# QizhiPei/FABind

Hardware: AMD Instinct MI355X
Metric: complexes/sec fwd+bwd (1500p/40l nodes), full IaBNet on the whole graph (pocket model + 4-layer complex model + distance-map head on all nodes / pairs) with the pocket-cls + pocket-centre + coord + distmap + distmap-by-coords + distill losses (BASELINE configs[2] read literally) (higher is better)
Workload: dtype bf16

## Files before the change

fabind_amd/_lib.py:

```python
import ctypes
import os

import torch

from . import config as _cfg

_HERE = os.path.dirname(os.path.abspath(__file__))
LIB_PATH = _cfg.knob("FABIND_LIB") or os.path.join(_HERE, "libfabind_hip.so")

ABI_VERSION = 19
DT_F32, DT_BF16 = 0, 1
ACT_NONE, ACT_SILU, ACT_RELU, ACT_SIGMOID, ACT_STORED_DERIV = 0, 1, 2, 3, 4
GEMM_FAM_NT_F32, GEMM_FAM_NT_F32_BF16, GEMM_FAM_NT_BF16, GEMM_FAM_GLDS, GEMM_FAM_PIPE, GEMM_FAM_X3, GEMM_FAM_X3_PRO, GEMM_FAM_PERSIST = range(8)

LNR_8S16, LNR_8S32, LNR_V8_1, LNR_V8_2, LNR_V8_3, LNR_V8_4, LNR_S2, LNR_S8, LNR_S16, LNR_S32, LNR_COUNT = range(11)
LNB_8S16, LNB_8S32, LNB_V8_1, LNB_V8_2, LNB_V8_3, LNB_S2, LNB_S8, LNB_S16, LNB_S20, LNB_S32, LNB_COUNT = range(11)
RST_BF16_1, RST_BF16_2, RST_BF16_4, RST_GENERIC, RST_COUNT = range(5)
ELF_WAVE1, ELF_WAVE1_TAIL, ELF_WAVE2_TAIL, ELF_CHUNK, ELF_COUNT = range(5)
ELB_NPL1, ELB_NPL2, ELB_NPL3, ELB_COUNT = range(4)

_vp, _i, _f, _l = ctypes.c_void_p, ctypes.c_int, ctypes.c_float, ctypes.c_long


class GemmArgs(ctypes.Structure):
    _fields_ = [(n, _vp) for n in ("A", "A2", "W", "C", "bias", "R", "r_index", "dotvec", "dot_out", "aux", "groups", "C2")] + \
               [(n, _i) for n in ("M", "N", "K", "K1", "lda", "lda2", "ldw", "ldc", "ldr", "ldaux", "dot_ld",
                                  "a_dtype", "w_dtype", "c_dtype", "aux_dtype", "act_pro", "act_epi", "dact_epi",
                                  "accumulate", "store_preact", "n_groups", "max_m", "max_n", "groups_ext", "epi_fast", "k_splits")] + \
               [("alpha", _f), ("p_drop", _f), ("drop_seed", ctypes.c_uint)] + \
               [(n, _vp) for n in ("row_mu", "row_rs", "col_c", "C16")] + [("ldc16", _i), ("split3", _i), ("r_dtype", _i), ("c2_bf16", _i)]


class EdgeBwdArgs(ctypes.Structure):
    _fields_ = [(n, _vp) for n in ("AB", "row", "col", "rhohat", "w_r", "W2p", "Wcp", "W2Tp", "WcTp", "b2", "bc", "w3", "ds",
                                  "dagg", "S1", "Mm", "dT", "dP2", "dP1", "drh", "dABrow", "part", "dbg", "bnd", "d2scratch")] + \
               [(n, _i) for n in ("ldab", "lddagg", "lddab", "E")] + [("p_drop", _f), ("seed", ctypes.c_uint), ("xcd_aware", _i), ("lddab16", _i), ("dAB16", _vp),
                                                                  ("d2f", _vp), ("z3f", _vp)]


class PairUpdateArgs(ctypes.Structure):
    _fields_ = [(n, _vp) for n in ("T", "p_node", "c_node", "z_in", "z_out", "Wop", "bo", "ln_w", "ln_b", "W1p", "b1", "W2p", "b2",
                                  "Wbp", "bb", "bias_out")] + \
               [(n, _i) for n in ("ldt", "b_off", "n_pairs")] + [("eps", _f), ("p_drop", _f), ("seed", ctypes.c_uint)]


class TnJob(ctypes.Structure):
    _fields_ = [(n, _vp) for n in ("Y", "X", "C_part", "out", "out_tail")] + \
               [(n, _i) for n in ("ldy", "ldx", "M", "N", "E", "splits", "e_per", "n_tiles", "with_colsum", "out_dt", "ldo",
                                  "wg0", "n_wg", "blk0", "n_blk", "pad_")]


class AttnFusedBwdArgs(ctypes.Structure):
    _fields_ = [(n, _vp) for n in ("qg", "kv", "a0", "bo", "boT", "toff", "koff", "bconst", "desc", "desc_p", "out", "lse", "dout",
                                  "dqg", "dkv", "dO", "Dv", "da0", "acat", "colpart", "part")] + \
               [(n, _i) for n in ("ldq", "ldkv", "lda0", "ldda0", "ldacat", "kcol0", "ldcolpart", "kp")] + [("scale", _f)] + \
               [(n, _i) for n in ("nsplit", "B", "part_rows")]


class AdamRow(ctypes.Structure):
    _fields_ = [(n, _vp) for n in ("p", "g", "m", "v")] + [("numel", ctypes.c_longlong), ("chunk0", _i), ("step_idx", _i)] + \
               [(n, ctypes.c_double) for n in ("lr", "beta1", "beta2", "eps", "weight_decay")] + [("decoupled", _i), ("pad_", _i)]


SIGNATURES = {
    "fabind_gemm": [ctypes.POINTER(GemmArgs), _vp],
    "fabind_gemm_plan": [ctypes.POINTER(GemmArgs), ctypes.POINTER(_i), ctypes.POINTER(_i), ctypes.POINTER(_i)],
    "fabind_gemm_tn_multi": [_vp, _vp, _i, _vp, _i, _vp, _i, _vp, _vp],
    "fabind_gemm_tn": [_vp, _i, _vp, _i, _vp, _i, _i, _i, _i, _vp, _vp, _i, _i, _vp],
    "fabind_transpose_act": [_vp, _i, _i, _vp, _i, _i, _i, _i, _i, _vp],
    "fabind_colsum": [_vp, _i, _i, _vp, _i, _i, _i, _vp, _i, _vp],
    "fabind_edges_count": [_vp, _vp, _vp, _i, _i, _vp, _vp, _f, _f, _vp, _vp, _vp],
    "fabind_edges_fill": [_vp, _vp, _vp, _i, _i, _vp, _vp, _vp, _f, _f, _vp, _vp, _vp, _vp, _vp, _vp, _vp],
    "fabind_exclusive_scan": [_vp, _vp, _i, _vp],
    "fabind_inter_meta": [_vp, _vp, _i, _vp, _vp, _vp, _i, _vp, _vp, _vp, _vp, _vp, _vp],
    "fabind_edge_geom": [_vp, _vp, _vp, _vp, _vp, _i, _vp, _vp, _vp, _vp, _vp],
    "fabind_gcl_pre": [_vp, _i, _i, _i, _vp, _vp, _vp, _vp, _vp, _i, _i, _i, _vp, _vp],
    "fabind_gcl_edge_fused": [_vp, _i, _i, _vp, _vp, _vp, _vp, _vp, _vp, _vp, _vp, _vp, _i, _vp, _vp, _f, ctypes.c_uint, _vp, _vp, _vp],
    "fabind_gcl_edge_fused_train": [_vp, _i, _i, _vp, _vp, _vp, _vp, _vp, _vp, _vp, _vp, _vp, _i, _vp, _vp, _f, ctypes.c_uint, _vp, _vp, _vp, _vp, _vp, _vp],
    "fabind_gcl_edge_fused_x3": [_vp, _i, _i, _i, _vp, _vp, _vp, _vp, _vp, _vp, _vp, _vp, _vp, _vp, _vp, _i, _vp, _vp, _f, ctypes.c_uint, _vp, _vp],
    "fabind_gcl_edge_fused_x3_train": [_vp, _i, _i, _i, _vp, _vp, _vp, _vp, _vp, _vp, _vp, _vp, _vp, _vp, _vp, _i, _vp, _vp, _f, ctypes.c_uint, _vp, _vp, _vp, _vp, _vp],
    "fabind_gcl_edge_fused_bwd": [ctypes.POINTER(EdgeBwdArgs), _i, _i, _vp],
    "fabind_pair_update_fused": [ctypes.POINTER(PairUpdateArgs), _i, _vp],
    "fabind_gcl_edge_fused_bwd_set_tile": [_i],
    "fabind_gcl_edge_fused_bwd_tile": [],
    "fabind_gcl_edge_fused_bwd_set_variant": [_i],
    "fabind_gcl_edge_fused_set_variant": [_i],
    "fabind_gcl_edge_fused_variant": [],
    "fabind_gcl_edge_fused_bwd_variant": [],
    "fabind_gcl_edge_fused_bwd_variant_for": [_i],
    "fabind_row_stats": [_vp, _i, _i, _f, _i, _i, _vp, _vp, _vp],
    "fabind_layernorm_rows": [_vp, _i, _i, _vp, _vp, _f, _i, _i, _vp, _i, _i, _i, _vp],
    "fabind_edge_ln_concat": [_vp, _i, _i, _vp, _vp, _vp, _vp, _vp, _f, _i, _vp, _i, _i, _i, _vp],
    "fabind_edge_lnfold": [_vp, _i, _i, _i, _vp, _vp, _vp, _vp, _f, _vp, _vp, _vp, _vp, _i, _vp, _f, ctypes.c_uint, _vp],
    "fabind_edge_lnfold_bwd_blocks": [_i],
    "fabind_edge_lnfold_bwd": [_vp, _i, _i, _i, _vp, _vp, _vp, _vp, _f, _vp, _vp, _vp, _vp, _vp, _i, _f, _vp, _vp, _vp, _vp, _i, _vp],
    "fabind_layernorm_rows_form": [_vp, _i, _i, _vp, _i, _i],
    "fabind_layernorm_rows_bwd_form": [_vp, _i, _vp, _i, _vp, _i, _i],
    "fabind_row_stats_form": [_vp, _i, _i, _i],
    "fabind_edge_lnfold_form": [_i, _i, ctypes.POINTER(_i)],
    "fabind_edge_lnfold_blocks": [_i],
    "fabind_edge_lnfold_bwd_form": [_i, ctypes.POINTER(_i)],
    "fabind_inter_coord_fold_blocks": [_i],
    "fabind_inter_coord_fold": [_vp, _i, _i, _vp, _vp, _vp, _f, _f, _vp, _vp, _vp, _i, _vp, _f, ctypes.c_uint, _vp],
    "fabind_post_optimize": [_vp, _vp, _vp, _vp, _vp, _i, _i, _i, _i, _f, _vp, _vp, _vp, _vp],
    "fabind_sym_automorphisms": [_vp, _vp, _vp, _vp, _i, _i, _i, _vp, _vp, _vp, _vp, _vp, _vp],
    "fabind_sym_score": [_vp, _i, _i, _vp, _vp, _vp, _vp, _vp, _i, _i, _vp, _vp, _vp, _vp, _vp, _vp],
    "fabind_pose_stats": [_vp, _vp, _vp, _i, _vp, _vp, _vp],
    "fabind_rank_loss_fwd": [_vp, _vp, _vp, _i, _i, _i, _vp, _vp, _vp, _vp],
    "fabind_multi_copy": [_vp, _i, _i, _vp],
    "fabind_adam_chunk": [],
    "fabind_multi_sqnorm": [_vp, _i, _i, _vp, _vp, _vp, _vp],
    "fabind_multi_adam": [_vp, _i, _i, _vp, _vp, _vp, _f, _i, _vp, _vp, _vp],
    "fabind_zero_empty_rows": [_vp, _i, _vp, _i, _i, _i, _vp, _i, _i, _vp],
    "fabind_split_sum": [_vp, _i, ctypes.c_long, _vp, _i, ctypes.c_long, _vp, _vp],
    "fabind_segment_sum": [_vp, _i, _i, _i, _vp, _vp, _i, _i, _i, _vp, _i, _vp, _i, _vp],
    "fabind_coord_update": [_vp, _vp, _vp, _i, _vp, _vp, _i, _i, _f, _vp, _vp, _vp],
    "fabind_cross_attn_fwd": [_vp, _i, _vp, _vp, _i, _vp, _i, _vp, _i, _i, _i, _vp, _i, _i, _f, _vp, _i, _vp, _i, _vp, _i,
                              _vp],
    "fabind_cross_attn_mfma_fwd": [_vp, _i, _vp, _vp, _i, _vp, _i, _vp, _i, _i, _i, _vp, _i, _i, _f, _vp, _i, _vp, _i, _vp, _i,
                                   _vp],
    "fabind_cross_attn_fused_fwd": [_vp, _i, _vp, _vp, _i, _vp, _i, _vp, _i, _vp, _vp, _vp, _vp, _i, _i, _i, _i, _i, _f, _vp, _i, _vp, _i, _vp, _vp],
    "fabind_cross_attn_fused_bwd": [ctypes.POINTER(AttnFusedBwdArgs), _i, _i, _i, _i, _i, _i, _vp],
    "fabind_pair_bot_pack": [_vp, _i, _vp, _i, _vp, _vp, _vp, _vp, _i, _vp, _i, _l, _vp],
    "fabind_pair_bo_pack": [_vp, _i, _vp, _i, _vp, _vp, _vp, _vp, _i, _vp, _i, _l, _vp],
    "fabind_cross_attn_mfma_bwd": [_vp, _i, _vp, _i, _vp, _i, _i, _i, _vp, _i, _i, _i, _f, _vp, _vp, _vp, _vp, _vp, _vp, _vp,
                                   _vp, _vp, _vp],
    "fabind_pair_bmat": [_vp, _i, _vp, _i, _i, _vp, _i, _vp, _i, _vp],
    "fabind_pair_hadamard": [_vp, _vp, _i, _i, _vp, _vp, _i, _i, _vp, _vp, _i, _vp, _i, _i, _vp],
    "fabind_inter_attn_fwd": [_vp, _i, _vp, _i, _i, _vp, _i, _vp, _vp, _vp, _vp, _vp, _vp, _vp, _i, _vp, _vp, _vp,
                              _vp, _f, _i, _vp, _vp, _vp, _vp, _vp, _vp, _vp],
    "fabind_inter_attn_fwd_rows": [_vp, _i, _vp, _i, _i, _vp, _i, _vp, _vp, _vp, _vp, _vp, _vp, _vp, _i, _vp, _vp, _vp,
                                   _vp, _f, _i, _vp, _vp, _vp, _vp, _vp, _vp, _vp, _i, _i, _vp],
    "fabind_layernorm_rows_bwd": [_vp, _i, _i, _vp, _vp, _i, _i, _f, _i, _i, _vp, _i, _i, _vp, _vp, _i, _vp],
    "fabind_edge_concat": [_vp, _i, _i, _vp, _vp, _vp, _i, _vp, _i, _i, _i, _vp],
    "fabind_las_step": [_vp, _vp, _vp, _vp, _vp, _vp, _vp, _i, _i, _f, _f, _vp, _vp, _vp],
    "fabind_select_rows": [_vp, _vp, _vp, _i, _i, _vp, _vp],
    "fabind_add": [_vp, _vp, _vp, _l, _vp],
    "fabind_mul_dact": [_vp, _i, _vp, _i, _i, _vp, _i, _l, _f, _vp],
    "fabind_mul_dact_colsum": [_vp, _i, _vp, _i, _i, _vp, _i, _i, _i, _vp, _vp, _i, _f, _vp],
    "fabind_drop_mix": [_vp, _vp, _vp, _l, _f, ctypes.c_uint, _vp],
    "fabind_drop_mix_bwd": [_vp, _vp, _vp, _l, _f, ctypes.c_uint, _vp],
    "fabind_mul_dropmask_colsum": [_vp, _i, _vp, _i, _i, _i, _f, ctypes.c_uint, _vp, _vp, _i, _vp],
    "fabind_rowdot_bwd": [_vp, _i, _vp, _i, _vp, _i, _i, _i, _vp, _vp, _vp, _i, _vp],
    "fabind_edge_geom_bwd": [_vp, _vp, _vp, _vp, _vp, _vp, _vp, _vp, _vp, _vp, _i, _i, _i, _vp, _vp, _vp, _vp],
    "fabind_gcl_pre_bwd": [_vp, _i, _i, _vp, _vp, _i, _vp, _vp, _vp, _i, _vp],
    "fabind_gather_dact": [_vp, _i, _vp, _vp, _i, _i, _vp, _i, _i, _i, _vp],
    "fabind_coord_update_bwd": [_vp, _vp, _vp, _i, _i, _f, _vp, _vp, _vp, _vp],
    "fabind_cross_attn_bwd": [_vp, _i, _vp, _i, _vp, _i, _i, _i, _vp, _i, _i, _i, _f, _vp, _vp, _vp, _vp, _vp, _vp, _vp,
                              _vp, _vp, _vp],
    "fabind_pair_bias_cat": [_vp, _i, _vp, _i, _i, _i, _vp, _i, _vp, _i, _vp, _vp, _i, _vp, _i, _vp, _vp],
    "fabind_batched_transpose_pad": [_vp, _i, _vp, _i, _i, _i, _i, _vp, _vp],
    "fabind_node_chain_fwd": [_vp, _i, _vp, _i, _vp, _vp, _vp, _vp, _vp, _vp, _i, _i, _vp, _i, _vp, _i, _vp, _i, _i, _i, _vp],
    "fabind_node_chain_x3_fwd": [_vp, _i, _vp, _i, _vp, _vp, _vp, _vp, _vp, _vp, _vp, _vp, _vp, _vp, _i, _i, _vp, _i, _vp, _i, _vp, _i, _vp, _i, _vp, _i,
                                 _i, _i, _vp],
    "fabind_rows_hadamard_bwd": [_vp, _i, _i, _vp, _i, _i, _vp, _vp, _vp, _i, _vp, _i, _vp],
    "fabind_pair_hadamard_bwd_grid": [_vp, _i, _i, _vp, _i, _i, _vp, _vp, _vp, _vp, _i, _vp, _i, _vp],
    "fabind_pair_hadamard_bwd_rows": [_vp, _i, _i, _vp, _i, _i, _vp, _i, _i, _vp, _vp, _vp, _vp, _i, _vp, _i, _vp, _i, _vp],
    "fabind_pair_hadamard_bwd": [_vp, _i, _i, _vp, _vp, _i, _i, _vp, _vp, _i, _i, _vp, _vp, _i, _vp, _vp, _i, _vp, _vp, _i,
                                 _vp],
    "fabind_inter_attn_bwd": [_vp, _i, _vp, _i, _i, _vp, _vp, _vp, _vp, _vp, _vp, _vp, _vp, _vp, _vp, _vp, _vp, _f, _i,
                              _vp, _vp, _vp, _vp, _vp, _vp, _vp, _vp, _vp, _vp, _i, _vp],
    "fabind_inter_attn_bwd_rows": [_vp, _i, _vp, _i, _i, _vp, _vp, _vp, _vp, _vp, _vp, _vp, _vp, _vp, _vp, _vp, _vp, _f, _i,
                                   _vp, _vp, _vp, _vp, _vp, _vp, _vp, _vp, _vp, _vp, _i, _vp, _i, _i, _vp],
    "fabind_las_step_bwd": [_vp, _vp, _vp, _vp, _vp, _vp, _vp, _vp, _i, _i, _f, _f, _vp, _vp, _vp],
    "fabind_pair_bias_bwd": [_vp, _i, _vp, _i, _i, _vp, _vp, _i, _i, _i, _vp, _vp, _vp, _vp, _vp],
    "fabind_pair_bias_btcat": [_vp, _i, _vp, _vp, _vp, _i, _i, _i, _vp, _i, _i, _vp],
    "fabind_pair_bias_finish": [_vp, _vp, _i, _i, _vp, _vp, _i, _vp, _vp, _l, _vp],
    "fabind_pack_frag_multi": [_vp, _vp, _i, _vp],
    "fabind_lower_bound": [_vp, _i, _vp, _i, _vp, _vp],
    "fabind_pocket_center_fwd": [_vp, _vp, _vp, _vp, _i, _i, _f, _i, _vp, _vp, _vp],
    "fabind_pocket_center_bwd": [_vp, _vp, _vp, _vp, _i, _i, _f, _vp, _vp, _vp, _vp, _vp],
    "fabind_pair_dist_fwd": [_vp, _i, _i, _vp, _vp, _f, _f, _f, _vp, _vp],
    "fabind_pair_dist_bwd": [_vp, _i, _i, _vp, _vp, _vp, _f, _f, _f, _vp, _vp, _vp],
    "fabind_block_hadamard_fwd": [_vp, _i, _i, _vp, _i, _vp, _i, _i, _vp, _i, _vp],
    "fabind_block_hadamard_bwd": [_vp, _i, _i, _vp, _i, _vp, _i, _vp, _i, _i, _vp, _i, _i, _vp, _vp, _i, _vp, _i, _vp],
    "fabind_loss_fwd": [_vp, _vp, _l, _vp, _vp, _vp, _l, _vp, _vp, _i, _vp, _l, _vp, _vp, _l, _f, _f, _f, _f, _f, _f, _vp, _vp, _vp, _vp, _vp, _vp],
    "fabind_loss_bwd": [_vp, _vp, _l, _vp, _vp, _vp, _l, _vp, _vp, _i, _l, _vp, _vp, _l, _f, _f, _f, _f, _f, _f, _vp, _vp, _vp,
                        _vp, _vp, _vp, _vp, _vp, _vp],
    "fabind_layernorm_fwd": [_vp, _vp, _vp, _f, _i, _i, _vp, _vp, _vp, _vp],
    "fabind_layernorm_bwd": [_vp, _vp, _vp, _vp, _vp, _i, _i, _vp, _vp, _vp, _vp],
}

_lib = None


def load():
    global _lib
    if _lib is not None:
        return _lib
    if not os.path.exists(LIB_PATH):
        raise RuntimeError(
            "fabind_amd: %s is missing -- build it with `python -m fabind_amd.build` (hipcc, gfx950). "
            "There is no CPU/eager fallback for the hot path." % LIB_PATH)
    lib = ctypes.CDLL(LIB_PATH)
    lib.fabind_last_error.restype = ctypes.c_char_p
    lib.fabind_abi_version.restype = ctypes.c_int
    got = lib.fabind_abi_version()
    if got != ABI_VERSION:
# ... 68 lines not shown
```

fabind_amd/csrc/fused_common.h:

```cpp
#pragma once
#include "common.h"

#define FE_BM 64
#define FE_PRIO(x) __builtin_amdgcn_s_setprio(x)

__device__ __forceinline__ float fe_sigmoid(float x) { return __builtin_amdgcn_rcpf(1.0f + __builtin_amdgcn_exp2f(-1.44269504f * x)); }
__device__ __forceinline__ float fe_silu(float x) { return x * fe_sigmoid(x); }

__device__ __forceinline__ uint32_t fe_hash(uint32_t x) {
    x ^= x >> 16; x *= 0x7feb352dU; x ^= x >> 15; x *= 0x846ca68bU; x ^= x >> 16;
    return x;
}
__device__ __forceinline__ float fe_keep(uint32_t seed, uint32_t e, uint32_t c, uint32_t H, uint32_t thr16, float scale) {
    const uint32_t h = fe_hash(seed + (e >> 1) * H + c);
    return (((e & 1u) ? (h >> 16) : (h & 0xffffu)) >= thr16) ? scale : 0.f;
}

__device__ __forceinline__ void unpack8(const uint4 u, float* f) {
    f[0] = __uint_as_float(u.x << 16); f[1] = __uint_as_float(u.x & 0xffff0000u);
    f[2] = __uint_as_float(u.y << 16); f[3] = __uint_as_float(u.y & 0xffff0000u);
    f[4] = __uint_as_float(u.z << 16); f[5] = __uint_as_float(u.z & 0xffff0000u);
    f[6] = __uint_as_float(u.w << 16); f[7] = __uint_as_float(u.w & 0xffff0000u);
}
__device__ __forceinline__ uint4 pack8(const float* f) {
// ... 125 lines not shown
    bf16x8_t b0[4];
    fe_gemm_prefetch(Wp, wave, lane, b0);
    fe_gemm_rolled_pf<H, MI, SWAP, SWZ>(sX, Wp, wave, lane, acc, b0, wmode);
}
template <int H, int MI, bool SWAP = false, int SWZ = 7>
__device__ __forceinline__ void fe_gemm_rot(const bf16_t* sX, const bf16_t* __restrict__ Wp, int wave, int lane, f32x4_t (&acc)[MI][4]) {
    bf16x8_t b0[4];
    fe_gemm_prefetch(Wp, wave, lane, b0);
    fe_gemm_rot_pf<H, MI, SWAP, SWZ>(sX, Wp, wave, lane, acc, b0);
}

template <int H, int MI, int SWZ>
__device__ __forceinline__ void fe_gemm_x3(const bf16_t* sXh, const bf16_t* sXl, const bf16_t* __restrict__ Wph,
                                           const bf16_t* __restrict__ Wpl, int wave, int lane, f32x4_t (&acc)[MI][4]) {
    constexpr int NKS = H / 32;
    constexpr int NG = H / 16;
    const int fr = lane & 15, fq = lane >> 4;
    const bf16x8_t* wh = (const bf16x8_t*)Wph + ((size_t)wave * 4) * 64 + lane;
    const bf16x8_t* wl = (const bf16x8_t*)Wpl + ((size_t)wave * 4) * 64 + lane;
    bf16x8_t h0[4], l0[4], h1[4], l1[4];
#pragma unroll
    for (int j = 0; j < 4; ++j) { h0[j] = wh[(size_t)j * 64]; l0[j] = wl[(size_t)j * 64]; }
#pragma unroll 1
    for (int ks = 0; ks < NKS; ks += 2) {
#pragma unroll
        for (int j = 0; j < 4; ++j) { h1[j] = wh[((size_t)(ks + 1) * NG + j) * 64]; l1[j] = wl[((size_t)(ks + 1) * NG + j) * 64]; }
        bf16x8_t ah[MI], al[MI];
#pragma unroll
        for (int i = 0; i < MI; ++i) {
            const int r = i * 16 + fr;
            const int o = r * H + (((ks * 4 + fq) ^ (r & SWZ)) * 8);
            ah[i] = *(const bf16x8_t*)&sXh[o];
            al[i] = *(const bf16x8_t*)&sXl[o];
        }
        FE_PRIO(1);
#pragma unroll
        for (int i = 0; i < MI; ++i) {
#pragma unroll
            for (int j = 0; j < 4; ++j) acc[i][j] = __builtin_amdgcn_mfma_f32_16x16x32_bf16(h0[j], al[i], acc[i][j], 0, 0, 0);
#pragma unroll
            for (int j = 0; j < 4; ++j) acc[i][j] = __builtin_amdgcn_mfma_f32_16x16x32_bf16(l0[j], ah[i], acc[i][j], 0, 0, 0);
#pragma unroll
            for (int j = 0; j < 4; ++j) acc[i][j] = __builtin_amdgcn_mfma_f32_16x16x32_bf16(h0[j], ah[i], acc[i][j], 0, 0, 0);
        }
        FE_PRIO(0);
        {
            const int kn = min(ks + 2, NKS - 2);
#pragma unroll
            for (int j = 0; j < 4; ++j) { h0[j] = wh[((size_t)kn * NG + j) * 64]; l0[j] = wl[((size_t)kn * NG + j) * 64]; }
        }
#pragma unroll
        for (int i = 0; i < MI; ++i) {
            const int r = i * 16 + fr;
            const int o = r * H + ((((ks + 1) * 4 + fq) ^ (r & SWZ)) * 8);
            ah[i] = *(const bf16x8_t*)&sXh[o];
            al[i] = *(const bf16x8_t*)&sXl[o];
        }
        FE_PRIO(1);
#pragma unroll
        for (int i = 0; i < MI; ++i) {
#pragma unroll
            for (int j = 0; j < 4; ++j) acc[i][j] = __builtin_amdgcn_mfma_f32_16x16x32_bf16(h1[j], al[i], acc[i][j], 0, 0, 0);
#pragma unroll
            for (int j = 0; j < 4; ++j) acc[i][j] = __builtin_amdgcn_mfma_f32_16x16x32_bf16(l1[j], ah[i], acc[i][j], 0, 0, 0);
#pragma unroll
            for (int j = 0; j < 4; ++j) acc[i][j] = __builtin_amdgcn_mfma_f32_16x16x32_bf16(h1[j], ah[i], acc[i][j], 0, 0, 0);
        }
        FE_PRIO(0);
    }
}

__device__ __forceinline__ void fe_split2(float x0, float x1, uint32_t& hi, uint32_t& lo) {
    hi = pack2_bf16(x0, x1);
    lo = pack2_bf16(x0 - __uint_as_float(hi << 16), x1 - __uint_as_float(hi & 0xffff0000u));
}

template <int H>
__device__ __forceinline__ void fe_tile_store(const bf16_t* sB, bf16_t* __restrict__ g, int e0, int ne, int tid) {
    constexpr int CH = H / 8;
    bf16_t* gt = g + (size_t)e0 * H;
    for (unsigned q = tid; q < (unsigned)ne * CH; q += H) {
        const unsigned rw = q / CH, ch = q % CH;
        *(uint4*)&gt[rw * H + ch * 8] = *(const uint4*)&sB[rw * H + ((ch ^ (rw & 7)) * 8)];
    }
}

typedef unsigned int fe_u32x4_t __attribute__((ext_vector_type(4)));
__device__ __forceinline__ void fe_store16_stream(__amdgpu_buffer_rsrc_t rsrc, unsigned byte_off, const uint4 v) {
    __builtin_amdgcn_raw_buffer_store_b128(fe_u32x4_t{v.x, v.y, v.z, v.w}, rsrc, (int)byte_off, 0,  16);
}
__device__ __forceinline__ __amdgpu_buffer_rsrc_t fe_rsrc(void* base, unsigned bytes) {
    return __builtin_amdgcn_make_buffer_rsrc(base, 0, (int)bytes, 0x00020000);
}
template <int H>
__device__ __forceinline__ void fe_tile_store_stream(const bf16_t* sB, bf16_t* __restrict__ g, int e0, int ne, int tid) {
    constexpr int CH = H / 8;
    const __amdgpu_buffer_rsrc_t rs = fe_rsrc(g + (size_t)e0 * H, (unsigned)ne * H * 2);
    for (unsigned q = tid; q < (unsigned)ne * CH; q += H) {
        const unsigned rw = q / CH, ch = q % CH;
        fe_store16_stream(rs, (rw * H + ch * 8) * 2, *(const uint4*)&sB[rw * H + ((ch ^ (rw & 7)) * 8)]);
    }
}

template <int MI>
__device__ __forceinline__ void fe_zero(f32x4_t (&acc)[MI][4]) {
#pragma unroll
    for (int i = 0; i < MI; ++i)
#pragma unroll
        for (int j = 0; j < 4; ++j) acc[i][j] = f32x4_t{0.f, 0.f, 0.f, 0.f};
}


template <int H, bool WITH_RH, int BM_, int SWZ = 7>
__device__ __forceinline__ float fe_scan_rows(const bf16_t* sX, const int* sRow, const float* sRh, int ne, bool head_cont,
                                              bool tail_cont, float* out, unsigned ld, float* bnd_tile, int c,
                                              bf16_t* out16 = nullptr, unsigned ld16 = 0) {
    auto put = [&](int node, float v) {
        if (out) out[(unsigned)node * ld + c] = v;
        if (out16) out16[(unsigned)node * ld16 + c] = f32_to_bf16(v);
    };
    float run = 0.f, pwr = 0.f;
    int cur = sRow[0];
    bool first = true;
    for (int rw0 = 0; rw0 < ne; rw0 += 8) {
        int rr[8];
        float v[8], rhv[8];
#pragma unroll
        for (int u = 0; u < 8; ++u) {
            const int rw = min(rw0 + u, BM_ - 1);
            rr[u] = sRow[rw];
            rhv[u] = WITH_RH ? sRh[rw] : 0.f;
            v[u] = bf16_to_f32(sX[rw * H + (((c >> 3) ^ (rw & SWZ)) * 8) + (c & 7)]);
        }
#pragma unroll
        for (int u = 0; u < 8; ++u) {
            if (rw0 + u < ne) {
                if (rr[u] != cur) {
                    if (first && head_cont) bnd_tile[c] = run; else put(cur, run);
                    run = 0.f; cur = rr[u]; first = false;
                }
                run += v[u];
                if (WITH_RH) pwr += rhv[u] * v[u];
            }
        }
    }
    if (ne > 0) {
        if (first && head_cont) bnd_tile[c] = run;
        else if (tail_cont) bnd_tile[H + c] = run;
        else put(cur, run);
    }
    return pwr;
}

template <int H, bool WITH_RH, int SWZ>
__device__ __forceinline__ float fe_scan_runs64(const bf16_t* sX, const int* sRow, const float* sRh, int ne, bool head_cont,
                                                bool tail_cont, float* out, unsigned ld, float* bnd_tile, int c,
                                                bf16_t* out16 = nullptr, unsigned ld16 = 0, const bf16_t* sXlo = nullptr) {
    const int lane = threadIdx.x & 63;
    const int mine = sRow[lane], prev = sRow[max(lane - 1, 0)];
    const float rhl = WITH_RH ? sRh[lane] : 0.f;
    const unsigned long long m = __ballot(lane < ne && lane > 0 && mine != prev);
    const int c8 = c >> 3, c7 = c & 7;
    float v[64];
#pragma unroll
    for (int rw = 0; rw < 64; ++rw) v[rw] = bf16_to_f32(sX[rw * H + ((c8 ^ (rw & SWZ)) * 8) + c7]);
    if (sXlo) {
#pragma unroll
        for (int rw = 0; rw < 64; ++rw) v[rw] += bf16_to_f32(sXlo[rw * H + ((c8 ^ (rw & SWZ)) * 8) + c7]);
    }
    float run = 0.f, pwr = 0.f;
    int rs = 0;
    auto flush = [&](bool last) {
        if (rs == 0 && head_cont) bnd_tile[c] = run;
        else if (last && tail_cont) bnd_tile[H + c] = run;
        else {
            const unsigned node = (unsigned)__builtin_amdgcn_readlane(mine, rs);
            if (out) out[node * ld + c] = run;
            if (out16) out16[node * ld16 + c] = f32_to_bf16(run);
        }
    };
#pragma unroll
    for (int rw = 0; rw < 64; ++rw) {
        if (rw < ne) {
            if ((m >> rw) & 1ull) {
                flush(false);
                run = 0.f;
                rs = rw;
            }
            run += v[rw];
            if (WITH_RH) pwr += __builtin_bit_cast(float, __builtin_amdgcn_readlane(__builtin_bit_cast(int, rhl), rw)) * v[rw];
        }
    }
    if (ne > 0) flush(true);
    return pwr;
}

template <int BM>
__global__ void fe_boundary_fix_kernel(const int* __restrict__ row, int E, int H, const float* __restrict__ bnd, float* out,
                                       unsigned ld, bf16_t* out16 = nullptr, unsigned ld16 = 0) {
    const int t = blockIdx.x, e0 = t * BM, ne = min(BM, E - e0);
    if (ne <= 0 || e0 + ne >= E) return;
    const int r = row[e0 + ne - 1];
    if (row[e0 + ne] != r) return;
    if (row[e0] == r && e0 > 0 && row[e0 - 1] == r) return;
    for (int c = threadIdx.x; c < H; c += blockDim.x) {
        float sum = bnd[((size_t)t * 2 + 1) * H + c];
        for (int u = t + 1;; ++u) {
            const int f0 = u * BM, fn = min(BM, E - f0);
            sum += bnd[((size_t)u * 2) * H + c];
            const bool through = row[f0 + fn - 1] == r && f0 + fn < E && row[f0 + fn] == r;
            if (!through) break;
        }
        if (out) out[(unsigned)r * ld + c] = sum;
        if (out16) out16[(unsigned)r * ld16 + c] = f32_to_bf16(sum);
    }
}

__device__ __forceinline__ float fe3_row16_sum(float v) {
#define FE_DPP_ADD(ctrl_) v += __builtin_bit_cast(float, __builtin_amdgcn_update_dpp(0, __builtin_bit_cast(int, v), (ctrl_), 0xF, 0xF, true))
    FE_DPP_ADD(0xB1);
    FE_DPP_ADD(0x4E);
    FE_DPP_ADD(0x141);
    FE_DPP_ADD(0x140);
#undef FE_DPP_ADD
    return v;
}

typedef float fe_f2 __attribute__((ext_vector_type(2)));
__device__ __forceinline__ void fe3_silu_pair(const fe_f2 z, fe_f2& m, fe_f2& d) {
    const fe_f2 t = z * -1.44269504f;
    const fe_f2 o = fe_f2{__builtin_amdgcn_exp2f(t.x), __builtin_amdgcn_exp2f(t.y)} + 1.0f;
    const fe_f2 s = fe_f2{__builtin_amdgcn_rcpf(o.x), __builtin_amdgcn_rcpf(o.y)};
    m = z * s;
    d = s + (m - m * s);
}
__device__ __forceinline__ uint32_t fe3_pack(const fe_f2 v) { return pack2_bf16(v.x, v.y); }
__device__ __forceinline__ fe_f2 fe3_unpack(const uint32_t u) { return fe_f2{__uint_as_float(u << 16), __uint_as_float(u & 0xffff0000u)}; }

__device__ __forceinline__ uint4 fe3_bload16(const __amdgpu_buffer_rsrc_t rs, const unsigned voff, const unsigned soff) {
    const fe_u32x4_t v = __builtin_amdgcn_raw_buffer_load_b128(rs, (int)voff, (int)soff, 0);
    return make_uint4(v.x, v.y, v.z, v.w);
}
__device__ __forceinline__ void fe3_bstore16(const __amdgpu_buffer_rsrc_t rs, const unsigned voff, const unsigned soff, const uint4 v) {
    __builtin_amdgcn_raw_buffer_store_b128(fe_u32x4_t{v.x, v.y, v.z, v.w}, rs, (int)voff, (int)soff, 0);
}

struct FabindEdgeBwdArgs;
int fe_bwd3_launch(const FabindEdgeBwdArgs* a, int H, int bm, int n_groups, hipStream_t stream);
int fe_fwd3_launch(const float* AB, int ldab, int H, const int* row, const int* col, const float* rhohat, const float* w_r,
                   const void* W2ph, const void* W2pl, const float* b2, const void* Wcph, const void* Wcpl, const float* bc,
                   const float* w3, int E, float* agg, float* s_out, uint32_t thr16, float dscale, unsigned seed, float* bnd,
                   int xcd_aware, hipStream_t stream, void* Msave = nullptr, void* d2f = nullptr, void* z3f = nullptr);
int fe_fwd2_launch(const void* AB, int ldab, int H, const int* row, const int* col, const float* rhohat, const float* w_r,
                   const void* W2p, const float* b2, const void* Wcp, const float* bc, const float* w3, int E, float* agg,
                   float* s_out, uint32_t thr16, float dscale, unsigned seed, float* bnd, void* agg16, int xcd_aware, hipStream_t stream,
                   void* Msave = nullptr, void* d2f = nullptr, void* z3f = nullptr);
int fe_bwd4_launch(const FabindEdgeBwdArgs* a, int H, int n_groups, hipStream_t stream);
```

fabind_amd/csrc/fused_edge.hip:

```cpp
#include "common.h"
#include "fabind_hip.h"
#include "fused_common.h"

static int g_fe_xcd_aware = 1;
extern "C" void fabind_gcl_edge_fused_set_xcd_aware(int on) { g_fe_xcd_aware = on ? 1 : 0; }
static int g_fe_fwd_variant = 1;
extern "C" int fabind_gcl_edge_fused_set_variant(int v) {
    FB_REQUIRE(v == 1, "fabind_gcl_edge_fused_set_variant: 1 (row-wise / operand-swapped) is the only forward form built (variant 0 was retired in round 5)");
    g_fe_fwd_variant = v;
    return 0;
}
extern "C" int fabind_gcl_edge_fused_variant(void) { return g_fe_fwd_variant; }

static int fe_fwd_entry(const void* AB, int ldab, int H, const int* row, const int* col, const float* rhohat,
                        const float* w_r, const void* W2p, const float* b2, const void* Wcp, const float* bc,
                        const float* w3, int E, float* agg, float* s_out, float p_drop, unsigned seed,
                        float* bnd, void* agg16, void* Msave, void* d2f, void* z3f, hipStream_t stream) {
    if (E <= 0) return 0;
    FB_REQUIRE((Msave != nullptr) == (d2f != nullptr) && (Msave != nullptr) == (z3f != nullptr),
               "fabind_gcl_edge_fused_train: M, d2f and z3f come together");
    FB_REQUIRE(Msave == nullptr || g_fe_fwd_variant == 1, "fabind_gcl_edge_fused_train: the saving forward is the row-wise / operand-swapped kernel (variant 1)");
    FB_REQUIRE(bnd != nullptr, "fabind_gcl_edge_fused: bnd (ceil(E/64) x 2 x H floats of scratch) is required");
    FB_REQUIRE(p_drop >= 0.f && p_drop < 1.f, "fabind_gcl_edge_fused: p_drop in [0, 1)");
    const uint32_t thr16 = (uint32_t)(p_drop * 65536.0f + 0.5f);
    const float dscale = 1.0f / (1.0f - (float)thr16 / 65536.0f);
    FB_REQUIRE(H == 512 || H == 256 || H == 128 || H == 64, "fabind_gcl_edge_fused: H must be 64, 128, 256 or 512");
    FB_REQUIRE(ldab % 8 == 0, "fabind_gcl_edge_fused: ldab % 8");
    {
        const int rc = fe_fwd2_launch(AB, ldab, H, row, col, rhohat, w_r, W2p, b2, Wcp, bc, w3, E, agg, s_out, thr16, dscale, seed, bnd,
                                      agg16, g_fe_xcd_aware, stream, Msave, d2f, z3f);
        if (rc) return rc;
    }
    hipLaunchKernelGGL((fe_boundary_fix_kernel<FE_BM>), dim3((E + FE_BM - 1) / FE_BM), dim3(H < 256 ? H : 256), 0, stream, row, E, H,
                       bnd, agg, (unsigned)H, (bf16_t*)agg16, (unsigned)H);
    FB_CHECK_LAUNCH();
    return 0;
}

extern "C" int fabind_gcl_edge_fused(const void* AB, int ldab, int H, const int* row, const int* col, const float* rhohat,
                                     const float* w_r, const void* W2p, const float* b2, const void* Wcp, const float* bc,
                                     const float* w3, int E, float* agg, float* s_out, float p_drop, unsigned seed,
                                     float* bnd, void* agg16, hipStream_t stream) {
    return fe_fwd_entry(AB, ldab, H, row, col, rhohat, w_r, W2p, b2, Wcp, bc, w3, E, agg, s_out, p_drop, seed, bnd, agg16, nullptr, nullptr,
                        nullptr, stream);
}
extern "C" int fabind_gcl_edge_fused_train(const void* AB, int ldab, int H, const int* row, const int* col, const float* rhohat,
                                           const float* w_r, const void* W2p, const float* b2, const void* Wcp, const float* bc,
                                           const float* w3, int E, float* agg, float* s_out, float p_drop, unsigned seed,
                                           float* bnd, void* agg16, void* M, void* d2f, void* z3f, hipStream_t stream) {
    FB_REQUIRE(M != nullptr && d2f != nullptr && z3f != nullptr, "fabind_gcl_edge_fused_train: M, d2f, z3f are required");
    return fe_fwd_entry(AB, ldab, H, row, col, rhohat, w_r, W2p, b2, Wcp, bc, w3, E, agg, s_out, p_drop, seed, bnd, agg16, M, d2f, z3f, stream);
}

static int fe_x3_entry(const float* AB, int ldab, int n_rows, int H, const int* row, const int* col, const float* rhohat,
                       const float* w_r, const void* W2ph, const void* W2pl, const float* b2, const void* Wcph,
                       const void* Wcpl, const float* bc, const float* w3, int E, float* agg, float* s_out,
                       float p_drop, unsigned seed, float* bnd, void* Msave, void* d2f, void* z3f, hipStream_t stream) {
    if (E <= 0) return 0;
    FB_REQUIRE(bnd != nullptr, "fabind_gcl_edge_fused_x3: bnd (ceil(E/64) x 2 x H floats of scratch) is required");
    FB_REQUIRE(p_drop >= 0.f && p_drop < 1.f, "fabind_gcl_edge_fused_x3: p_drop in [0, 1)");
    FB_REQUIRE(H == 512 || H == 256 || H == 128 || H == 64, "fabind_gcl_edge_fused_x3: H must be 64, 128, 256 or 512");
    FB_REQUIRE(ldab % 4 == 0 && ((uintptr_t)AB & 15) == 0, "fabind_gcl_edge_fused_x3: AB must be 16-byte aligned with ldab % 4 == 0");
    FB_REQUIRE(n_rows >= 0 && (size_t)n_rows * (size_t)ldab * 4 < ((size_t)1 << 32), "fabind_gcl_edge_fused_x3: AB larger than 4 GiB (n_rows * ldab * 4 bytes): split the batch");
    const uint32_t thr16 = (uint32_t)(p_drop * 65536.0f + 0.5f);
    const float dscale = 1.0f / (1.0f - (float)thr16 / 65536.0f);
    const int rc = fe_fwd3_launch(AB, ldab, H, row, col, rhohat, w_r, W2ph, W2pl, b2, Wcph, Wcpl, bc, w3, E, agg, s_out, thr16, dscale,
                                  seed, bnd, g_fe_xcd_aware, stream, Msave, d2f, z3f);
    if (rc) return rc;
    hipLaunchKernelGGL((fe_boundary_fix_kernel<FE_BM>), dim3((E + FE_BM - 1) / FE_BM), dim3(H < 256 ? H : 256), 0, stream, row, E, H,
                       bnd, agg, (unsigned)H, (bf16_t*)nullptr, 0u);
    FB_CHECK_LAUNCH();
    return 0;
}
extern "C" int fabind_gcl_edge_fused_x3(const float* AB, int ldab, int n_rows, int H, const int* row, const int* col, const float* rhohat,
                                        const float* w_r, const void* W2ph, const void* W2pl, const float* b2, const void* Wcph,
                                        const void* Wcpl, const float* bc, const float* w3, int E, float* agg, float* s_out,
                                        float p_drop, unsigned seed, float* bnd, hipStream_t stream) {
    return fe_x3_entry(AB, ldab, n_rows, H, row, col, rhohat, w_r, W2ph, W2pl, b2, Wcph, Wcpl, bc, w3, E, agg, s_out, p_drop, seed, bnd,
                       nullptr, nullptr, nullptr, stream);
}
extern "C" int fabind_gcl_edge_fused_x3_train(const float* AB, int ldab, int n_rows, int H, const int* row, const int* col, const float* rhohat,
                                              const float* w_r, const void* W2ph, const void* W2pl, const float* b2, const void* Wcph,
                                              const void* Wcpl, const float* bc, const float* w3, int E, float* agg, float* s_out,
                                              float p_drop, unsigned seed, float* bnd, void* M, void* d2f, void* z3f, hipStream_t stream) {
    FB_REQUIRE(M != nullptr && d2f != nullptr && z3f != nullptr, "fabind_gcl_edge_fused_x3_train: M, d2f, z3f are required");
    return fe_x3_entry(AB, ldab, n_rows, H, row, col, rhohat, w_r, W2ph, W2pl, b2, Wcph, Wcpl, bc, w3, E, agg, s_out, p_drop, seed, bnd,
                       M, d2f, z3f, stream);
}

template <int H, int BM, bool DBG>
__global__ __launch_bounds__(H, (BM == 32 ? 4 : 2)) void gcl_edge_fused_bwd_kernel(const FabindEdgeBwdArgs p) {
    constexpr int TPE = H / BM;
    constexpr int CPT = BM / 8;
    constexpr int MI = BM / 16;
    extern __shared__ __attribute__((aligned(16))) unsigned char smem[];
    bf16_t* sX = (bf16_t*)smem;
    bf16_t* sY = sX + BM * H;
    int* sRow = (int*)(sY + BM * H);
    float* sDs = (float*)(sRow + BM);
    float* sRh = sDs + BM;
    const bf16_t* __restrict__ AB = (const bf16_t*)p.AB;
    const int tid = threadIdx.x, lane = tid & 63, wave = tid >> 6;
    const int fr = lane & 15, cq = lane >> 4;
    const int el = tid / TPE, cth = tid % TPE;
    const int n_tiles = (p.E + BM - 1) / BM;
    const uint32_t thr16 = (uint32_t)(p.p_drop * 65536.0f + 0.5f);
    const float dscale = 1.0f / (1.0f - (float)thr16 / 65536.0f);
    int cbase[2][2];
#pragma unroll
    for (int f0 = 0; f0 < 2; ++f0)
#pragma unroll
        for (int f2 = 0; f2 < 2; ++f2)
            cbase[f0][f2] = cq * 4 * H + (wave * 8 + (((cq & 1) ^ f2) << 2) + ((fr >> 3) ^ f0)) * 8 + (fr & 7);
#define FE_COFF(i, j, r) (cbase[(r) & 1][(j) >> 1] + ((i) * 16 + (r)) * H + ((((j) & 1) ^ ((r) >> 1)) * 16))
    long long tph[12] = {0, 0, 0, 0, 0, 0, 0, 0, 0, 0, 0, 0};
    long long tlast = 0;
#define FE_TICK(k_)                                                   \
    if constexpr (DBG) {                                              \
        const long long now_ = __builtin_readcyclecounter();         \
        tph[k_] += now_ - tlast;                                      \
        tlast = now_;                                                 \
    }
    float pb2[4] = {0.f, 0.f, 0.f, 0.f}, pbc[4] = {0.f, 0.f, 0.f, 0.f}, pw3[4] = {0.f, 0.f, 0.f, 0.f}, pwr = 0.f;

    uint4 pfa[CPT], pfb[CPT];
    const unsigned uld = (unsigned)p.ldab;
    auto fe_prefetch = [&](unsigned r, unsigned c) {
        const unsigned aoff = r * uld + cth * (CPT * 8), boff = c * uld + H + cth * (CPT * 8);
#pragma unroll
        for (int q = 0; q < CPT; ++q) {
            pfa[q] = *(const uint4*)(AB + (aoff + q * 8));
            pfb[q] = *(const uint4*)(AB + (boff + q * 8));
        }
    };
    int t_first, t_end, t_step;
    if (p.xcd_aware && (gridDim.x & 7) == 0) {
        const int tpx = (n_tiles + 7) / 8, xcd = blockIdx.x & 7;
        t_first = xcd * tpx + (int)(blockIdx.x >> 3);
        t_end = min(n_tiles, (xcd + 1) * tpx);
        t_step = (int)(gridDim.x >> 3);
    } else {
        t_first = blockIdx.x; t_end = n_tiles; t_step = gridDim.x;
    }
    unsigned ur = 0, uc = 0;
    if (t_first < t_end) {
        const int e0 = t_first * BM;
        if (el < min(BM, p.E - e0)) {
            ur = (unsigned)(p.row + e0)[(unsigned)el];
            uc = (unsigned)(p.col + e0)[(unsigned)el];
        }
    }
    fe_prefetch(ur, uc);

    for (int tile = t_first; tile < t_end; tile += t_step) {
        const int e0 = tile * BM;
        const int ne = min(BM, p.E - e0);
        int lz = 0;
        asm volatile("" : "+s"(lz));
        const float* w_r = p.w_r + lz;
        const float* b2 = p.b2 + lz;
        const float* bc = p.bc + lz;
        const float* w3 = p.w3 + lz;
        const bf16_t* W2p = (const bf16_t*)p.W2p + lz;
        const bf16_t* Wcp = (const bf16_t*)p.Wcp + lz;
        const bf16_t* W2Tp = (const bf16_t*)p.W2Tp + lz;
        const bf16_t* WcTp = (const bf16_t*)p.WcTp + lz;
        if constexpr (DBG) tlast = __builtin_readcyclecounter();
        const int* grow = p.row + e0;
        const int* gcol = p.col + e0;
        const float* grh = p.rhohat + e0;
        const float* gds = p.ds + e0;
        if (tid < BM) {
            const bool ok = tid < ne;
            sRow[tid] = ok ? grow[(unsigned)tid] : -1;
// ... 106 lines not shown
        fe_tile_store<H>(sX, (bf16_t*)p.dT, e0, ne, tid);
        FE_TICK(1)

#pragma unroll
        for (int i = 0; i < MI; ++i)
#pragma unroll
            for (int r = 0; r < 4; ++r) {
                const int rr = sRow[i * 16 + cq * 4 + r];
                const unsigned doff = (unsigned)max(rr, 0) * (unsigned)p.lddagg + wave * 64 + fr;
                const float keep = rr >= 0 ? 1.f : 0.f;
#pragma unroll
                for (int j = 0; j < 4; ++j) acc[i][j][r] = p.dagg[doff + j * 16] * keep;
            }
        FE_TICK(5)
        fe_gemm_rolled<H, MI>(sX, WcTp, wave, lane, acc);
        FE_TICK(2)
#pragma unroll 1
        for (int j = 0; j < 4; ++j) {
            FE_JADDR(j)
            float a2 = 0.f;
#pragma unroll
            for (int i = 0; i < MI; ++i)
#pragma unroll
                for (int r = 0; r < 4; ++r) {
                    const uint32_t pk = (r >> 1) ? d2b[i][0] : d2a[i][0];
                    const float dd = __uint_as_float((r & 1) ? (pk & 0xffff0000u) : (pk << 16));
                    const float dp = acc[i][0][r] * dd;
                    a2 += dp;
                    sY[FE_LOFF(i, r)] = f32_to_bf16(dp);
                }
            pb2[0] += a2;
            FE_ROT_ACC() FE_ROT_D2() FE_ROT4(pb2)
        }
        __syncthreads();
        FE_TICK(6)
        fe_tile_store<H>(sY, (bf16_t*)p.dP2, e0, ne, tid);
        FE_TICK(1)

        fe_prefetch(ur, uc);
        fe_zero(acc);
        fe_gemm_rolled<H, MI>(sY, W2Tp, wave, lane, acc);
        FE_TICK(2)
#pragma unroll 1
        for (int j = 0; j < 4; ++j) {
            FE_JADDR(j)
#pragma unroll
            for (int i = 0; i < MI; ++i)
#pragma unroll
                for (int r = 0; r < 4; ++r) sX[FE_LOFF(i, r)] = f32_to_bf16(acc[i][0][r]);
            FE_ROT_ACC()
        }
        __syncthreads();
        FE_TICK(7)

        if (el < ne) {
            const float rh = sRh[el];
            const float* wp = w_r + (unsigned)(cth * (CPT * 8));
            float dot = 0.f;
#pragma unroll
            for (int q = 0; q < CPT; ++q) {
                float fa[8], fb[8], g[8];
                unpack8(pfa[q], fa);
                unpack8(pfb[q], fb);
                uint4* sp = (uint4*)&sX[el * H + (((cth * CPT + q) ^ (el & 7)) * 8)];
                unpack8(*sp, g);
                const float4 w0 = *(const float4*)(wp + q * 8), w1 = *(const float4*)(wp + q * 8 + 4);
                const float wv[8] = {w0.x, w0.y, w0.z, w0.w, w1.x, w1.y, w1.z, w1.w};
#pragma unroll
                for (int k = 0; k < 8; ++k) {
                    const float z = fa[k] + fb[k] + rh * wv[k], sg = fe_sigmoid(z);
                    g[k] *= sg * (1.0f + z * (1.0f - sg));
                    dot += g[k] * wv[k];
                }
                *sp = pack8(g);
            }
#pragma unroll
            for (int o = 1; o < TPE; o <<= 1) dot += __shfl_xor(dot, o, 64);
            if (cth == 0) (p.drh + e0)[(unsigned)el] = dot;
        }
        ur = nr; uc = nc;
        fe_prefetch(ur, uc);
        __syncthreads();
        FE_TICK(8)
        fe_tile_store<H>(sX, (bf16_t*)p.dP1, e0, ne, tid);
        FE_TICK(1)

        {
            const bool head_cont = e0 > 0 && p.row[e0 - 1] == sRow[0];
            const bool tail_cont = e0 + ne < p.E && p.row[e0 + ne] == sRow[ne - 1];
            pwr += fe_scan_rows<H, true, BM>(sX, sRow, sRh, ne, head_cont, tail_cont, p.dABrow, (unsigned)p.lddab,
                                             p.bnd + (size_t)tile * 2 * H, tid);
        }
        __syncthreads();
        FE_TICK(9)
    }
    if constexpr (DBG) {
        if (p.dbg && blockIdx.x == 0 && tid == 0)
            for (int k = 0; k < 12; ++k) ((long long*)p.dbg)[k] = tph[k];
    }

    float* part = p.part + (size_t)blockIdx.x * 4 * H;
#pragma unroll
    for (int j = 0; j < 4; ++j) {
        float a = pb2[j], b = pbc[j], c = pw3[j];
        a += __shfl_xor(a, 16, 64); a += __shfl_xor(a, 32, 64);
        b += __shfl_xor(b, 16, 64); b += __shfl_xor(b, 32, 64);
        c += __shfl_xor(c, 16, 64); c += __shfl_xor(c, 32, 64);
        if (cq == 0) {
            const int colj = wave * 64 + j * 16 + fr;
            part[colj] = a; part[H + colj] = b; part[2 * H + colj] = c;
        }
    }
    part[3 * H + tid] = pwr;
}

#undef FE_COFF
#undef FE_ROT4
#undef FE_ROT_ACC
#undef FE_ROT_D2
#undef FE_JADDR
#undef FE_LOFF
#undef FE_TICK

static int g_fe_bwd_bm = 64;
extern "C" int fabind_gcl_edge_fused_bwd_set_tile(int bm) {
    FB_REQUIRE(bm == 64, "fabind_gcl_edge_fused_bwd_set_tile: 64 edges per tile (the 32-edge build of the two-tile kernel was retired in round 5)");
    g_fe_bwd_bm = bm;
    return 0;
}
extern "C" int fabind_gcl_edge_fused_bwd_tile(void) { return g_fe_bwd_bm; }
static bool g_fe_bwd_variant_set = false;
static int g_fe_bwd_variant = 5;
extern "C" int fabind_gcl_edge_fused_bwd_set_variant(int v) {
    FB_REQUIRE(v == 0 || v == 5,
               "fabind_gcl_edge_fused_bwd_set_variant: 0 (two LDS tiles of 64 edges: the default for H <= 128) or 5 (row-wise, operand-swapped in-place tile + store wave: the recompute default above); variants 1-4 were knobs nobody reached and were retired in round 5");
    g_fe_bwd_variant = v;
    g_fe_bwd_variant_set = true;
    return 0;
}
extern "C" int fabind_gcl_edge_fused_bwd_variant(void) { return g_fe_bwd_variant; }
extern "C" int fabind_gcl_edge_fused_bwd_variant_for(int H) {
    return (!g_fe_bwd_variant_set && g_fe_bwd_variant == 5 && H <= 128) ? 0 : g_fe_bwd_variant;
}

extern "C" int fabind_gcl_edge_fused_bwd(const FabindEdgeBwdArgs* a_in, int H, int n_groups, hipStream_t stream) {
    FabindEdgeBwdArgs a_copy = *a_in;
    a_copy.xcd_aware = g_fe_xcd_aware;
    const FabindEdgeBwdArgs* a = &a_copy;
    if (a->E <= 0 || n_groups <= 0) return 0;
    FB_REQUIRE(H == 512 || H == 256 || H == 128 || H == 64, "fabind_gcl_edge_fused_bwd: H must be 64, 128, 256 or 512");
    FB_REQUIRE(a->ldab % 8 == 0, "fabind_gcl_edge_fused_bwd: ldab % 8");
    FB_REQUIRE(a->p_drop >= 0.f && a->p_drop < 1.f, "fabind_gcl_edge_fused_bwd: p_drop in [0, 1)");
    const int g_fe_bwd_variant = fabind_gcl_edge_fused_bwd_variant_for(H);
    if (a->d2f != nullptr || a->z3f != nullptr) {
        FB_REQUIRE(a->d2f != nullptr && a->z3f != nullptr, "fabind_gcl_edge_fused_bwd: d2f and z3f (saved by fabind_gcl_edge_fused_train) come together");
        return fe_bwd4_launch(a, H, n_groups, stream);
    }
    if (g_fe_bwd_variant == 5) return fe_bwd3_launch(a, H, 64, n_groups, stream);
    FB_REQUIRE(a->dAB16 == nullptr, "fabind_gcl_edge_fused_bwd: dAB16 (bf16 receiving-side sums) exists in variant 5 only");
    FB_REQUIRE(a->bnd != nullptr, "fabind_gcl_edge_fused_bwd: bnd (ceil(E / tile) x 2 x H floats of scratch) is required");
    const int BMr = g_fe_bwd_bm;
    const size_t lds = (size_t)2 * BMr * H * 2 + BMr * (sizeof(int) + 2 * sizeof(float));
#define FE_LAUNCH2(HH, BB)                                                                                         \
    do {                                                                                                           \
        static bool set_ = false;                                                                                  \
        if (!set_) { (void)hipFuncSetAttribute((const void*)gcl_edge_fused_bwd_kernel<HH, BB, false>, hipFuncAttributeMaxDynamicSharedMemorySize, (int)lds); set_ = true; } \
        hipLaunchKernelGGL((gcl_edge_fused_bwd_kernel<HH, BB, false>), dim3(n_groups), dim3(HH), lds, stream, *a);  \
    } while (0)
#define FE_LAUNCH(HH) FE_LAUNCH2(HH, 64)
    if (a->dbg != nullptr && H == 512) {
        static bool setd_ = false;
        if (!setd_) { (void)hipFuncSetAttribute((const void*)gcl_edge_fused_bwd_kernel<512, 64, true>, hipFuncAttributeMaxDynamicSharedMemorySize, (int)lds); }
        hipLaunchKernelGGL((gcl_edge_fused_bwd_kernel<512, 64, true>), dim3(n_groups), dim3(512), lds, stream, *a);
    } else
    if (H == 512) FE_LAUNCH(512); else if (H == 256) FE_LAUNCH(256); else if (H == 128) FE_LAUNCH(128); else FE_LAUNCH(64);
    hipLaunchKernelGGL((fe_boundary_fix_kernel<64>), dim3((a->E + 63) / 64), dim3(H < 256 ? H : 256), 0, stream, a->row, a->E, H,
                           a->bnd, a->dABrow, (unsigned)a->lddab);
#undef FE_LAUNCH
#undef FE_LAUNCH2
#undef FE_COFF
#undef FE_ROT4
#undef FE_ROT_ACC
#undef FE_ROT_D2
#undef FE_JADDR
#undef FE_LOFF
#undef FE_TICK
    FB_CHECK_LAUNCH();
    return 0;
}
```

fabind_amd/csrc/fused_edge_bwd3.hip:

```cpp
#include "common.h"
#include "fabind_hip.h"
#include "fused_common.h"
#ifndef FE3_ROT
#define FE3_ROT 0
#endif

template <int H, int SWZ>
__device__ __forceinline__ void fe3_wave_store(const bf16_t* sB, bf16_t* __restrict__ g, int e0, int ne, int lane) {
    constexpr int CH = H / 8;
    bf16_t* gt = g + (size_t)e0 * H;
    const unsigned total = (unsigned)ne * CH;
#pragma unroll 8
    for (unsigned q = lane; q < total; q += 64) {
        const unsigned rw = q / CH, ch = q % CH;
        *(uint4*)&gt[rw * H + ch * 8] = *(const uint4*)&sB[rw * H + ((ch ^ (rw & SWZ)) * 8)];
    }
}

template <int H, int SWZ>
__device__ __forceinline__ void fe3_wave_store_nt(const bf16_t* sB, bf16_t* __restrict__ g, int e0, int ne, int lane) {
    constexpr int CH = H / 8;
    const __amdgpu_buffer_rsrc_t rs = fe_rsrc(g + (size_t)e0 * H, (unsigned)ne * H * 2);
    const unsigned total = (unsigned)ne * CH;
#pragma unroll 8
    for (unsigned q = lane; q < total; q += 64) {
        const unsigned rw = q / CH, ch = q % CH;
        const uint4 v = *(const uint4*)&sB[rw * H + ((ch ^ (rw & SWZ)) * 8)];
        __builtin_amdgcn_raw_buffer_store_b128(fe_u32x4_t{v.x, v.y, v.z, v.w}, rs, (int)((rw * H + ch * 8) * 2), 0,  2);
    }
}

template <int H, int BM, bool DROP, bool DBG>
__global__ __launch_bounds__(H + 64) void gcl_edge_fused_bwd3_kernel(const FabindEdgeBwdArgs p, const int xf) {
    constexpr int MI = BM / 16;
    constexpr int NW = H / 64;
    constexpr int CH = H / 8;
    constexpr int EPW = 64 / CH;
    constexpr int EPI = NW * EPW;
    constexpr int NIT = BM / EPI;
    constexpr int PB = (NIT % 8 == 0) ? 8 : (NIT % 6 == 0) ? 6 : 4;
    static_assert(NIT % PB == 0 && BM % 16 == 0, "tile height");
    constexpr int SWZ = (H >= 128) ? 15 : 7;
    extern __shared__ __attribute__((aligned(16))) unsigned char smem[];
    bf16_t* sX = (bf16_t*)smem;
    bf16_t* sD = sX + BM * H;
    int* sTab = (int*)(sD + BM * H);
    float* sPart = (float*)(sTab + 8 * BM);
    const bf16_t* __restrict__ AB = (const bf16_t*)p.AB;
    const int tid = threadIdx.x, lane = tid & 63, wave = tid >> 6;
    const int n_tiles = (p.E + BM - 1) / BM;
    int t_first, t_end, t_step;
    if (p.xcd_aware && (gridDim.x & 7) == 0) {
        const int tpx = (n_tiles + 7) / 8, xcd = blockIdx.x & 7;
        t_first = xcd * tpx + (int)(blockIdx.x >> 3);
        t_end = min(n_tiles, (xcd + 1) * tpx);
        t_step = (int)(gridDim.x >> 3);
    } else {
        t_first = blockIdx.x; t_end = n_tiles; t_step = gridDim.x;
    }

    if (wave == NW) {
        __syncthreads();
        for (int tile = t_first; tile < t_end; tile += t_step) {
            const int e0 = tile * BM;
            const int ne = min(BM, p.E - e0);
            const bool st = !(xf & 1), nt = (xf & 32) == 0;
            auto put = [&](bf16_t* dst) {
                if (nt) fe3_wave_store_nt<H, SWZ>(sX, dst, e0, ne, lane); else fe3_wave_store<H, SWZ>(sX, dst, e0, ne, lane);
            };
            __syncthreads();
            if (st) put((bf16_t*)p.S1);
            fe3_wave_store<H, SWZ>(sD, (bf16_t*)p.d2scratch + (size_t)blockIdx.x * (BM * H), 0, BM, lane);
            __syncthreads();
            __syncthreads();
            if (st) put((bf16_t*)p.Mm);
            __syncthreads();
            __syncthreads();
            if (st) put((bf16_t*)p.dT);
            __syncthreads();
            __syncthreads();
            if (st) put((bf16_t*)p.dP2);
            __syncthreads();
            __syncthreads();
            __syncthreads();
            if (st) put((bf16_t*)p.dP1);
            __syncthreads();
        }
        __syncthreads();
        return;
    }

    const int fr = lane & 15, cq = lane >> 4;
    const int sub = lane / CH, ch = lane % CH;
    const uint32_t thr16 = (uint32_t)(p.p_drop * 65536.0f + 0.5f);
    const float dscale = 1.0f / (1.0f - (float)thr16 / 65536.0f);
    for (int k = 0; k < 4; ++k) sPart[k * H + tid] = 0.f;
    const unsigned uld = (unsigned)p.ldab;
    const __amdgpu_buffer_rsrc_t rs_d1 = fe_rsrc((bf16_t*)p.d2scratch + (size_t)blockIdx.x * (BM * H), BM * H * 2);
    const unsigned rw_off = (unsigned)((wave * EPW + sub) * CH + ch) * 16;
    const __amdgpu_buffer_rsrc_t rs_ab = fe_rsrc(const_cast<void*>(p.AB), 0xffffffffu);
    const __amdgpu_buffer_rsrc_t rs_dagg = fe_rsrc(const_cast<float*>(p.dagg), 0xffffffffu);
    const int cx = (wave * 8 + (cq >> 1)) ^ (fr & SWZ);
    const int lbase = fr * H + (cq & 1) * 4;
    const int wmode = DBG ? ((xf >> 2) & 3) : 0;
#define FE_QOFF(i, j) (lbase + (i) * 16 * H + ((cx ^ ((j) * 2)) * 8))
    const int fcol = wave * 64 + cq * 4;
    long long tph[12] = {0, 0, 0, 0, 0, 0, 0, 0, 0, 0, 0, 0};
    long long tlast = 0;
#define FE_TICK(k_)                                                   \
    if constexpr (DBG) {                                              \
        const long long now_ = __builtin_readcyclecounter();         \
        tph[k_] += now_ - tlast;                                      \
        tlast = now_;                                                 \
    }
    int tb_r = -1, tb_c = 0;
    float tb_d = 0.f, tb_h = 0.f;
    auto fetch_tables = [&](int tile) {
        const int e0 = tile * BM;
        const int ne = min(BM, p.E - e0);
        if (tid < BM) {
            const bool ok = tid < ne;
            const unsigned ge = (unsigned)(e0 + (ok ? tid : 0));
            const int r = p.row[ge], c = p.col[ge];
            const float d = p.ds[ge], h = p.rhohat[ge];
            tb_r = ok ? r : -1; tb_c = ok ? c : 0; tb_d = ok ? d : 0.f; tb_h = ok ? h : 0.f;
        }
    };
    auto commit_tables = [&](int hb) {
        int* tb = sTab + hb * 4 * BM;
        if (tid < BM) {
            tb[tid] = tb_r;
            tb[BM + tid] = tb_c;
            ((float*)tb)[2 * BM + tid] = tb_d;
            ((float*)tb)[3 * BM + tid] = tb_h;
        }
    };
    constexpr int NB = NIT / PB;
    uint4 ga[NB][PB], gb[NB][PB];
    auto gather_batch = [&](const int* tab, int b) {
#pragma unroll
        for (int u = 0; u < PB; ++u) {
            const int e = (b * PB + u) * EPI + wave * EPW + sub;
            const unsigned r = (unsigned)max(tab[e], 0), c = (unsigned)tab[BM + e];
            ga[b][u] = fe3_bload16(rs_ab, (r * uld + ch * 8) * 2, 0);
            gb[b][u] = fe3_bload16(rs_ab, (c * uld + H + ch * 8) * 2, 0);
        }
    };
    static_assert(BM <= H, "one thread per table row");
    if (t_first < t_end) { fetch_tables(t_first); commit_tables(0); }
    __syncthreads();
    int hb = 0;

    for (int tile = t_first; tile < t_end; tile += t_step, hb ^= 1) {
        const int e0 = tile * BM;
        const int ne = min(BM, p.E - e0);
        const int* sRow = sTab + hb * 4 * BM;
        const int* sCol = sRow + BM;
        const float* sDs = (const float*)(sRow + 2 * BM);
        const float* sRh = (const float*)(sRow + 3 * BM);
        int lz = 0;
        asm volatile("" : "+s"(lz));
        const float* w_r = p.w_r + lz;
        const float* b2 = p.b2 + lz;
        const float* bc = p.bc + lz;
        const float* w3 = p.w3 + lz;
        const bf16_t* W2p = (const bf16_t*)p.W2p + lz;
        const bf16_t* Wcp = (const bf16_t*)p.Wcp + lz;
        const bf16_t* W2Tp = (const bf16_t*)p.W2Tp + lz;
// ... 157 lines not shown

        fe_zero(acc);
        if (DBG || FE3_ROT == 0) fe_gemm_rolled<H, MI, true, SWZ>(sX, W2Tp, wave, lane, acc, wmode);
        else fe_gemm_rot<H, MI, true, SWZ>(sX, W2Tp, wave, lane, acc);
        __syncthreads();
        FE_TICK(2)
        uint4 gd[NIT];
#pragma unroll
        for (int it = 0; it < NIT; ++it) gd[it] = fe3_bload16(rs_d1, rw_off, (unsigned)(it * EPI * CH * 16));
#pragma unroll
        for (int j = 0; j < 4; ++j)
#pragma unroll
            for (int i = 0; i < MI; ++i)
                *(uint2*)&sX[FE_QOFF(i, j)] = make_uint2(pack2_bf16(acc[i][j][0], acc[i][j][1]), pack2_bf16(acc[i][j][2], acc[i][j][3]));
        __syncthreads();
        FE_TICK(7)

        const bool has_next = tile + t_step < t_end;
        {
            fe_f2 wv2[4];
            {
                const float4 w0 = *(const float4*)(w_r + ch * 8), w1 = *(const float4*)(w_r + ch * 8 + 4);
                wv2[0] = fe_f2{w0.x, w0.y}; wv2[1] = fe_f2{w0.z, w0.w}; wv2[2] = fe_f2{w1.x, w1.y}; wv2[3] = fe_f2{w1.z, w1.w};
            }
#pragma unroll
            for (int it0 = 0; it0 < NIT; it0 += PB) {
#pragma unroll
                for (int u = 0; u < PB; ++u) {
                    const int e = (it0 + u) * EPI + wave * EPW + sub;
                    uint4* sp = (uint4*)&sX[e * H + ((ch ^ (e & SWZ)) * 8)];
                    const uint4 gs = *sp;
                    const uint4 gq = gd[it0 + u];
                    const uint32_t ug[4] = {gs.x, gs.y, gs.z, gs.w}, ud[4] = {gq.x, gq.y, gq.z, gq.w};
                    uint32_t pg[4];
                    fe_f2 dot2 = fe_f2{0.f, 0.f};
#pragma unroll
                    for (int k = 0; k < 4; ++k) {
                        const fe_f2 g = fe3_unpack(ug[k]) * fe3_unpack(ud[k]);
                        dot2 += g * wv2[k];
                        pg[k] = fe3_pack(g);
                    }
                    float dot = dot2.x + dot2.y;
                    *sp = make_uint4(pg[0], pg[1], pg[2], pg[3]);
                    if constexpr (CH >= 16) {
                        dot = fe3_row16_sum(dot);
#pragma unroll
                        for (int o = 16; o < CH; o <<= 1) dot += __shfl_xor(dot, o, 64);
                    } else {
#pragma unroll
                        for (int o = 1; o < CH; o <<= 1) dot += __shfl_xor(dot, o, 64);
                    }
                    if (ch == 0 && e < ne) (p.drh + e0)[(unsigned)e] = dot;
                }
            }
        }
        __syncthreads();
        FE_TICK(8)

        if (has_next) fetch_tables(tile + t_step);
        if (!(xf & 16)) {
            const bool head_cont = e0 > 0 && p.row[e0 - 1] == sRow[0];
            const bool tail_cont = e0 + ne < p.E && p.row[e0 + ne] == sRow[ne - 1];
            sPart[3 * H + tid] += fe_scan_rows<H, true, BM, SWZ>(sX, sRow, sRh, ne, head_cont, tail_cont, p.dAB16 ? nullptr : p.dABrow, (unsigned)p.lddab,
                                                         p.bnd + (size_t)tile * 2 * H, tid, (bf16_t*)p.dAB16, (unsigned)p.lddab16);
        }
        if (has_next) commit_tables(hb ^ 1);
        __syncthreads();
        FE_TICK(9)
    }
    if constexpr (DBG) {
        if (p.dbg && blockIdx.x == 0 && tid == 0)
            for (int k = 0; k < 12; ++k) ((long long*)p.dbg)[k] = tph[k];
    }
    __syncthreads();
    float* part = p.part + (size_t)blockIdx.x * 4 * H;
    for (int k = 0; k < 4; ++k) part[k * H + tid] = sPart[k * H + tid];
#undef FE_QOFF
#undef FE_TICK
}

static int g_fe_bwd3_exp = 0;
extern "C" void fabind_gcl_edge_fused_bwd3_set_exp(int m) { g_fe_bwd3_exp = m; }

int fe_bwd3_launch(const FabindEdgeBwdArgs* a, int H, int bm, int n_groups, hipStream_t stream) {
    FB_REQUIRE(a->d2scratch != nullptr, "fabind_gcl_edge_fused_bwd: the store-wave form needs d2scratch (n_groups x 64 x H x 2 bytes)");
    FB_REQUIRE(a->bnd != nullptr, "fabind_gcl_edge_fused_bwd: bnd (ceil(E / tile) x 2 x H floats of scratch) is required");
    FB_REQUIRE(a->lddagg % 4 == 0 && ((uintptr_t)a->dagg & 15) == 0, "fabind_gcl_edge_fused_bwd: dagg must be 16-byte aligned with lddagg % 4 == 0");
    const size_t lds = (size_t)2 * bm * H * 2 + (size_t)8 * bm * sizeof(int) + (size_t)4 * H * sizeof(float);
#define FE_LAUNCH3_(HH, BB, KK, DD)                                                                                   \
    do {                                                                                                           \
        static bool set_ = false;                                                                                  \
        if (!set_) {                                                                                               \
            const hipError_t e_ = hipFuncSetAttribute((const void*)gcl_edge_fused_bwd3_kernel<HH, BB, KK, DD>,         \
                                                      hipFuncAttributeMaxDynamicSharedMemorySize, (int)lds);       \
            if (e_ != hipSuccess) { fabind_set_error(hipGetErrorString(e_)); return (int)e_; }                     \
            set_ = true;                                                                                           \
        }                                                                                                          \
        hipLaunchKernelGGL((gcl_edge_fused_bwd3_kernel<HH, BB, KK, DD>), dim3(n_groups), dim3(HH + 64), lds, stream, *a, g_fe_bwd3_exp); \
    } while (0)
#define FE_LAUNCH3(HH, BB, DD) do { if (a->p_drop > 0.f) FE_LAUNCH3_(HH, BB, true, DD); else FE_LAUNCH3_(HH, BB, false, DD); } while (0)
    FB_REQUIRE(bm == 64, "fabind_gcl_edge_fused_bwd: the store-wave form has 64-edge tiles");
    if (a->dbg != nullptr && H == 512) FE_LAUNCH3(512, 64, true);
    else if (H == 512) FE_LAUNCH3(512, 64, false); else if (H == 256) FE_LAUNCH3(256, 64, false);
    else if (H == 128) FE_LAUNCH3(128, 64, false); else FE_LAUNCH3(64, 64, false);
    hipLaunchKernelGGL((fe_boundary_fix_kernel<64>), dim3((a->E + 63) / 64), dim3(H < 256 ? H : 256), 0, stream, a->row, a->E, H,
                       a->bnd, a->dAB16 ? nullptr : a->dABrow, (unsigned)a->lddab, (bf16_t*)a->dAB16, (unsigned)a->lddab16);
#undef FE_LAUNCH3
#undef FE_LAUNCH3_
    FB_CHECK_LAUNCH();
    return 0;
}
```

fabind_amd/csrc/fused_edge_bwd4.hip:

```cpp
#include "common.h"
#include "fabind_hip.h"
#include "fused_common.h"

#ifndef FE4_E3_DB
#define FE4_E3_DB 0
#endif
#ifndef FE4_SCAN64
#define FE4_SCAN64 0
#endif
#ifndef FE4_P5_BATCH
#define FE4_P5_BATCH 4
#endif

#ifndef FE4_NT_LOADS
#define FE4_NT_LOADS 1
#endif
#if FE4_NT_LOADS
typedef unsigned fe_u32x2_nt_t __attribute__((ext_vector_type(2)));
__device__ __forceinline__ uint2 fe4_ldq(const bf16_t* p_) { const fe_u32x2_nt_t v = __builtin_nontemporal_load((const fe_u32x2_nt_t*)p_); return make_uint2(v.x, v.y); }
#else
__device__ __forceinline__ uint2 fe4_ldq(const bf16_t* p_) { return *(const uint2*)p_; }
#endif

template <int H>
__global__ __launch_bounds__(H, 4) void gcl_edge_fused_bwd4_kernel(const FabindEdgeBwdArgs p, const int xf) {
    constexpr int BM = FE_BM, MI = BM / 16;
    constexpr int NW = H / 64;
    constexpr int CH = H / 8;
    constexpr int EPW = 64 / CH;
    constexpr int EPI = NW * EPW;
    constexpr int NIT = BM / EPI;
    constexpr int SWZ = (H >= 128) ? 15 : 7;
    static_assert(BM <= H, "one thread per table row");
    extern __shared__ __attribute__((aligned(16))) unsigned char smem[];
    bf16_t* sX = (bf16_t*)smem;
    int* sTab = (int*)(sX + BM * H);
    float* sPart = (float*)(sTab + 8 * BM);
    const int tid = threadIdx.x, lane = tid & 63, wave = tid >> 6;
    const int fr = lane & 15, cq = lane >> 4;
    const int sub = lane / CH, ch = lane % CH;
    const int n_tiles = (p.E + BM - 1) / BM;
    int t_first, t_end, t_step;
    if (p.xcd_aware && (gridDim.x & 7) == 0) {
        const int tpx = (n_tiles + 7) / 8, xcd = blockIdx.x & 7;
        t_first = xcd * tpx + (int)(blockIdx.x >> 3);
        t_end = min(n_tiles, (xcd + 1) * tpx);
        t_step = (int)(gridDim.x >> 3);
    } else {
        t_first = blockIdx.x; t_end = n_tiles; t_step = gridDim.x;
    }
    for (int k = 0; k < 4; ++k) sPart[k * H + tid] = 0.f;
    const unsigned uld = (unsigned)p.ldab;
    const __amdgpu_buffer_rsrc_t rs_ab = fe_rsrc(const_cast<void*>(p.AB), 0xffffffffu);
    const __amdgpu_buffer_rsrc_t rs_dagg = fe_rsrc(const_cast<float*>(p.dagg), 0xffffffffu);
    const bf16_t* __restrict__ d2f = (const bf16_t*)p.d2f;
    const bf16_t* __restrict__ z3f = (const bf16_t*)p.z3f;
    const int cx = (wave * 8 + (cq >> 1)) ^ (fr & SWZ);
    const int lbase = fr * H + (cq & 1) * 4;
#define FE_OPAQUE(v_) asm volatile("" : "+v"(v_))
#define FE_QOFF(i, j) (lb_ + (i) * 16 * H + ((cx_ ^ ((j) * 2)) * 8))
#define FE_FOFF(i, j) (fbase + (size_t)((i) * 4 + (j)) * 256)
    const int fcol = wave * 64 + cq * 4;

    int tb_r = -1, tb_c = 0;
    float tb_d = 0.f, tb_h = 0.f;
    auto fetch_tables = [&](int tile) {
        const int e0 = tile * BM;
        const int ne = min(BM, p.E - e0);
        if (tid < BM) {
            const bool ok = tid < ne;
            const unsigned ge = (unsigned)(e0 + (ok ? tid : 0));
            const int r = p.row[ge], c = p.col[ge];
            const float d = p.ds[ge], h = p.rhohat[ge];
            tb_r = ok ? r : -1; tb_c = ok ? c : 0; tb_d = ok ? d : 0.f; tb_h = ok ? h : 0.f;
        }
    };
    auto commit_tables = [&](int hb) {
        int* tb = sTab + hb * 4 * BM;
        if (tid < BM) {
            tb[tid] = tb_r;
            tb[BM + tid] = tb_c;
            ((float*)tb)[2 * BM + tid] = tb_d;
            ((float*)tb)[3 * BM + tid] = tb_h;
        }
    };
    if (t_first < t_end) { fetch_tables(t_first); commit_tables(0); }
    __syncthreads();
    int hb = 0;

    for (int tile = t_first; tile < t_end; tile += t_step, hb ^= 1) {
        const int e0 = tile * BM;
        const int ne = min(BM, p.E - e0);
        const int* sRow = sTab + hb * 4 * BM;
        const int* sCol = sRow + BM;
        const float* sDs = (const float*)(sRow + 2 * BM);
        const float* sRh = (const float*)(sRow + 3 * BM);
        int lz = 0;
        asm volatile("" : "+s"(lz));
        const float* w_r = p.w_r + lz;
        const float* w3 = p.w3 + lz;
        const bf16_t* W2Tp = (const bf16_t*)p.W2Tp + lz;
        const bf16_t* WcTp = (const bf16_t*)p.WcTp + lz;
        int ln_ = lane;
        FE_OPAQUE(ln_);
        const size_t fbase = (((size_t)tile * NW + wave) * (MI * 4) * 64 + ln_) * 4;
        auto copy_out = [&](void* dst) {
            const __amdgpu_buffer_rsrc_t rs = fe_rsrc((bf16_t*)dst + (size_t)e0 * H, (unsigned)ne * H * 2);
            int t_ = tid;
            FE_OPAQUE(t_);
#pragma unroll
            for (int it = 0; it < BM * CH / H; ++it) {
                const int q = t_ + it * H;
                const int rw = q / CH, c8 = q % CH;
                const uint4 v = *(const uint4*)&sX[rw * H + ((c8 ^ (rw & SWZ)) * 8)];
                __builtin_amdgcn_raw_buffer_store_b128(fe_u32x4_t{v.x, v.y, v.z, v.w}, rs, (int)((rw * H + c8 * 8) * 2), 0,  2);
            }
        };

        {
            int cx_ = cx, lb_ = lbase;
            FE_OPAQUE(cx_); FE_OPAQUE(lb_);
            uint2 zq[4][MI];
#pragma unroll
            for (int j = 0; j < 4; ++j)
#pragma unroll
                for (int i = 0; i < MI; ++i) zq[j][i] = fe4_ldq(&z3f[FE_FOFF(i, j)]);
            float dsr[MI];
#pragma unroll
            for (int i = 0; i < MI; ++i) dsr[i] = sDs[i * 16 + fr];
            float4 wq4[4];
#pragma unroll
            for (int j = 0; j < 4; ++j) wq4[j] = *(const float4*)(w3 + fcol + j * 16);
#pragma unroll
            for (int j = 0; j < 4; ++j) {
                const fe_f2 w01 = fe_f2{wq4[j].x, wq4[j].y}, w23 = fe_f2{wq4[j].z, wq4[j].w};
                fe_f2 a3a = fe_f2{0.f, 0.f}, a3b = a3a, aca = a3a, acb = a3a;
#pragma unroll
                for (int i = 0; i < MI; ++i) {
                    fe_f2 m01, d01, m23, d23;
                    fe3_silu_pair(fe3_unpack(zq[j][i].x), m01, d01);
                    fe3_silu_pair(fe3_unpack(zq[j][i].y), m23, d23);
                    const fe_f2 t01 = (w01 * dsr[i]) * d01, t23 = (w23 * dsr[i]) * d23;
                    a3a += m01 * dsr[i]; a3b += m23 * dsr[i];
                    aca += t01; acb += t23;
                    *(uint2*)&sX[FE_QOFF(i, j)] = make_uint2(fe3_pack(t01), fe3_pack(t23));
                }
                float a3[4] = {a3a.x, a3a.y, a3b.x, a3b.y}, ac[4] = {aca.x, aca.y, acb.x, acb.y};
#pragma unroll
                for (int r = 0; r < 4; ++r) { a3[r] = fe3_row16_sum(a3[r]); ac[r] = fe3_row16_sum(ac[r]); }
                if (fr < 4) {
                    const float va = fr == 0 ? a3[0] : fr == 1 ? a3[1] : fr == 2 ? a3[2] : a3[3];
                    const float vc = fr == 0 ? ac[0] : fr == 1 ? ac[1] : fr == 2 ? ac[2] : ac[3];
                    sPart[2 * H + fcol + j * 16 + fr] += va;
                    sPart[1 * H + fcol + j * 16 + fr] += vc;
                }
                __builtin_amdgcn_sched_barrier(0);
            }
        }
        __syncthreads();

        if (!(xf & 1)) copy_out(p.dT);
        f32x4_t acc[MI][4];
        fe_zero(acc);
        if (!(xf & 8)) fe_gemm_rolled<H, MI, true, SWZ>(sX, WcTp, wave, lane, acc);
        __syncthreads();

        {
            int cx_ = cx, lb_ = lbase;
            FE_OPAQUE(cx_); FE_OPAQUE(lb_);
            float4 dg[FE4_E3_DB ? 2 : 1][MI];
            uint2 dq[FE4_E3_DB ? 2 : 1][MI];
            unsigned dgo[MI];
            float dgk[MI];
#pragma unroll
            for (int i = 0; i < MI; ++i) {
                const int rr = sRow[i * 16 + fr];
                dgk[i] = rr >= 0 ? 1.f : 0.f;
                dgo[i] = ((unsigned)max(rr, 0) * (unsigned)p.lddagg + fcol) * 4;
            }
            auto fetch_block = [&](int j, int slot) {
#pragma unroll
                for (int i = 0; i < MI; ++i) {
                    const uint4 v = fe3_bload16(rs_dagg, dgo[i], (unsigned)(j * 64));
                    dg[slot][i] = make_float4(__uint_as_float(v.x), __uint_as_float(v.y), __uint_as_float(v.z), __uint_as_float(v.w));
                    dq[slot][i] = fe4_ldq(&d2f[FE_FOFF(i, j)]);
                }
            };
            if (FE4_E3_DB) fetch_block(0, 0);
#pragma unroll
            for (int j = 0; j < 4; ++j) {
                if (FE4_E3_DB) { if (j < 3) fetch_block(j + 1, (j + 1) & 1); } else fetch_block(j, 0);
                fe_f2 a2a = fe_f2{0.f, 0.f}, a2b = a2a;
#pragma unroll
                for (int i = 0; i < MI; ++i) {
                    const float4 g4 = dg[FE4_E3_DB ? (j & 1) : 0][i];
                    const uint2 dd = dq[FE4_E3_DB ? (j & 1) : 0][i];
                    const fe_f2 p01 = (fe_f2{acc[i][j][0], acc[i][j][1]} + fe_f2{g4.x, g4.y} * dgk[i]) * fe3_unpack(dd.x);
                    const fe_f2 p23 = (fe_f2{acc[i][j][2], acc[i][j][3]} + fe_f2{g4.z, g4.w} * dgk[i]) * fe3_unpack(dd.y);
                    a2a += p01; a2b += p23;
                    *(uint2*)&sX[FE_QOFF(i, j)] = make_uint2(fe3_pack(p01), fe3_pack(p23));
                }
                float a2[4] = {a2a.x, a2a.y, a2b.x, a2b.y};
#pragma unroll
                for (int r = 0; r < 4; ++r) a2[r] = fe3_row16_sum(a2[r]);
                if (fr < 4) sPart[fcol + j * 16 + fr] += fr == 0 ? a2[0] : fr == 1 ? a2[1] : fr == 2 ? a2[2] : a2[3];
                __builtin_amdgcn_sched_barrier(0);
            }
        }
        __syncthreads();

        if (!(xf & 1)) copy_out(p.dP2);
        fe_zero(acc);
        if (!(xf & 8)) fe_gemm_rolled<H, MI, true, SWZ>(sX, W2Tp, wave, lane, acc);
        __syncthreads();
        {
            int cx_ = cx, lb_ = lbase;
            FE_OPAQUE(cx_); FE_OPAQUE(lb_);
#pragma unroll
            for (int j = 0; j < 4; ++j)
#pragma unroll
                for (int i = 0; i < MI; ++i)
                    *(uint2*)&sX[FE_QOFF(i, j)] = make_uint2(pack2_bf16(acc[i][j][0], acc[i][j][1]), pack2_bf16(acc[i][j][2], acc[i][j][3]));
        }
        __syncthreads();

        const bool has_next = tile + t_step < t_end;
        {
            int ch_ = ch, es_ = wave * EPW + sub;
            FE_OPAQUE(ch_); FE_OPAQUE(es_);
#define ch ch_
            fe_f2 wv2[4];
            {
                const float4 w0 = *(const float4*)(w_r + ch * 8), w1 = *(const float4*)(w_r + ch * 8 + 4);
                wv2[0] = fe_f2{w0.x, w0.y}; wv2[1] = fe_f2{w0.z, w0.w}; wv2[2] = fe_f2{w1.x, w1.y}; wv2[3] = fe_f2{w1.z, w1.w};
            }
            const __amdgpu_buffer_rsrc_t rs_s1 = fe_rsrc((bf16_t*)p.S1 + (size_t)e0 * H, (unsigned)ne * H * 2);
            const __amdgpu_buffer_rsrc_t rs_p1 = fe_rsrc((bf16_t*)p.dP1 + (size_t)e0 * H, (unsigned)ne * H * 2);
            constexpr int PB = (NIT % FE4_P5_BATCH == 0) ? FE4_P5_BATCH : NIT;
#pragma unroll
            for (int u0 = 0; u0 < NIT; u0 += PB) {
            uint4 ga[PB], gb[PB];
#pragma unroll
            for (int v = 0; v < PB; ++v) {
                const int e = (u0 + v) * EPI + es_;
                const unsigned r = (unsigned)max(sRow[e], 0), c = (unsigned)sCol[e];
                ga[v] = fe3_bload16(rs_ab, (r * uld + ch * 8) * 2, 0);
                gb[v] = fe3_bload16(rs_ab, (c * uld + H + ch * 8) * 2, 0);
            }
#pragma unroll
            for (int v = 0; v < PB; ++v) {
                const int u = v;
                const int e = (u0 + v) * EPI + es_;
                const float rh = sRh[e];
                uint4* sp = (uint4*)&sX[e * H + ((ch ^ (e & SWZ)) * 8)];
                const uint4 gs = *sp;
                const uint32_t ua[4] = {ga[u].x, ga[u].y, ga[u].z, ga[u].w}, ub[4] = {gb[u].x, gb[u].y, gb[u].z, gb[u].w};
                const uint32_t ug[4] = {gs.x, gs.y, gs.z, gs.w};
                uint32_t po[4], pg[4];
                fe_f2 dot2 = fe_f2{0.f, 0.f};
#pragma unroll
                for (int k = 0; k < 4; ++k) {
                    const fe_f2 z = fe3_unpack(ua[k]) + fe3_unpack(ub[k]) + wv2[k] * rh;
                    fe_f2 m, d;
                    fe3_silu_pair(z, m, d);
                    const fe_f2 g = fe3_unpack(ug[k]) * d;
                    dot2 += g * wv2[k];
                    po[k] = fe3_pack(m);
                    pg[k] = fe3_pack(g);
                }
                *sp = make_uint4(pg[0], pg[1], pg[2], pg[3]);
                const unsigned goff = (unsigned)(e * H + ch * 8) * 2;
                if (!(xf & 2)) {
                    __builtin_amdgcn_raw_buffer_store_b128(fe_u32x4_t{po[0], po[1], po[2], po[3]}, rs_s1, (int)goff, 0,  2);
                    __builtin_amdgcn_raw_buffer_store_b128(fe_u32x4_t{pg[0], pg[1], pg[2], pg[3]}, rs_p1, (int)goff, 0,  2);
                }
                float dot = dot2.x + dot2.y;
                if constexpr (CH >= 16) {
                    dot = fe3_row16_sum(dot);
#pragma unroll
                    for (int o = 16; o < CH; o <<= 1) dot += __shfl_xor(dot, o, 64);
                } else {
#pragma unroll
                    for (int o = 1; o < CH; o <<= 1) dot += __shfl_xor(dot, o, 64);
                }
                if (ch == 0 && e < ne) (p.drh + e0)[(unsigned)e] = dot;
            }
            }
#undef ch
        }
        __syncthreads();

        if (has_next) fetch_tables(tile + t_step);
        if (!(xf & 4)) {
            const bool head_cont = e0 > 0 && p.row[e0 - 1] == sRow[0];
            const bool tail_cont = e0 + ne < p.E && p.row[e0 + ne] == sRow[ne - 1];
#if FE4_SCAN64
            sPart[3 * H + tid] += fe_scan_runs64<H, true, SWZ>(sX, sRow, sRh, ne, head_cont, tail_cont, p.dAB16 ? nullptr : p.dABrow, (unsigned)p.lddab,
                                                              p.bnd + (size_t)tile * 2 * H, tid, (bf16_t*)p.dAB16, (unsigned)p.lddab16);
#else
            sPart[3 * H + tid] += fe_scan_rows<H, true, BM, SWZ>(sX, sRow, sRh, ne, head_cont, tail_cont, p.dAB16 ? nullptr : p.dABrow, (unsigned)p.lddab,
                                                                p.bnd + (size_t)tile * 2 * H, tid, (bf16_t*)p.dAB16, (unsigned)p.lddab16);
#endif
        }
        if (has_next) commit_tables(hb ^ 1);
        __syncthreads();
    }
    __syncthreads();
    float* part = p.part + (size_t)blockIdx.x * 4 * H;
    for (int k = 0; k < 4; ++k) part[k * H + tid] = sPart[k * H + tid];
#undef FE_QOFF
#undef FE_FOFF
#undef FE_OPAQUE
}

static int g_fe_bwd4_exp = 0;
extern "C" void fabind_gcl_edge_fused_bwd4_set_exp(int m) { g_fe_bwd4_exp = m; }

int fe_bwd4_launch(const FabindEdgeBwdArgs* a, int H, int n_groups, hipStream_t stream) {
    FB_REQUIRE(a->bnd != nullptr, "fabind_gcl_edge_fused_bwd: bnd (ceil(E / 64) x 2 x H floats of scratch) is required");
    FB_REQUIRE(a->lddagg % 4 == 0 && ((uintptr_t)a->dagg & 15) == 0, "fabind_gcl_edge_fused_bwd: dagg must be 16-byte aligned with lddagg % 4 == 0");
    const size_t lds = (size_t)FE_BM * H * 2 + (size_t)8 * FE_BM * sizeof(int) + (size_t)4 * H * sizeof(float);
#define FE_LAUNCH4(HH)                                                                                                \
    do {                                                                                                           \
        static bool set_ = false;                                                                                  \
        if (!set_) {                                                                                               \
            const hipError_t e_ = hipFuncSetAttribute((const void*)gcl_edge_fused_bwd4_kernel<HH>,                    \
                                                      hipFuncAttributeMaxDynamicSharedMemorySize, (int)lds);       \
            if (e_ != hipSuccess) { fabind_set_error(hipGetErrorString(e_)); return (int)e_; }                     \
            set_ = true;                                                                                           \
        }                                                                                                          \
        hipLaunchKernelGGL((gcl_edge_fused_bwd4_kernel<HH>), dim3(n_groups), dim3(HH), lds, stream, *a, g_fe_bwd4_exp); \
    } while (0)
    if (H == 512) FE_LAUNCH4(512); else if (H == 256) FE_LAUNCH4(256); else if (H == 128) FE_LAUNCH4(128); else FE_LAUNCH4(64);
#undef FE_LAUNCH4
    hipLaunchKernelGGL((fe_boundary_fix_kernel<64>), dim3((a->E + 63) / 64), dim3(H < 256 ? H : 256), 0, stream, a->row, a->E, H,
                       a->bnd, a->dAB16 ? nullptr : a->dABrow, (unsigned)a->lddab, (bf16_t*)a->dAB16, (unsigned)a->lddab16);
    FB_CHECK_LAUNCH();
    return 0;
}
```

fabind_amd/csrc/gcl.hip:

```cpp
#include "common.h"
#include "fabind_hip.h"

__global__ __launch_bounds__(256) void gcl_pre_kernel(const void* __restrict__ AB, int ab_dt, int ldab, int H,
                                                      const int* row, const int* col, const float* rhohat,
                                                      const float* __restrict__ w_r, void* pre, int pre_dt, int E, int act,
                                                      void* dact_out) {
    const int lane = threadIdx.x & 63;
    int e = blockIdx.x * 4 + (threadIdx.x >> 6);
    if (e >= E) return;
    const size_t a = (size_t)row[e] * ldab, b = (size_t)col[e] * ldab + H;
    const float rh = rhohat[e];
    for (int c = lane * 4; c < H; c += 256) {
        float4 va = ld4_any(AB, ab_dt, a + c), vb = ld4_any(AB, ab_dt, b + c), w = *(const float4*)(w_r + c);
        const float4 z = make_float4(va.x + vb.x + rh * w.x, va.y + vb.y + rh * w.y, va.z + vb.z + rh * w.z,
                                     va.w + vb.w + rh * w.w);
        st4_any(pre, pre_dt, (size_t)e * H + c,
                make_float4(apply_act(z.x, act), apply_act(z.y, act), apply_act(z.z, act), apply_act(z.w, act)));
        if (dact_out)
            st4_any(dact_out, pre_dt, (size_t)e * H + c,
                    make_float4(apply_dact(z.x, act), apply_dact(z.y, act), apply_dact(z.z, act), apply_dact(z.w, act)));
    }
}

#define GP_PASSES 4
// ... 183 lines not shown
                *(float4*)(o + 4) = make_float4(acc[s].v[4], acc[s].v[5], acc[s].v[6], acc[s].v[7]);
            }
            if (out16) st8_any(out16, FB_DT_BF16, (size_t)r * ldo16 + c, acc[s]);
        }
    }
}

template <int NSLAB>
__global__ __launch_bounds__(1024) void segment_sum_heavy_kernel(const void* __restrict__ Z, int z_dt, int ldz, int H,
                                                                 const int* rowptr, const int* eidx, int act, float* out,
                                                                 int ldo, int n_rows, bf16_t* out16, int ldo16, int rpw, int heavy_min) {
    __shared__ F8 part[15][NSLAB * 64];
    __shared__ int heavy[1024];
    __shared__ int n_heavy;
    const int lane = threadIdx.x & 63, w = threadIdx.x >> 6;
    if (threadIdx.x == 0) n_heavy = 0;
    __syncthreads();
    const int rr = blockIdx.x * rpw + threadIdx.x;
    if ((int)threadIdx.x < rpw && rr < n_rows && rowptr[rr + 1] - rowptr[rr] > heavy_min) heavy[atomicAdd(&n_heavy, 1)] = rr;
    __syncthreads();
    const int nh = n_heavy;
    for (int q = 0; q < nh; ++q) {
        const int r = heavy[q];
        F8 acc[NSLAB];
#pragma unroll
        for (int s = 0; s < NSLAB; ++s)
#pragma unroll
            for (int k = 0; k < 8; ++k) acc[s].v[k] = 0.f;
        ss_accum<NSLAB, 8 / NSLAB>(Z, z_dt, ldz, H, eidx, act, lane, rowptr[r] + w, rowptr[r + 1], 16, acc);
        if (w > 0) {
#pragma unroll
            for (int s = 0; s < NSLAB; ++s) part[w - 1][s * 64 + lane] = acc[s];
        }
        __syncthreads();
        if (w == 0) {
#pragma unroll
            for (int s = 0; s < NSLAB; ++s) {
                for (int k = 0; k < 15; ++k) {
                    const F8 p = part[k][s * 64 + lane];
#pragma unroll
                    for (int t = 0; t < 8; ++t) acc[s].v[t] += p.v[t];
                }
                const int c = s * 512 + lane * 8;
                if (c < H) {
                    if (out) {
                        float* o = out + (size_t)r * ldo + c;
                        *(float4*)o = make_float4(acc[s].v[0], acc[s].v[1], acc[s].v[2], acc[s].v[3]);
                        *(float4*)(o + 4) = make_float4(acc[s].v[4], acc[s].v[5], acc[s].v[6], acc[s].v[7]);
                    }
                    if (out16) st8_any(out16, FB_DT_BF16, (size_t)r * ldo16 + c, acc[s]);
                }
            }
        }
        __syncthreads();
    }
}

extern "C" int fabind_segment_sum(const void* Z, int z_dt, int ldz, int H, const int* rowptr, const int* eidx,
                                  int n_rows, int n_edges, int act, float* out, int ldo, void* out16v, int ldo16,
                                  hipStream_t stream) {
    bf16_t* out16 = (bf16_t*)out16v;
    FB_REQUIRE(H % 8 == 0 && ldz % 8 == 0 && ldo % 4 == 0, "fabind_segment_sum: H/ldz must be multiples of 8, ldo of 4");
    FB_REQUIRE(H <= 1024, "fabind_segment_sum: H <= 1024");
    FB_REQUIRE(out != nullptr || out16 != nullptr, "fabind_segment_sum: no output");
    FB_REQUIRE(((uintptr_t)Z % 16 == 0) && ((uintptr_t)out % 16 == 0), "fabind_segment_sum: 16-byte alignment");
    FB_REQUIRE(out16 == nullptr || (ldo16 % 8 == 0 && (uintptr_t)out16 % 16 == 0), "fabind_segment_sum: out16 needs 16-byte alignment and ldo16 % 8 == 0");
    if (n_rows <= 0) return 0;
    (void)n_edges;
    int rpw = 1024;
    while (rpw > 64 && (n_rows + rpw - 1) / rpw < 256) rpw >>= 1;
    const int heavy_min = n_rows < 16384 ? 32 : 128;
    const dim3 g((n_rows + 3) / 4), gh((n_rows + rpw - 1) / rpw);
    if (H <= 512) {
        hipLaunchKernelGGL((segment_sum_kernel<1>), g, dim3(256), 0, stream, Z, z_dt, ldz, H, rowptr, eidx, act, out, ldo, n_rows, out16, ldo16, heavy_min);
        hipLaunchKernelGGL((segment_sum_heavy_kernel<1>), gh, dim3(1024), 0, stream, Z, z_dt, ldz, H, rowptr, eidx, act, out, ldo, n_rows, out16, ldo16, rpw, heavy_min);
    } else {
        hipLaunchKernelGGL((segment_sum_kernel<2>), g, dim3(256), 0, stream, Z, z_dt, ldz, H, rowptr, eidx, act, out, ldo, n_rows, out16, ldo16, heavy_min);
        hipLaunchKernelGGL((segment_sum_heavy_kernel<2>), gh, dim3(1024), 0, stream, Z, z_dt, ldz, H, rowptr, eidx, act, out, ldo, n_rows, out16, ldo16, rpw, heavy_min);
    }
    FB_CHECK_LAUNCH();
    return 0;
}

__global__ __launch_bounds__(256) void coord_update_kernel(const float* __restrict__ x, const float* __restrict__ d,
                                                           const float* __restrict__ s_part, int n_part,
                                                           const float* weight, const int* rowptr, int n_rows, int mean,
                                                           float clampv, float* x_out, float* s_out) {
    const int lane = threadIdx.x & 63;
    int r = blockIdx.x * 4 + (threadIdx.x >> 6);
    if (r >= n_rows) return;
    const int e0 = rowptr[r], e1 = rowptr[r + 1];
    float ax = 0.f, ay = 0.f, az = 0.f;
    for (int e = e0 + lane; e < e1; e += 64) {
        float s = 0.f;
        for (int k = 0; k < n_part; ++k) s += s_part[(size_t)e * n_part + k];
        if (weight) s *= weight[e];
        if (s_out) s_out[e] = s;
        ax += d[(size_t)e * 3] * s; ay += d[(size_t)e * 3 + 1] * s; az += d[(size_t)e * 3 + 2] * s;
    }
    ax = wave_sum(ax); ay = wave_sum(ay); az = wave_sum(az);
    if (lane == 0) {
        const int deg = e1 - e0;
        const float den = mean ? (float)(deg < 1 ? 1 : deg) : 1.f;
        float tx = ax / den, ty = ay / den, tz = az / den;
        tx = fminf(fmaxf(tx, -clampv), clampv); ty = fminf(fmaxf(ty, -clampv), clampv); tz = fminf(fmaxf(tz, -clampv), clampv);
        x_out[(size_t)r * 3] = x[(size_t)r * 3] + tx;
        x_out[(size_t)r * 3 + 1] = x[(size_t)r * 3 + 1] + ty;
        x_out[(size_t)r * 3 + 2] = x[(size_t)r * 3 + 2] + tz;
    }
}

extern "C" int fabind_coord_update(const float* x, const float* d, const float* s_part, int n_part,
                                   const float* weight, const int* rowptr, int n_rows, int mean, float clampv,
                                   float* x_out, float* s_out, hipStream_t stream) {
    if (n_rows <= 0) return 0;
    hipLaunchKernelGGL(coord_update_kernel, dim3((n_rows + 3) / 4), dim3(256), 0, stream, x, d, s_part, n_part, weight,
                       rowptr, n_rows, mean, clampv, x_out, s_out);
    FB_CHECK_LAUNCH();
    return 0;
}

__global__ __launch_bounds__(256) void zero_empty_rows_kernel(const int* __restrict__ rowptr, int n_rows, void* out, int out_dt, int ld,
                                                              int C, void* out2, int out2_dt, int ld2) {
    const int lane = threadIdx.x & 63;
    const int r = blockIdx.x * 4 + (threadIdx.x >> 6);
    if (r >= n_rows || rowptr[r] != rowptr[r + 1]) return;
    for (int c = lane; c < C; c += 64) {
        st_any(out, out_dt, (size_t)r * ld + c, 0.f);
        if (out2) st_any(out2, out2_dt, (size_t)r * ld2 + c, 0.f);
    }
}

extern "C" int fabind_zero_empty_rows(const int* rowptr, int n_rows, void* out, int out_dt, int ld, int C, void* out2, int out2_dt,
                                      int ld2, hipStream_t stream) {
    if (n_rows <= 0 || C <= 0) return 0;
    FB_REQUIRE(rowptr != nullptr && out != nullptr, "fabind_zero_empty_rows: rowptr / out");
    hipLaunchKernelGGL(zero_empty_rows_kernel, dim3((n_rows + 3) / 4), dim3(256), 0, stream, rowptr, n_rows, out, out_dt, ld, C, out2,
                       out2_dt, ld2);
    FB_CHECK_LAUNCH();
    return 0;
}


__global__ __launch_bounds__(256) void pack_frag_multi_kernel(const FabindPackSeg* __restrict__ segs) {
    const FabindPackSeg sg = segs[blockIdx.y];
    const int N = sg.N, Kd = sg.K;
    const long n_vec = (long)N * Kd / 8;
    bf16_t* dst = (bf16_t*)sg.dst;
    for (long t = (long)blockIdx.x * 256 + threadIdx.x; t < n_vec; t += (long)gridDim.x * 256) {
        const int r = (int)(t & 15), q = (int)((t >> 4) & 3);
        const long tb = t >> 6;
        const int nb = (int)(tb % (N / 16)), kb = (int)(tb / (N / 16));
        const long n = (long)nb * 16 + r, k0 = (long)kb * 32 + q * 8;
        uint32_t w[4];
#pragma unroll
        for (int j = 0; j < 4; ++j) {
            float a, b;
            const long i0 = n * sg.src_sr + (k0 + 2 * j) * sg.src_sc, i1 = i0 + sg.src_sc;
            if (sg.src_dt == FB_DT_BF16) {
                a = bf16_to_f32(((const bf16_t*)sg.src)[i0]);
                b = bf16_to_f32(((const bf16_t*)sg.src)[i1]);
            } else {
                a = ((const float*)sg.src)[i0];
                b = ((const float*)sg.src)[i1];
                if (sg.src_dt == 2) {
                    const uint32_t h = pack2_bf16(a, b);
// ... 26 lines not shown
```

fabind_amd/engine.py:

```python
import math

import numpy as np
import torch

from . import config as _cfg
from . import kernels as K
from . import ops

from .config import fp32_storage, get_precision, set_precision, split_sites
from .config import x3_backward_bf16 as config_x3_backward_bf16
from .param_pack import EagerPack, ParamPack


FUSED_EDGE = True
LAYOUT_CACHE = _cfg.knob("FABIND_LAYOUT_CACHE")
DEBUG_GRAPH = _cfg.knob("FABIND_DEBUG_GRAPH")
DEBUG_CAPTURE = None


def _wd():
    return torch.float32 if fp32_storage() else torch.bfloat16


def _count(idx, n):
# ... 8 lines not shown
        import weakref
        if not LAYOUT_CACHE:
            return cls(batch_id, segment_id, n_pair_out)
        for ent in cls._cache:
            if ent[0]() is batch_id and ent[2]() is segment_id and ent[1] == batch_id._version and ent[3] == segment_id._version \
                    and ent[4] == n_pair_out:
                return ent[5]
        lay = cls(batch_id, segment_id, n_pair_out)
        cls._cache.insert(0, (weakref.ref(batch_id), batch_id._version, weakref.ref(segment_id), segment_id._version, n_pair_out, lay))
        del cls._cache[4:]
        return lay

    def __init__(self, batch_id, segment_id, n_pair_out=8):
        dev = batch_id.device
        B = int(batch_id[-1].item()) + 1
        seg = (segment_id > 0.5) if segment_id.is_floating_point() else segment_id.bool()
        bid = batch_id.long()
        bound = torch.searchsorted(bid, torch.arange(B + 1, dtype=torch.int64, device=dev))
        cs = torch.cat([torch.zeros(1, dtype=torch.int64, device=dev), torch.cumsum(seg.to(torch.int64), 0)])
        ok = (bid[1:] >= bid[:-1]).all().to(torch.int64).reshape(1) if bid.numel() > 1 else torch.ones(1, dtype=torch.int64, device=dev)
        cnt = torch.cat([bound[1:] - bound[:-1], cs[bound[1:]] - cs[bound[:-1]], ok]).cpu().numpy()
        if cnt[-1] != 1:
            raise ValueError("fabind_amd: batch_id must be sorted (the nodes of a complex contiguous), as the reference's to_dense_batch requires")
        n, P = cnt[:B].astype(np.int64), cnt[B:2 * B].astype(np.int64)
        C = n - P
        off = np.concatenate([[0], np.cumsum(n)])
        self.B, self.N = B, int(off[-1])
        self.n, self.P, self.C, self.off = n, P, C, off
        self.max_n, self.max_P, self.max_C = int(n.max()), int(P.max()), int(C.max())
        coff = np.concatenate([[0], np.cumsum(C)])
        poff = np.concatenate([[0], np.cumsum(P)])
        pair_off = np.concatenate([[0], np.cumsum(P * C)])
        self.n_pairs = int(pair_off[-1])
        self.sumC, self.sumP = int(coff[-1]), int(poff[-1])
        bidx = np.repeat(np.arange(B), n)
        loc = np.arange(self.N) - off[:-1][bidx]
        is_c = loc < C[bidx]
        c_index, p_index = np.nonzero(is_c)[0], np.nonzero(~is_c)[0]
        inv = np.empty(self.N, dtype=np.int64)
        inv[c_index] = np.arange(self.sumC)
        inv[p_index] = self.sumC + np.arange(self.sumP)
        lo = lambda v: (v & 0xFFFFFFFF).astype(np.uint32).astype(np.int64)
        hi = lambda v: v >> 32
        one, zero = np.ones(B, dtype=np.int64), np.zeros(B, dtype=np.int64)
        o, cf, pf, po = off[:-1], coff[:-1], poff[:-1], pair_off[:-1]
        NO = n_pair_out
        self.NO = NO
        desc = lambda cols: np.stack(cols, 1).reshape(-1)
        parts = dict(
            node_off=off, c_cnt=C, c_index=c_index, p_index=p_index, inv_perm=inv,
            desc_p=desc([pf, P, cf, C, lo(po), hi(po), C, one]),
            desc_c=desc([cf, C, pf, P, lo(po), hi(po), one, C]),
            desc_pf=desc([o + C, P, cf, C, lo(po), hi(po), C, one]),
            desc_cf=desc([cf, C, o + C, P, lo(po), hi(po), one, C]),
            pb_groups=desc([o + C, P, cf * NO, C * NO, lo(po * NO), hi(po * NO), C * NO, zero]),
            pb_tn_groups=desc([lo(po * NO), hi(po * NO), C * NO, C * NO, o + C, P, zero, zero]))
        flat = np.concatenate([np.asarray(v, dtype=np.int64) for v in parts.values()])
        flat = torch.from_numpy((flat & 0xFFFFFFFF).astype(np.uint32).view(np.int32)).to(dev)
        pos = 0
        for name, v in parts.items():
            t = flat[pos:pos + len(v)]
            pos += len(v)
            setattr(self, name, t.view(-1, 8) if name.startswith(("desc", "pb_")) else t)
        for name in ("desc_p", "desc_c", "desc_pf", "desc_cf"):
            getattr(self, name)._fab_covers_all = True
        self.c_index64, self.p_index64 = self.c_index.long(), self.p_index.long()
        self.inv_perm = self.inv_perm.long()
        self.pb_max_n = int((C * NO).max())
        self.coff, self.pair_off_np = coff, pair_off

    def ranges(self, idx_first):
        if idx_first.is_cuda and idx_first.dtype == torch.int32 and idx_first.is_contiguous():
            out = torch.empty(self.B + 1, dtype=torch.int32, device=idx_first.device)
            K.check(K._lib.load().fabind_lower_bound(K.ptr(idx_first), idx_first.shape[0], K.ptr(self.node_off), self.B + 1, K.ptr(out),
                                                     K.stream()), "fabind_lower_bound")
            return out
        which = torch.bucketize(idx_first, self.node_off[1:].to(idx_first.dtype), right=True)
        cnt = _count(which, self.B)
        out = torch.zeros(self.B + 1, dtype=torch.int32, device=idx_first.device)
        out[1:] = torch.cumsum(cnt, 0).to(torch.int32)
        return out


class Graph:
    _warned_fallback = False

    @torch.no_grad()
    def __init__(self, lay, x, bond_row, bond_col, bond_off, cut_intra, cut_inter):
        deg_ctx, deg_int = K.edges_count(x, lay.node_off, lay.c_cnt, lay.B, lay.max_n, bond_row, bond_off, cut_intra,
                                         cut_inter)
        rp_ctx, rp_int = K.exclusive_scan(deg_ctx), K.exclusive_scan(deg_int)
        lo = lay.node_off[:-1].long()
        n_lig_rows = (rp_int[lo + lay.c_cnt.long()] - rp_int[lo]).sum()
        E_ctx, E_int, n_half, n_act, n_heavy = torch.stack([rp_ctx[-1], rp_int[-1], n_lig_rows.to(rp_int.dtype), (deg_int > 0).sum().to(rp_int.dtype),
                                                            (deg_int > K.INTER_ATTN_HEAVY).sum().to(rp_int.dtype)]).tolist()
        if 2 * n_half != E_int:
            raise RuntimeError("fabind_amd: inter-graph is not symmetric (%d ligand-row edges of %d): finite coordinates: %s"
                               % (n_half, E_int, bool(torch.isfinite(x).all())))
        if E_int == 0:
            if get_precision() == "bf16" and not Graph._warned_fallback:
                Graph._warned_fallback = True
                import warnings
                warnings.warn("fabind_amd: no ligand-protein pair within the inter cut-off in this batch -- the reference's one "
                              "fake pair is used (att_model.py:85-86).  In bf16 mode ligand coordinates are accurate to only "
                              "~0.1-0.3 A on such inputs (long edges amplify bf16 operand rounding; DESIGN.md); use "
                              "engine.set_precision('fp32') if that matters.")
            u, v = 1, int(lay.C[0]) + 1
            deg_int[u] = 1
            deg_int[v] = 1
            rp_int = K.exclusive_scan(deg_int)
            E_int, n_act, n_heavy = 2, 2, 0
            self.col_ctx, self.row_ctx, _, _ = K.edges_fill(x, lay.node_off, lay.c_cnt, lay.B, lay.max_n, bond_row,
                                                            bond_col, bond_off, cut_intra, -1.0, rp_ctx, rp_ctx * 0,
                                                            E_ctx, 0)
            self.col_int = torch.tensor([v, u], dtype=torch.int32, device=x.device)
            self.row_int = torch.tensor([u, v], dtype=torch.int32, device=x.device)
        else:
            self.col_ctx, self.row_ctx, self.col_int, self.row_int = K.edges_fill(
                x, lay.node_off, lay.c_cnt, lay.B, lay.max_n, bond_row, bond_col, bond_off, cut_intra, cut_inter, rp_ctx,
                rp_int, E_ctx, E_int)
        self.rp_ctx, self.rp_int, self.E_ctx, self.E_int = rp_ctx, rp_int, E_ctx, E_int
        if DEBUG_GRAPH:
            r, c, Nn = self.row_int.long(), self.col_int.long(), lay.N
            k1, k2 = torch.sort(r * Nn + c)[0], torch.sort(c * Nn + r)[0]
            nbad = int((k1 != k2).sum())
            rr = torch.repeat_interleave(torch.arange(Nn, device=r.device), (rp_int[1:] - rp_int[:-1]).long())
            print("[fabind] graph check: E_int %d, col range [%d, %d] of %d, row mismatch %d, mirror mismatches %d, finite %s"
                  % (E_int, int(c.min()), int(c.max()), Nn, int((rr != r).sum()), nbad, bool(torch.isfinite(x).all())), flush=True)
        self.red_off, self.red_idx, self.red_c, self.red_p, self.mirror = K.inter_meta(
            lay.node_off, lay.c_cnt, lay.B, rp_int, self.col_int, self.row_int)
        self.int_deal = (torch.argsort(deg_int, descending=True, stable=True).to(torch.int32), int(n_heavy), int(n_act))
        self._ctx_bycol = None
        self.N = lay.N

    def int_by_col(self):
        return self.rp_int, self.mirror

    def ctx_by_col(self):
        if self._ctx_bycol is None:
            colsorted, perm = torch.sort(self.col_ctx.long(), stable=True)
            cnt = _count(colsorted, self.N)
            colptr = torch.zeros(self.N + 1, dtype=torch.int32, device=perm.device)
            colptr[1:] = torch.cumsum(cnt, 0).to(torch.int32)
            self._ctx_bycol = (colptr, perm.to(torch.int32).contiguous())
        return self._ctx_bycol


def _cat(ts, d=0):
    return torch.cat(list(ts), d)


def gcl_params(m, pk=None):
    wd = _wd()
    own = pk is None
    pk = pk or EagerPack(m.edge_mlp[0].weight.device)
    W1 = m.edge_mlp[0].weight
    Hin = (W1.shape[1] - 1) // 2
    H = W1.shape[0]
    d = dict(
        W_ab=pk.cat([W1[:, :Hin], W1[:, Hin:2 * Hin]], 0, wd, with_T=True),
        b_ab=pk.cat([m.edge_mlp[0].bias, pk.zeros(H)]),
        w_r=pk.copy(W1[:, 2 * Hin]), W2=pk.copy(m.edge_mlp[2].weight, wd), b2=pk.copy(m.edge_mlp[2].bias),
        Wc=pk.copy(m.coord_mlp[0].weight, wd), bc=pk.copy(m.coord_mlp[0].bias), w3=pk.copy(m.coord_mlp[2].weight[0]),
        Wn1=pk.copy(m.node_mlp[0].weight, wd, with_T=True), bn1=pk.copy(m.node_mlp[0].bias),
        Wn2=pk.copy(m.node_mlp[2].weight, wd, with_T=True), bn2=pk.copy(m.node_mlp[2].bias))
    return pk.resolve(d) if own else d


_PACK_CACHE = {}
_LAST_PARAMS = [None, None]


def last_params_of(model):
    ref = _LAST_PARAMS[0]
    return _LAST_PARAMS[1] if (ref is not None and ref() is model) else list(model.parameters())


def cached_pack(model, builder):
    params = list(model.parameters())
    import weakref
    _LAST_PARAMS[:] = [weakref.ref(model), params]
    if torch.is_grad_enabled() and any(p.requires_grad for p in params):
        return builder(model)
    key = (get_precision(), split_sites(), tuple((p.data_ptr(), p._version) for p in params))
    ent = _PACK_CACHE.get(id(model))
    if ent is not None and ent[0] == key and ent[2]() is model:
        return ent[1]
    import weakref
    with torch.no_grad():
        P = builder(model)
    _PACK_CACHE[id(model)] = (key, P, weakref.ref(model, lambda _r, k=id(model): _PACK_CACHE.pop(k, None)))
    return P


def prepare_stack_params(model):
    return cached_pack(model, _build_stack_params)


def cam_node_params(cam, pk=None):
    wd = _wd()
    own = pk is None
    pk = pk or EagerPack(cam.inter_layer.linear_p.weight.device)
    d = {}
    for tag, blk in (("p", cam.p_attention_block), ("c", cam.c_attention_block)):
        a = blk.mha
        d["Wqg_" + tag] = pk.cat([a.linear_q.weight, a.linear_g.weight], 0, wd, with_T=True)
        d["bqg_" + tag] = pk.cat([pk.zeros(a.linear_g.bias.shape[0]), a.linear_g.bias])
        d["Wkv_" + tag] = pk.cat([a.linear_k.weight, a.linear_v.weight], 0, wd, with_T=True)
        d["Wo_" + tag], d["bo_" + tag] = pk.copy(a.linear_o.weight, wd, with_T=True), pk.copy(a.linear_o.bias)
    for tag, tr in (("p", cam.p_transition), ("c", cam.c_transition)):
        d["Wt1_" + tag], d["bt1_" + tag] = pk.copy(tr.linear_1.weight, wd, with_T=True), pk.copy(tr.linear_1.bias)
        d["Wt2_" + tag], d["bt2_" + tag] = pk.copy(tr.linear_2.weight, wd, with_T=True), pk.copy(tr.linear_2.bias)
    i32 = cam.inter_layer
    zw, zb = pk.zeros(*i32.linear_p.weight.shape), pk.zeros(i32.linear_p.bias.shape[0])
    d["W_ab32"] = pk.cat([i32.linear_p.weight, zw, i32.linear_c.weight, zw], 0, wd, with_T=True)
    d["b_ab32"] = pk.cat([i32.linear_p.bias, zb, i32.linear_c.bias, zb])
    return pk.resolve(d) if own else d


def att_edge_params(m, pk=None):
    wd = _wd()
    own = pk is None
    pk = pk or EagerPack(m.linear_q.weight.device)
    d = {}
    Wkv, bkv = m.linear_kv.weight, m.linear_kv.bias
    d["Wqkv"] = pk.cat([m.linear_q.weight, Wkv[0::2, 1:], Wkv[1::2, 1:]], 0, wd, with_T=True)
    d["bqkv"] = pk.cat([m.linear_q.bias, bkv[0::2], bkv[1::2]])
    d["w_rk"], d["w_rv"] = pk.copy(Wkv[0::2, 0]), pk.copy(Wkv[1::2, 0])
# ... 409 lines not shown
        self.step = float(args.geometry_reg_step_size)
        self.clampv = 10.0 / self.scale
        self.P = prepare_stack_params(model)
        pre = _take_prefetched(X, batch_id) if _PREFETCHED else None
        self.prefetched_graph = pre[1] if pre is not None else None
        self.lay = lay = pre[0] if pre is not None else Layout.of(batch_id, segment_id)
        self.bond_row = compound_edge_index[0].to(torch.int32).contiguous()
        self.bond_col = compound_edge_index[1].to(torch.int32).contiguous()
        self.bond_off = lay.ranges(self.bond_row)
        las = (LAS_edge_index[0].to(torch.int32).contiguous(), LAS_edge_index[1].to(torch.int32).contiguous())
        self.las = las + (lay.ranges(las[0]),)
        self.x_las = coord_LAS.reshape(-1, 3).float().contiguous()
        self.mask_u8 = mask.to(torch.uint8).contiguous()
        self.Hin = Hin.float().contiguous()
        self.a0b0 = ops.shared_grad(ops.linear(self.Hin, self.P["W_ab0"], self.P["b_ab0"]))
        self.pairbias = pair_bias_all(self.P, self.a0b0, lay)
        self.cut_intra = float(model.extract_edges.intra_cutoff)
        self.cut_inter = float(model.extract_edges.inter_cutoff)
        self.drop = None
        if model.training:
            gnn = model.gnn
            drop = dict(gnn=gnn.dropout.p, gcl=gnn.gcl_0.dropout.p, att=gnn.att_0.dropout.p, out=gnn.out_layer.dropout.p,
                        row=gnn.att_0.cross_attn_module.p_attention_block.dropout.p)
            self.drop = drop if any(v > 0 for v in drop.values()) else None
        self.g = None

    def rebuild_graph(self, x, input_coords=False):
        pre, self.prefetched_graph = self.prefetched_graph, None
        if input_coords and pre is not None:
            self.g = pre
            return self.g
        self.g = Graph(self.lay, x.detach().reshape(-1, 3).float().contiguous(), self.bond_row, self.bond_col, self.bond_off,
                       self.cut_intra, self.cut_inter)
        return self.g

    def layer(self, i, h, x):
        dp = self.drop or {}
        h, x = gcl_layer(self.P["gcl"][i], h, x, self.lay, self.g, self.clampv, dp.get("gcl", 0.0))
        h, x, alpha = att_layer(self.P["att"][i], h, x, self.lay, self.g, self.a0b0, self.pairbias, i, self.clampv,
                                dp.get("att", 0.0), dp.get("row", 0.0))
        x = ops.las_step(x, self.x_las, self.las, self.lay, self.step, 15.0 / self.scale)
        return h, x, alpha

    def gnn(self, h, x):
        return egnn_forward(self.P, h, x, self.lay, self.g, self.las, self.x_las, self.a0b0, self.pairbias, self.scale,
                            self.step, self.drop)


def stack_forward(model, X, Hin, batch_id, segment_id, mask, is_global, compound_edge_index, LAS_edge_index,
                  coord_LAS, n_iter):
    ctx = StackContext(model, X, Hin, batch_id, segment_id, mask, is_global, compound_edge_index, LAS_edge_index, coord_LAS)
    x = X.reshape(-1, 3).float().contiguous()
    Hout = None
    for r in range(n_iter):
        last = r == n_iter - 1
        g = ctx.rebuild_graph(x, input_coords=(r == 0))
        with torch.set_grad_enabled(last and torch.is_grad_enabled()):
            Hout, z = ctx.gnn(ctx.Hin, x)
            x = ops.select_rows(x, z, ctx.mask_u8)
    model.last_graph = g
    with torch.no_grad():
        X.copy_(x.reshape(X.shape).to(X.dtype))
    Xout = x.reshape(X.shape)
    return (Xout if Xout.requires_grad else X), Hout


class EdgeListGraph:

    def __init__(self, edge_index, n_nodes):
        row, col = edge_index[0].long(), edge_index[1].long()
        srow, order = torch.sort(row, stable=True)
        self.row_ctx = srow.to(torch.int32).contiguous()
        self.col_ctx = col[order].to(torch.int32).contiguous()
        rp = torch.zeros(n_nodes + 1, dtype=torch.int32, device=row.device)
        rp[1:] = torch.cumsum(torch.bincount(srow, minlength=n_nodes), 0).to(torch.int32)
        self.rp_ctx, self.N, self.E_ctx, self._bycol = rp, n_nodes, int(row.shape[0]), None

    def ctx_by_col(self):
        if self._bycol is None:
            cs, perm = torch.sort(self.col_ctx.long(), stable=True)
            cp = torch.zeros(self.N + 1, dtype=torch.int32, device=perm.device)
            cp[1:] = torch.cumsum(torch.bincount(cs, minlength=self.N), 0).to(torch.int32)
            self._bycol = (cp, perm.to(torch.int32).contiguous())
        return self._bycol


class BatchOnlyLayout:

    def __init__(self, batch_id):
        B = int(batch_id[-1].item()) + 1
        off = torch.zeros(B + 1, dtype=torch.int32, device=batch_id.device)
        off[1:] = torch.cumsum(torch.bincount(batch_id, minlength=B), 0).to(torch.int32)
        self.node_off, self.B, self.N = off, B, int(batch_id.shape[0])
```

fabind_amd/kernels.py:

```python
import ctypes

import numpy as np
import torch

from . import _lib
from . import config as _cfg
from ._lib import ACT_NONE, ACT_RELU, ACT_SIGMOID, ACT_SILU, ACT_STORED_DERIV, GemmArgs, check, dt_code, ptr, stream

__all__ = ["gemm", "colsum", "edges_count", "edges_fill", "exclusive_scan", "inter_meta",
           "edge_geom", "gcl_pre", "segment_sum", "coord_update", "cross_attn_fwd", "pair_bmat", "pair_hadamard",
           "inter_attn_fwd", "las_step", "select_rows", "ACT_NONE", "ACT_SILU", "ACT_RELU", "ACT_SIGMOID", "ACT_STORED_DERIV"]

GEMM_BN = 128
GEMM_DEFAULT_CONFIG = 13
PROFILE = None
PROFILE_ONLY = None


PROFILE_BYTES = {}
PROFILE_ALGO = {}


def _profiled(label, flops, fn, nbytes=0.0, algo=None):
    if PROFILE is None or (PROFILE_ONLY is not None and not label.startswith(PROFILE_ONLY)):
# ... 110 lines not shown

def exclusive_scan(deg):
    out = torch.empty(deg.shape[0] + 1, dtype=torch.int32, device=deg.device)
    check(_lib.load().fabind_exclusive_scan(ptr(deg), ptr(out), deg.shape[0], stream()), "fabind_exclusive_scan")
    return out


def edges_fill(x, node_off, c_cnt, B, max_n, bond_row, bond_col, bond_off, cut_intra, cut_inter, rowptr_ctx, rowptr_int,
               E_ctx, E_int):
    dev = x.device
    col_ctx = torch.empty(max(E_ctx, 1), dtype=torch.int32, device=dev)
    row_ctx = torch.empty(max(E_ctx, 1), dtype=torch.int32, device=dev)
    col_int = torch.empty(max(E_int, 1), dtype=torch.int32, device=dev)
    row_int = torch.empty(max(E_int, 1), dtype=torch.int32, device=dev)
    check(_lib.load().fabind_edges_fill(ptr(x), ptr(node_off), ptr(c_cnt), B, max_n, ptr(bond_row), ptr(bond_col),
                                        ptr(bond_off), cut_intra, cut_inter, ptr(rowptr_ctx), ptr(rowptr_int),
                                        ptr(col_ctx), ptr(row_ctx), ptr(col_int), ptr(row_int), stream()),
          "fabind_edges_fill")
    return col_ctx[:E_ctx], row_ctx[:E_ctx], col_int[:E_int], row_int[:E_int]


def inter_meta(node_off, c_cnt, B, rowptr_int, col_int, row_int):
    dev = col_int.device
    E = col_int.shape[0]
    red_off = torch.empty(B + 1, dtype=torch.int32, device=dev)
    red_idx = torch.empty(max(E, 1), dtype=torch.int32, device=dev)
    n_red = E // 2
    red_c = torch.empty(max(n_red, 1), dtype=torch.int32, device=dev)
    red_p = torch.empty(max(n_red, 1), dtype=torch.int32, device=dev)
    mirror = torch.empty(max(E, 1), dtype=torch.int32, device=dev)
    check(_lib.load().fabind_inter_meta(ptr(node_off), ptr(c_cnt), B, ptr(rowptr_int), ptr(col_int), ptr(row_int), E,
                                        ptr(red_off), ptr(red_idx), ptr(red_c), ptr(red_p), ptr(mirror), stream()),
          "fabind_inter_meta")
    return red_off, red_idx[:E], red_c[:n_red], red_p[:n_red], mirror[:E]


def edge_geom(x, row, col, rowptr, node_off, B):
    E, dev = row.shape[0], x.device
    d = torch.empty((max(E, 1), 3), dtype=torch.float32, device=dev)
    rho = torch.empty(max(E, 1), dtype=torch.float32, device=dev)
    rhohat = torch.empty(max(E, 1), dtype=torch.float32, device=dev)
    norm = torch.empty(B, dtype=torch.float32, device=dev)
    check(_lib.load().fabind_edge_geom(ptr(x), ptr(row), ptr(col), ptr(rowptr), ptr(node_off), B, ptr(d), ptr(rho),
                                       ptr(rhohat), ptr(norm), stream()), "fabind_edge_geom")
    return d[:E], rho[:E], rhohat[:E], norm


def gcl_pre(AB, H, row, col, rhohat, w_r, out_dtype, act=ACT_NONE, want_dact=False):
    E = row.shape[0]
    pre = torch.empty((E, H), dtype=out_dtype, device=AB.device)
    dact = torch.empty((E, H), dtype=out_dtype, device=AB.device) if want_dact else None
    check(_lib.load().fabind_gcl_pre(ptr(AB), dt_code(AB.dtype), _ld(AB), H, ptr(row), ptr(col), ptr(rhohat), ptr(w_r), ptr(pre),
                                     dt_code(out_dtype), E, act, ptr(dact), stream()), "fabind_gcl_pre")
    return (pre, dact) if want_dact else pre


def layernorm_rows(x, w, b, out_dtype, pad_to=None, eps=1e-5):
    R, C = x.shape
    pad_to = pad_to or C
    y = torch.empty((R, pad_to), dtype=out_dtype, device=x.device)
    check(_lib.load().fabind_layernorm_rows(ptr(x), dt_code(x.dtype), _ld(x), ptr(w), ptr(b), eps, R, C, ptr(y),
                                            dt_code(out_dtype), pad_to, pad_to, stream()), "fabind_layernorm_rows")
    return y


def edge_ln_concat(h, row, col, rhohat, w, b, out_dtype, pad_to, eps=1e-5):
    E, H = row.shape[0], h.shape[1]
    y = torch.empty((E, pad_to), dtype=out_dtype, device=h.device)
    check(_lib.load().fabind_edge_ln_concat(ptr(h), _ld(h), H, ptr(row), ptr(col), ptr(rhohat), ptr(w), ptr(b), eps, E, ptr(y),
                                            dt_code(out_dtype), pad_to, pad_to, stream()), "fabind_edge_ln_concat")
    return y


def segment_sum(Z, rowptr, n_rows, act=ACT_NONE, eidx=None, out=None, out16=None):
    H = Z.shape[1]
    if out is None and out16 is None:
        out = torch.empty((n_rows, H), dtype=torch.float32, device=Z.device)
    check(_lib.load().fabind_segment_sum(ptr(Z), dt_code(Z.dtype), _ld(Z), H, ptr(rowptr), ptr(eidx), n_rows,
                                         Z.shape[0] if eidx is None else eidx.numel(), act, ptr(out), _ld(out) if out is not None else 0,
                                         ptr(out16), _ld(out16) if out16 is not None else 0, stream()), "fabind_segment_sum")
    return out if out is not None else out16


def coord_update(x, d, s_part, rowptr, mean, clampv, weight=None, want_s=False):
    n_rows = x.shape[0]
    x_out = torch.empty_like(x)
    s_out = torch.empty(s_part.shape[0], dtype=torch.float32, device=x.device) if want_s else None
    check(_lib.load().fabind_coord_update(ptr(x), ptr(d), ptr(s_part), s_part.shape[1], ptr(weight), ptr(rowptr), n_rows,
                                          1 if mean else 0, clampv, ptr(x_out), ptr(s_out), stream()), "fabind_coord_update")
    return x_out, s_out


CROSS_ATTN_MFMA = None


def cross_attn_use_mfma():
    from .config import get_precision
    return (get_precision() == "bf16") if CROSS_ATTN_MFMA is None else bool(CROSS_ATTN_MFMA)


def cross_attn_fwd(q, k, v, gpre, bias, lin_col, gate_col, desc, B, max_nq, scale, out, want_lse=False, max_nk=0):
    lse = torch.empty((q.shape[0], 4), dtype=torch.float32, device=q.device) if want_lse else None
    assert k.stride(0) == v.stride(0)
    ksplit = max(1, min(32, max_nk // 128)) if (max_nq <= 256 and max_nk >= 512) else 1
    part = torch.empty(q.shape[0] * ksplit * 4 * 34, dtype=torch.float32, device=q.device) if ksplit > 1 else None
    mfma = cross_attn_use_mfma()
    fn = _lib.load().fabind_cross_attn_mfma_fwd if mfma else _lib.load().fabind_cross_attn_fwd
    n_tiles = sum(1 for _ in range(0, max_nq, 16))
    flops = 2.0 * 16 * 16 * 32 * 16 * n_tiles * ((max_nk + 31) // 32) * B if mfma else 0.0
    _profiled("cross_attn_%s_fwd B=%d nq<=%d nk<=%d" % ("mfma" if mfma else "fp32", B, max_nq, max_nk), flops,
              lambda: check(fn(ptr(q), _ld(q), ptr(k), ptr(v), _ld(k), ptr(gpre), _ld(gpre), ptr(bias), _ld(bias), lin_col, gate_col,
                               ptr(desc), B, max_nq, scale, ptr(out), _ld(out), ptr(lse), ksplit, ptr(part), q.shape[0], stream()),
                            "fabind_cross_attn_fwd"))
    return out, lse


CROSS_ATTN_FUSED_MAX_C = 62


def bo_tiles(lay):
    c = getattr(lay, "_bo_tiles", None)
    if c is None:
        import numpy as np
        T = (np.asarray(lay.C) + 1) // 2
        toff = np.concatenate([[0], np.cumsum(T)]).astype(np.int32)
        tile_b = np.repeat(np.arange(lay.B, dtype=np.int32), T)
        dev = lay.node_off.device
        from .param_pack import upload
        c = lay._bo_tiles = (upload(toff, dev, torch.int32), upload(tile_b, dev, torch.int32), int(toff[-1]))
    return c


def pair_bo_pack(b0, wcomp, H, lay):
    toff, tile_b, n_tiles = bo_tiles(lay)
    wc = wcomp.reshape(-1, 8, wcomp.shape[-1]).float().contiguous()
    nblk = wc.shape[0]
    per = max(n_tiles, 1) * (H // 32) * 512
    out = torch.empty((nblk, per), dtype=torch.bfloat16, device=b0.device)
    check(_lib.load().fabind_pair_bo_pack(ptr(b0), _ld(b0), ptr(wc), H, ptr(lay.c_index), ptr(lay.desc_pf), ptr(toff), ptr(tile_b),
                                          n_tiles, ptr(out), nblk, per, stream()), "fabind_pair_bo_pack")
    return [out[k] for k in range(nblk)]


def cross_attn_fused_fwd(q, k, v, gpre, a0_16, bo, bconst8, lay, H, mode, scale, out, lse=None):
    toff, _, _ = bo_tiles(lay)
    nsplit = (lay.max_P + 63) // 64
    part = torch.empty(lay.sumC * nsplit * 4 * 34, dtype=torch.float32, device=q.device) if mode == 1 else None
    assert k.stride(0) == v.stride(0) and a0_16.dtype == torch.bfloat16
    n_wg = nsplit * lay.B
    flops = 2.0 * n_wg * 64 * (((lay.max_C + 1) // 2 + 3) // 4 * 4 * 16) * H + 2.0 * 16 * 16 * 32 * 16 * n_wg * 4 * ((lay.max_C if mode == 0 else 64) + 31) // 32
    _profiled("cross_attn_fused_fwd mode=%d B=%d P<=%d C<=%d (bias contraction K=%d + attention)" % (mode, lay.B, lay.max_P, lay.max_C, H), flops,
              lambda: check(_lib.load().fabind_cross_attn_fused_fwd(ptr(q), _ld(q), ptr(k), ptr(v), _ld(k), ptr(gpre), _ld(gpre), ptr(a0_16),
                                                                    _ld(a0_16), ptr(bo), ptr(toff), ptr(bconst8), ptr(lay.desc_pf), lay.B,
                                                                    lay.max_P, lay.max_C, H, mode, scale, ptr(out), _ld(out), ptr(part),
                                                                    lay.sumC, ptr(lse), stream()), "fabind_cross_attn_fused_fwd"))
    return out


def bot_ksteps(lay):
    c = getattr(lay, "_bot_ksteps", None)
    if c is None:
        KS = (np.asarray(lay.C) + 3) // 4
        koff = np.concatenate([[0], np.cumsum(KS)]).astype(np.int32)
        kstep_b = np.repeat(np.arange(lay.B, dtype=np.int32), KS)
        dev = lay.node_off.device
        from .param_pack import upload
# ... 321 lines not shown
    part = torch.empty((nb, 4 * Kp), dtype=torch.float32, device=dev)
    assert AB16.dtype == torch.bfloat16 and out.dtype == torch.bfloat16 and dout.dtype == torch.bfloat16 and dout.is_contiguous() and out.is_contiguous()
    check(lib.fabind_edge_lnfold_bwd(ptr(AB16), _ld(AB16), Kp, H, ptr(row), ptr(col), ptr(rho), ptr(stat), float(eps), ptr(w_r), ptr(c_r),
                                     ptr(c_c), ptr(out), ptr(dout), E, float(p_drop), ptr(du), ptr(es), ptr(drho), ptr(part), nb,
                                     stream()), "fabind_edge_lnfold_bwd")
    return du[:E], es[:E], drho[:E], colsum(part).view(4, Kp)


def inter_coord_fold(P16, H, col, rho, stat, q_w, eps, u, d, w3, p_drop=0.0, seed=0):
    E = col.shape[0]
    out = torch.empty(max(E, 1), dtype=torch.float32, device=P16.device)
    assert P16.dtype == torch.bfloat16 and stat.dtype == torch.float32 and stat.is_contiguous()
    check(_lib.load().fabind_inter_coord_fold(ptr(P16), _ld(P16), H, ptr(col), ptr(rho), ptr(stat), float(q_w), float(eps),
                                              ptr(u), ptr(d), ptr(w3), E, ptr(out), float(p_drop), int(seed) & 0xFFFFFFFF,
                                              stream()), "fabind_inter_coord_fold")
    return out[:E]


def row_stats(x, eps):
    R, C = x.shape
    mu = torch.empty(max(R, 1), dtype=torch.float32, device=x.device)
    rs = torch.empty(max(R, 1), dtype=torch.float32, device=x.device)
    check(_lib.load().fabind_row_stats(ptr(x), dt_code(x.dtype), _ld(x), float(eps), R, C, ptr(mu), ptr(rs), stream()),
          "fabind_row_stats")
    return mu, rs


def layernorm_rows_form(x, out, C=None, pad_to=None):
    C = x.shape[1] if C is None else C
    pad_to = out.shape[1] if pad_to is None else pad_to
    return int(_lib.load().fabind_layernorm_rows_form(ptr(x), _ld(x), C, ptr(out), _ld(out), pad_to))


def layernorm_rows_bwd_form(x, dy, dx, C=None):
    C = x.shape[1] if C is None else C
    return int(_lib.load().fabind_layernorm_rows_bwd_form(ptr(x), _ld(x), ptr(dy), _ld(dy), ptr(dx), _ld(dx), C))


def row_stats_form(x):
    return int(_lib.load().fabind_row_stats_form(ptr(x), dt_code(x.dtype), _ld(x), x.shape[1]))


def edge_lnfold_form(Kp, H):
    u = ctypes.c_int(0)
    lib = _lib.load()
    return int(lib.fabind_edge_lnfold_form(Kp, H, ctypes.byref(u))), u.value, int(lib.fabind_edge_lnfold_blocks(2 ** 31 - 1))


def edge_lnfold_bwd_form(Kp):
    u = ctypes.c_int(0)
    lib = _lib.load()
    return int(lib.fabind_edge_lnfold_bwd_form(Kp, ctypes.byref(u))), u.value, int(lib.fabind_edge_lnfold_bwd_blocks(2 ** 31 - 1))


def inter_coord_fold_blocks(E=2 ** 31 - 1):
    return int(_lib.load().fabind_inter_coord_fold_blocks(E))


def pair_update_fused(T, b_off, p_node, c_node, z, Wop, bo, ln_w, ln_b, eps, W1p, b1, W2p, b2, Wbp=None, bb=None, p_drop=0.0,
                      seed=0):
    n, H = z.shape
    assert z.dtype == torch.bfloat16 and z.is_contiguous() and T.dtype == torch.float32
    z_out = torch.empty_like(z)
    bias_out = torch.empty((max(n, 1), 16), dtype=torch.float32, device=z.device) if Wbp is not None else None
    a = _lib.PairUpdateArgs()
    for name, t in (("T", T), ("p_node", p_node), ("c_node", c_node), ("z_in", z), ("z_out", z_out), ("Wop", Wop), ("bo", bo),
                    ("ln_w", ln_w), ("ln_b", ln_b), ("W1p", W1p), ("b1", b1), ("W2p", W2p), ("b2", b2), ("Wbp", Wbp), ("bb", bb),
                    ("bias_out", bias_out)):
        setattr(a, name, ptr(t))
    a.ldt, a.b_off, a.n_pairs = _ld(T), int(b_off), n
    a.eps, a.p_drop, a.seed = float(eps), float(p_drop), int(seed) & 0xFFFFFFFF
    _profiled("pair_update_fused_kernel<%d> pairs=%d (Hadamard + LN + 2 chained H x H contractions + 16 biases)" % (H, n),
              2.0 * n * H * (2 * H + 32 + 16),
              lambda: check(_lib.load().fabind_pair_update_fused(ctypes.byref(a), H, stream()), "fabind_pair_update_fused"))
    return z_out, (bias_out[:n] if bias_out is not None else None)


_N_CU = {}
EDGE_BWD_GROUPS = 0
EDGE_BWD_TIMES = None


def gcl_edge_fused_bwd(AB16, H, row, col, rhohat, w_r, W2, b2, Wc, bc, w3, ds, dagg, colptr, perm, p_drop=0.0, seed=0,
                       dab_bf16=False, w_dtype=torch.float32, rowptr=None, frags=None, saved=None):
    E, N, dev = row.shape[0], AB16.shape[0], AB16.device
    ng = _N_CU.get(dev)
    if ng is None:
        ng = _N_CU[dev] = torch.cuda.get_device_properties(dev).multi_processor_count
    lib = _lib.load()
    variant = lib.fabind_gcl_edge_fused_bwd_variant_for(H)
    if saved is not None and E > 0:
        variant = 6
    bm = 64
    if variant == 6:
        per_cu = max(1, min(8, (160 * 1024) // (2 * bm * H + 16 * H + 32 * bm), 16 // max(1, H // 64)))
    elif variant == 5:
        per_cu = max(1, min(8, (160 * 1024) // (4 * bm * H + 16 * H + 32 * bm), 12 // (H // 64 + 1)))
    else:
        per_cu = max(1, min(8, (160 * 1024) // (4 * bm * H + 1024), 512 // H))
    ng = max(1, min(ng * per_cu, (E + bm - 1) // bm))
    if EDGE_BWD_GROUPS:
        ng = int(EDGE_BWD_GROUPS)
    if ng >= 8:
        ng -= ng % 8
    d2scratch = torch.empty((2, ng, bm * H), dtype=torch.bfloat16, device=dev) if variant == 5 else None
    bnd = torch.empty(((E + bm - 1) // bm * 2 + 2, H), dtype=torch.float32, device=dev)
    if variant == 6:
        buf = torch.empty((4, max(E, 1), H), dtype=torch.bfloat16, device=dev)
        S1, Mm, dT, dP2, dP1 = buf[0], saved[0], buf[1], buf[2], buf[3]
    else:
        buf = torch.empty((5, max(E, 1), H), dtype=torch.bfloat16, device=dev)
        S1, Mm, dT, dP2, dP1 = buf[0], buf[1], buf[2], buf[3], buf[4]
    dab_bf16 = bool(dab_bf16) and variant in (5, 6)
    dAB = (torch.zeros if (rowptr is None or E == 0) else torch.empty)((N, 2 * H), dtype=torch.bfloat16 if dab_bf16 else torch.float32, device=dev)
    if rowptr is not None and E > 0:
        zero_empty_rows(rowptr, dAB, H)
    drh = torch.empty(max(E, 1), dtype=torch.float32, device=dev)
    part = torch.zeros((ng, 4, H), dtype=torch.float32, device=dev)
    dagg = dagg.contiguous()
    ds = ds.contiguous()
    a = _lib.EdgeBwdArgs()
    W2p, Wcp, W2Tp, WcTp = frags if (frags is not None and len(frags) == 4) else (pack_frag(W2), pack_frag(Wc), pack_frag(W2.t()), pack_frag(Wc.t()))
    keep = (W2p, Wcp, W2Tp, WcTp)
    for name, t in (("AB", AB16), ("row", row), ("col", col), ("rhohat", rhohat), ("w_r", w_r), ("W2p", W2p), ("Wcp", Wcp),
                    ("W2Tp", W2Tp), ("WcTp", WcTp), ("b2", b2), ("bc", bc), ("w3", w3), ("ds", ds), ("dagg", dagg),
                    ("S1", S1), ("Mm", Mm), ("dT", dT), ("dP2", dP2), ("dP1", dP1), ("drh", drh),
                    ("dABrow", None if dab_bf16 else dAB), ("dAB16", dAB if dab_bf16 else None),
                    ("part", part), ("d2scratch", d2scratch), ("bnd", bnd)):
        setattr(a, name, ptr(t))
    a.ldab, a.lddagg, a.lddab, a.E = _ld(AB16), _ld(dagg), _ld(dAB), E
    a.lddab16 = _ld(dAB)
    a.p_drop, a.seed = float(p_drop), int(seed) & 0xFFFFFFFF
    a.dbg = ptr(EDGE_BWD_TIMES) if (EDGE_BWD_TIMES is not None and variant != 6) else None
    if variant == 6:
        a.d2f, a.z3f = ptr(saved[1]), ptr(saved[2])
    _profiled(("gcl_edge_fused_bwd4_kernel<%d> E=%d (2 chained H x H contractions per edge over the forward's saved tiles)" % (H, E)) if variant == 6 else
              "gcl_edge_fused_bwd%s_kernel<%d> E=%d (recompute + 4 chained H x H contractions per edge)" % ("3" if variant == 5 else "", H, E),
              (4.0 if variant == 6 else 8.0) * E * H * H,
              lambda: check(_lib.load().fabind_gcl_edge_fused_bwd(ctypes.byref(a), H, ng, stream()),
                            "fabind_gcl_edge_fused_bwd"),
              E * ((12.0 if variant == 6 else 10.0) * H + 20) + N * (4.0 * H + 4.0 * H + (2.0 if dab_bf16 else 4.0) * H),
              algo=N * (2.0 * H * 2 + 4.0 * H + 2.0 * H * (2.0 if dab_bf16 else 4.0)) + E * 20.0)
    del keep
    if E > 0:
        if dab_bf16:
            segment_sum(dP1[:E], colptr, N, eidx=perm, out16=dAB[:, H:])
        else:
            segment_sum(dP1[:E], colptr, N, eidx=perm, out=dAB[:, H:])
        if tn_can_queue(dP2[:E], S1[:E], W2.data_ptr()) and tn_can_queue(dT[:E], Mm[:E], Wc.data_ptr()):
            dW2, dWc = torch.empty((H, H), dtype=w_dtype, device=dev), torch.empty((H, H), dtype=w_dtype, device=dev)
            gemm_tn_queued(dP2[:E], S1[:E], dW2, key=W2.data_ptr())
            gemm_tn_queued(dT[:E], Mm[:E], dWc, key=Wc.data_ptr())
        else:
            TN_STATS["direct"] += 2
            dW2 = gemm_tn(dP2[:E], S1[:E], out_dtype=w_dtype)
            dWc = gemm_tn(dT[:E], Mm[:E], out_dtype=w_dtype)
    else:
        dW2 = torch.zeros((H, H), dtype=w_dtype, device=dev)
        dWc = torch.zeros((H, H), dtype=w_dtype, device=dev)
    ps = part.sum(0)
    out = (dAB, drh[:E], ps[3], dW2, ps[0], dWc, ps[1], ps[2])
    return out


_ZERO_PAGE = {}


_TN_SPLITS = {}


def _tn_splits(M, N, E, tn):
    key = (M, N, E, tn)
    s = _TN_SPLITS.get(key)
    if s is not None:
        return s
    if tn != 256:
        tiles = ((M + 255) // 256) * ((N + 127) // 128)
        s = max(1, min(256, max(E // 2048, min(E // 256, 16)), max(1, 1024 // tiles)))
    elif E < 4096:
        s = max(1, min(16, E // 256))
    else:
        tiles = ((M + 255) // 256) * ((N + 255) // 256)
        best = None
        for c in range(8, 257, 8):
            if E // c < 256:
                break
            rounds = -(-(tiles * c // 8) // 32)
            cost = rounds * (-(-E // c) / 32.0 * 0.45 + 3.0) + c * M * N * 8 / 3e6
            if best is None or cost < best[0]:
                best = (cost, c)
        s = best[1] if best else 8
    _TN_SPLITS[key] = s
    return s


TN_DEFER = _cfg.knob("FABIND_TN_DEFER")
TN_DEFER_JOB_BYTES = 1024 << 20
TN_DEFER_QUEUE_BYTES = 6144 << 20
_TNQ = {"jobs": [], "bytes": 0, "armed": False, "outs": set()}
_TNJOB = np.dtype([(n_, np.uint64) for n_ in ("Y", "X", "C_part", "out", "out_tail")] +
                  [(n_, np.int32) for n_ in ("ldy", "ldx", "M", "N", "E", "splits", "e_per", "n_tiles", "with_colsum", "out_dt", "ldo",
                                             "wg0", "n_wg", "blk0", "n_blk", "pad_")])
TN_STATS = {"queued": 0, "flushes": 0, "direct": 0}


def tn_pending():
    return len(_TNQ["jobs"])


def _tn_multi_splits(E):
    return max(8, min(64, (E // 4096 + 7) // 8 * 8))


def gemm_tn_queued(Y, X, out, out_tail=None, key=None):
    E, M = Y.shape
    N = X.shape[1]
    nb = (Y.numel() + X.numel()) * 2
    q = _TNQ
    q["jobs"].append((Y, X, out, out_tail, M, N, E))
    q["bytes"] += nb
    if key is not None:
        q["outs"].add(key)
    TN_STATS["queued"] += 1
    if q["bytes"] > TN_DEFER_QUEUE_BYTES:
        tn_flush()


def _tn_end_of_backward():
    _TNQ["armed"] = False
    tn_flush()

# ... 142 lines not shown
```

fabind_amd/ops.py:

```python
import ctypes

import numpy as np
import torch

from . import config as _cfg
from . import kernels as K
from ._lib import GemmArgs, check, dt_code, load, ptr, stream


def act_dtype():
    return torch.float32 if _cfg.fp32_storage() else torch.bfloat16


mm_dtype = act_dtype


def needs_grad(*ts):
    return torch.is_grad_enabled() and any(torch.is_tensor(t) and t.requires_grad for t in ts)


_needs_grad = needs_grad


def _nchunk(rows):
# ... 527 lines not shown
        dx = K.gemm(dz, _wt(ctx.Wt, W), out_dtype=x.dtype)[0] if ni[0] else None
        dW, db = _param_grads(dz, x, None, W, ni[1], ni[2])
        return dx, dW, db, (du / ctx.scale if ni[3] else None), None, None


def linear_rowdot(x, W, b, u, act_pro=K.ACT_NONE, act_epi=K.ACT_NONE, p_drop=0.0, fold=None):
    if _needs_grad(x, W, b, u):
        assert fold is None, "the LayerNorm fold has no autograd path"
        K.tn_hook(W, b)
        if p_drop > 0.0:
            assert act_pro == K.ACT_NONE and act_epi == K.ACT_RELU, "epilogue dropout under autograd: ReLU outputs only"
            assert b is not None, "linear_rowdot with epilogue dropout under autograd needs a bias"
            return _LinearRowdotDrop.apply(x, W, b, u, p_drop, _drop_seed(p_drop))
        return _LinearRowdot.apply(x, W, b, u, act_pro, act_epi)
    return _gemm_rowdot(x, W, b, u, act_pro, act_epi, store=False, p_drop=p_drop, seed=_drop_seed(p_drop), fold=fold)[1]


class _EdgeTail(torch.autograd.Function):
    @staticmethod
    def forward(ctx, Mm, Wc, bc, w3, rowptr, row, n_rows, act_epi):
        z, part = _gemm_rowdot(Mm, Wc, bc, w3, K.ACT_NONE, act_epi, store=True)
        agg = K.segment_sum(Mm, rowptr, n_rows)
        ctx.act_epi, ctx.Wt = act_epi, _stored_wt(Wc)
        ctx.save_for_backward(Mm, Wc, w3, z, row)
        return part, agg

    @staticmethod
    def backward(ctx, dpart, dagg):
        Mm, Wc, w3, z, row = ctx.saved_tensors
        M, N = z.shape
        if dpart is None:
            dpart = torch.zeros((M, (N + K.GEMM_BN - 1) // K.GEMM_BN), dtype=torch.float32, device=z.device)
        dz, du = _rowdot_bwd(z, dpart.contiguous(), w3, ctx.act_epi)
        Wt = _wt(ctx.Wt, Wc)
        if dagg is not None:
            dM, _ = K.gemm(dz, Wt, residual=dagg.contiguous(), r_index=row, out_dtype=Mm.dtype)
        else:
            dM, _ = K.gemm(dz, Wt, out_dtype=Mm.dtype)
        dW, dbc = _param_grads(dz, Mm, None, Wc, True, True)
        return dM, dW, dbc, du, None, None, None, None


def edge_tail(Mm, Wc, bc, w3, rowptr, row, n_rows, act_epi=K.ACT_SILU):
    if _needs_grad(Mm, Wc, bc, w3):
        K.tn_hook(Wc, bc)
        return _EdgeTail.apply(Mm, Wc, bc, w3, rowptr, row, n_rows, act_epi)
    part = _gemm_rowdot(Mm, Wc, bc, w3, K.ACT_NONE, act_epi, store=False)[1]
    return part, K.segment_sum(Mm, rowptr, n_rows)


EDGE_SAVE_FWD = _cfg.knob("FABIND_EDGE_SAVE_FWD")
EDGE_SAVE_MIN_H = 256


class _FusedEdge(torch.autograd.Function):

    @staticmethod
    def forward(ctx, AB16, rhohat, w_r, W2, b2, Wc, bc, w3, H, g, p_drop, seed, holder=None, frags=None):
        ctx.H, ctx.g, ctx.p_drop, ctx.seed, ctx.frags = H, g, p_drop, seed, frags
        W2p, Wcp = (frags[0], frags[1]) if frags is not None else (K.pack_frag(W2), K.pack_frag(Wc))
        E = g.row_ctx.shape[0]
        save = EDGE_SAVE_FWD and H >= EDGE_SAVE_MIN_H and E >= 1 and AB16.dtype == torch.bfloat16
        out = K.gcl_edge_fused(AB16, H, g.row_ctx, g.col_ctx, rhohat, w_r, W2p, b2, Wcp, bc, w3,
                               AB16.shape[0], p_drop, seed, want16=holder is not None, rowptr=g.rp_ctx, save=save)
        ctx.n_saved = 3 if save else 0
        ctx.save_for_backward(AB16, rhohat, w_r, W2, b2, Wc, bc, w3, *(out[-1] if save else ()))
        if holder is not None:
            holder.append(out[2])
        return out[0], out[1]

    @staticmethod
    def backward(ctx, dagg, ds):
        AB16, rhohat, w_r, W2, b2, Wc, bc, w3 = ctx.saved_tensors[:8]
        saved = tuple(ctx.saved_tensors[8:]) if ctx.n_saved else None
        g = ctx.g
        colptr, perm = g.ctx_by_col()
        if dagg is None:
            dagg = torch.zeros((AB16.shape[0], ctx.H), dtype=torch.float32, device=AB16.device)
        if ds is None:
            ds = torch.zeros(g.row_ctx.shape[0], dtype=torch.float32, device=AB16.device)
        dAB, drh, dwr, dW2, db2, dWc, dbc, dw3 = K.gcl_edge_fused_bwd(
            AB16, ctx.H, g.row_ctx, g.col_ctx, rhohat, w_r, W2, b2, Wc, bc, w3, ds.reshape(-1).float(), dagg.float(),
            colptr, perm, ctx.p_drop, ctx.seed, dab_bf16=AB16.dtype == torch.bfloat16, w_dtype=W2.dtype, rowptr=g.rp_ctx, frags=ctx.frags,
            saved=saved)
        return (dAB.to(AB16.dtype), drh, dwr, dW2.to(W2.dtype), db2, dWc.to(Wc.dtype), dbc, dw3, None, None, None, None, None, None)


class _FusedEdgeX3(torch.autograd.Function):

    @staticmethod
    def forward(ctx, AB, rhohat, w_r, W2, b2, Wc, bc, w3, H, g, p_drop, seed):
        ctx.H, ctx.g, ctx.p_drop, ctx.seed = H, g, p_drop, seed
        E = g.row_ctx.shape[0]
        save = EDGE_SAVE_FWD and H >= EDGE_SAVE_MIN_H and E >= 1
        out = K.gcl_edge_fused_x3(AB, H, g.row_ctx, g.col_ctx, rhohat, w_r, W2, b2, Wc, bc, w3, AB.shape[0], p_drop, seed,
                                  rowptr=g.rp_ctx, save=save)
        ctx.n_saved = 3 if save else 0
        ctx.save_for_backward(AB, rhohat, w_r, W2, b2, Wc, bc, w3, *(out[2] if save else ()))
        return out[0], out[1]

    @staticmethod
    def backward(ctx, dagg, ds):
        AB, rhohat, w_r, W2, b2, Wc, bc, w3 = ctx.saved_tensors[:8]
        saved = tuple(ctx.saved_tensors[8:]) if ctx.n_saved else None
        g = ctx.g
        colptr, perm = g.ctx_by_col()
        if dagg is None:
            dagg = torch.zeros((AB.shape[0], ctx.H), dtype=torch.float32, device=AB.device)
        if ds is None:
            ds = torch.zeros(g.row_ctx.shape[0], dtype=torch.float32, device=AB.device)
        dAB, drh, dwr, dW2, db2, dWc, dbc, dw3 = K.gcl_edge_fused_bwd(
            AB.to(torch.bfloat16), ctx.H, g.row_ctx, g.col_ctx, rhohat, w_r, W2, b2, Wc, bc, w3, ds.reshape(-1).float(), dagg.float(),
            colptr, perm, ctx.p_drop, ctx.seed, dab_bf16=False, w_dtype=torch.float32, rowptr=g.rp_ctx, saved=saved)
        return (dAB, drh, dwr, dW2, db2, dWc, dbc, dw3, None, None, None, None)


def fused_edge(AB16, rhohat, w_r, W2, b2, Wc, bc, w3, H, g, p_drop=0.0, frags=None):
    seed = _drop_seed(p_drop)
    if _needs_grad(AB16, rhohat, w_r, W2, b2, Wc, bc, w3):
        K.tn_hook(W2, Wc)
    if _cfg.get_precision() == "bf16x3" and _cfg.x3_edge_bf16() and AB16.dtype == torch.float32:
        ab = AB16.to(torch.bfloat16)
        if _needs_grad(AB16, rhohat, w_r, W2, b2, Wc, bc, w3):
            agg, s = _FusedEdge.apply(ab, rhohat, w_r, W2, b2, Wc, bc, w3, H, g, p_drop, seed, None, None)
            return agg, s
        out = K.gcl_edge_fused(ab, H, g.row_ctx, g.col_ctx, rhohat, w_r, K.pack_frag(W2), b2, K.pack_frag(Wc), bc, w3, ab.shape[0], p_drop, seed,
                               want16=False, rowptr=g.rp_ctx)
        return out[0], out[1]
    if _cfg.get_precision() == "bf16x3":
        if _needs_grad(AB16, rhohat, w_r, W2, b2, Wc, bc, w3):
            return _FusedEdgeX3.apply(AB16, rhohat, w_r, W2, b2, Wc, bc, w3, H, g, p_drop, seed)
        return K.gcl_edge_fused_x3(AB16, H, g.row_ctx, g.col_ctx, rhohat, w_r, W2, b2, Wc, bc, w3, AB16.shape[0], p_drop, seed,
                                   rowptr=g.rp_ctx)
    w16 = _cfg.get_precision() == "bf16"
    if _needs_grad(AB16, rhohat, w_r, W2, b2, Wc, bc, w3):
        holder = [] if w16 else None
        agg, s = _FusedEdge.apply(AB16, rhohat, w_r, W2, b2, Wc, bc, w3, H, g, p_drop, seed, holder, frags)
        return _attach_b16(agg, holder[0] if holder else None), s
    W2p, Wcp = (frags[0], frags[1]) if frags is not None else (K.pack_frag(W2), K.pack_frag(Wc))
    out = K.gcl_edge_fused(AB16, H, g.row_ctx, g.col_ctx, rhohat, w_r, W2p, b2, Wcp, bc, w3,
                           AB16.shape[0], p_drop, seed, want16=w16, rowptr=g.rp_ctx)
    return (_attach_b16(out[0], out[2]), out[1]) if w16 else out


class _EdgeGeom(torch.autograd.Function):
    @staticmethod
    def forward(ctx, x, row, col, rowptr, lay, bycol):
        d, rho, rhohat, norm = K.edge_geom(x, row, col, rowptr, lay.node_off, lay.B)
        ctx.lay, ctx.n, ctx.bycol = lay, x.shape[0], bycol
        ctx.save_for_backward(row, col, rowptr, d, rho, norm)
        return d, rhohat

    @staticmethod
    def backward(ctx, dd, drhohat):
        row, col, rowptr, d, rho, norm = ctx.saved_tensors
        lay, E, dev = ctx.lay, row.shape[0], d.device
        if ctx.bycol is not None:
            colptr, perm = ctx.bycol()
        else:
            colsorted, perm64 = torch.sort(col.long(), stable=True)
            colptr = torch.zeros(ctx.n + 1, dtype=torch.int32, device=dev)
            colptr[1:] = torch.cumsum(torch.bincount(colsorted, minlength=ctx.n), 0).to(torch.int32)
            perm = perm64.to(torch.int32)
        dx = torch.empty((ctx.n, 3), dtype=torch.float32, device=dev)
        dd = dd.contiguous() if dd is not None else torch.zeros_like(d)
        drhohat = drhohat.contiguous() if drhohat is not None else torch.zeros_like(rho)
        gbuf = torch.empty((max(E, 1), 3), dtype=torch.float32, device=dev)
        check(load().fabind_edge_geom_bwd(ptr(d), ptr(rho), ptr(norm), ptr(dd), ptr(drhohat), ptr(row), ptr(rowptr),
                                          ptr(colptr), ptr(perm), ptr(lay.node_off), lay.B, E, ctx.n, ptr(dx), ptr(gbuf),
                                          ptr(torch.empty(lay.B, dtype=torch.float32, device=dev)), stream()),
              "fabind_edge_geom_bwd")
        return dx, None, None, None, None, None


def edge_geom(x, row, col, rowptr, lay, bycol=None):
    if _needs_grad(x):
        return _EdgeGeom.apply(x, row, col, rowptr, lay, bycol)
    d, _, rhohat, _ = K.edge_geom(x, row, col, rowptr, lay.node_off, lay.B)
    return d, rhohat


class _GclPre(torch.autograd.Function):
    @staticmethod
    def forward(ctx, AB, rhohat, w_r, H, g, act):
        ctx.H, ctx.g, ctx.act = H, g, act
        if act == K.ACT_NONE:
            out, D = K.gcl_pre(AB, H, g.row_ctx, g.col_ctx, rhohat, w_r, act_dtype()), None
        else:
            out, D = K.gcl_pre(AB, H, g.row_ctx, g.col_ctx, rhohat, w_r, act_dtype(), act, want_dact=True)
        ctx.save_for_backward(AB, rhohat, w_r, D)
        return out

    @staticmethod
    def backward(ctx, dout):
        AB, rhohat, w_r, D = ctx.saved_tensors
        H, g = ctx.H, ctx.g
# ... 1190 lines not shown
```

include/fabind_hip.h:

```cpp
#ifndef FABIND_HIP_H
#define FABIND_HIP_H

#include <stdint.h>

#ifdef __cplusplus
extern "C" {
#endif

#ifndef __HIP_PLATFORM_AMD__
typedef struct ihipStream_t* hipStream_t;
#endif

const char* fabind_last_error(void);
#define FABIND_ABI_VERSION 19
int fabind_abi_version(void);
int fabind_sizeof_args(int which);

typedef struct FabindGemmArgs {
    const void* A;
    const void* A2;
    const void* W;
    void* C;
    const float* bias;
    const void* R;
// ... 25 lines not shown

int fabind_gemm(const FabindGemmArgs* args, hipStream_t stream);

#define FB_GEMM_FAM_NT_F32 0
#define FB_GEMM_FAM_NT_F32_BF16 1
#define FB_GEMM_FAM_NT_BF16 2
#define FB_GEMM_FAM_GLDS 3
#define FB_GEMM_FAM_PIPE 4
#define FB_GEMM_FAM_X3 5
#define FB_GEMM_FAM_X3_PRO 6
#define FB_GEMM_FAM_PERSIST 7
int fabind_gemm_plan(const FabindGemmArgs* args, int* family, int* epi_fast, int* cfg);

int fabind_gemm_tn(const void* Y, int ldy, const void* X, int ldx, float* C_part, int M, int N, int E, int splits,
                   const void* zero_page, const int* groups, int n_groups, int with_colsum, hipStream_t stream);

typedef struct FabindTnJob {
    const void* Y; const void* X; float* C_part; void* out; float* out_tail;
    int ldy, ldx, M, N, E, splits, e_per, n_tiles, with_colsum, out_dt, ldo;
    int wg0, n_wg, blk0, n_blk, pad_;
} FabindTnJob;
int fabind_gemm_tn_multi(const FabindTnJob* jobs_dev, const FabindTnJob* jobs_host, int n_jobs, const int* wg_job_dev, int total_wg,
                         const int* blk_job_dev, int total_blk, const void* zero_page, hipStream_t stream);

int fabind_transpose_act(const void* in, int in_dt, int ldi, void* out, int out_dt, int ldo, int R, int C, int act,
                         hipStream_t stream);
typedef struct FabindCopySeg {
    const void* src;
    void* dst;
    long long src_sr, src_sc, dst_sr, dst_sc;
    int rows, cols;
    int src_dt, dst_dt;
    int vec4, pad_;
} FabindCopySeg;
int fabind_multi_copy(const FabindCopySeg* segs_dev, int n_segs, int blocks_per_seg, hipStream_t stream);
typedef struct FabindAdamRow {
    float* p;
    const float* g;
    float* m;
    float* v;
    long long numel;
    int chunk0, step_idx;
    double lr, beta1, beta2, eps, weight_decay;
    int decoupled, pad_;
} FabindAdamRow;
int fabind_adam_chunk(void);
int fabind_multi_sqnorm(const FabindAdamRow* rows_dev, int n_rows, int n_chunks, const float* steps, float* partials, float* snap,
                        hipStream_t stream);
int fabind_multi_adam(const FabindAdamRow* rows_dev, int n_rows, int n_chunks, const float* partials, const float* snap, float* steps,
                      float max_norm, int flags, float* grad_norm, int* skipped, hipStream_t stream);
typedef struct FabindPackSeg {
    const void* src;
    void* dst;
    long long src_sr, src_sc;
    int N, K, src_dt, pad_;
} FabindPackSeg;
int fabind_pack_frag_multi(const FabindPackSeg* segs_dev, const FabindPackSeg* segs_host, int n_segs, hipStream_t stream);
int fabind_split_sum(const float* part, int splits, long n, void* out, int out_dt, long n_tail, float* out_tail, hipStream_t stream);
int fabind_colsum(const void* in, int in_dt, int ldi, float* out, int R, int C, int accumulate, float* scratch,
                  int nchunk, hipStream_t stream);

int fabind_edges_count(const float* x, const int* node_off, const int* c_cnt, int B, int max_n, const int* bond_row,
                       const int* bond_off, float cut_intra, float cut_inter, int* deg_ctx, int* deg_int,
                       hipStream_t stream);
int fabind_edges_fill(const float* x, const int* node_off, const int* c_cnt, int B, int max_n, const int* bond_row,
                      const int* bond_col, const int* bond_off, float cut_intra, float cut_inter,
                      const int* rowptr_ctx, const int* rowptr_int, int* col_ctx, int* row_ctx, int* col_int,
                      int* row_int, hipStream_t stream);
int fabind_exclusive_scan(const int* in, int* out, int n, hipStream_t stream);
int fabind_lower_bound(const int* vals, int n, const int* keys, int n_keys, int* out, hipStream_t stream);
int fabind_inter_meta(const int* node_off, const int* c_cnt, int B, const int* rowptr_int, const int* col_int,
                      const int* row_int, int E_int, int* red_off, int* red_idx, int* red_c, int* red_p, int* mirror,
                      hipStream_t stream);

int fabind_edge_geom(const float* x, const int* row, const int* col, const int* rowptr, const int* node_off, int B,
                     float* d, float* rho, float* rhohat, float* norm, hipStream_t stream);

int fabind_gcl_pre(const void* AB, int ab_dt, int ldab, int H, const int* row, const int* col, const float* rhohat,
                   const float* w_r, void* pre, int pre_dt, int E, int act, void* dact_out, hipStream_t stream);
int fabind_segment_sum(const void* Z, int z_dt, int ldz, int H, const int* rowptr, const int* eidx, int n_rows, int n_edges,
                       int act, float* out, int ldo,
                       void* out16 , int ldo16,
                       hipStream_t stream);
int fabind_zero_empty_rows(const int* rowptr, int n_rows, void* out, int out_dt, int ld, int C, void* out2, int out2_dt, int ld2,
                           hipStream_t stream);
int fabind_coord_update(const float* x, const float* d, const float* s_part, int n_part, const float* weight,
                        const int* rowptr, int n_rows, int mean, float clampv, float* x_out, float* s_out,
                        hipStream_t stream);

int fabind_gcl_edge_fused_x3(const float* AB, int ldab, int n_rows, int H, const int* row, const int* col, const float* rhohat,
                             const float* w_r, const void* W2ph, const void* W2pl, const float* b2, const void* Wcph,
                             const void* Wcpl, const float* bc, const float* w3, int E, float* agg, float* s_out, float p_drop,
                             unsigned seed, float* bnd, hipStream_t stream);
int fabind_gcl_edge_fused_x3_train(const float* AB, int ldab, int n_rows, int H, const int* row, const int* col, const float* rhohat,
                                   const float* w_r, const void* W2ph, const void* W2pl, const float* b2, const void* Wcph,
                                   const void* Wcpl, const float* bc, const float* w3, int E, float* agg, float* s_out, float p_drop,
                                   unsigned seed, float* bnd, void* M, void* d2f, void* z3f, hipStream_t stream);

int fabind_gcl_edge_fused(const void* AB, int ldab, int H, const int* row, const int* col, const float* rhohat,
                          const float* w_r, const void* W2p, const float* b2, const void* Wcp, const float* bc,
                          const float* w3, int E, float* agg, float* s_out, float p_drop, unsigned seed,
                          float* bnd ,
                          void* agg16 ,
                          hipStream_t stream);

int fabind_gcl_edge_fused_train(const void* AB, int ldab, int H, const int* row, const int* col, const float* rhohat,
                                const float* w_r, const void* W2p, const float* b2, const void* Wcp, const float* bc,
                                const float* w3, int E, float* agg, float* s_out, float p_drop, unsigned seed, float* bnd,
                                void* agg16, void* M, void* d2f, void* z3f, hipStream_t stream);

typedef struct FabindEdgeBwdArgs {
    const void* AB; const int* row; const int* col; const float* rhohat; const float* w_r;
    const void* W2p; const void* Wcp; const void* W2Tp; const void* WcTp;
    const float* b2; const float* bc; const float* w3; const float* ds; const float* dagg;
    void* S1; void* Mm; void* dT; void* dP2; void* dP1;
    float* drh; float* dABrow; float* part;
    void* dbg;
    float* bnd;
    void* d2scratch;
    int ldab, lddagg, lddab, E;
    float p_drop;
    unsigned seed;
    int xcd_aware;
    int lddab16;
    void* dAB16;
    const void* d2f;
    const void* z3f;
} FabindEdgeBwdArgs;
int fabind_gcl_edge_fused_bwd(const FabindEdgeBwdArgs* args, int H, int n_groups, hipStream_t stream);
int fabind_gcl_edge_fused_bwd_set_tile(int bm);
int fabind_gcl_edge_fused_bwd_tile(void);
int fabind_gcl_edge_fused_bwd_set_variant(int v);
int fabind_gcl_edge_fused_bwd_variant(void);
int fabind_gcl_edge_fused_bwd_variant_for(int H);
void fabind_gcl_edge_fused_bwd3_set_exp(int mask);
void fabind_gcl_edge_fused_bwd4_set_exp(int mask);
void fabind_gcl_edge_fused_set_xcd_aware(int on);
int fabind_gcl_edge_fused_set_variant(int v);
int fabind_gcl_edge_fused_variant(void);

typedef struct FabindPairUpdateArgs {
    const float* T; const int* p_node; const int* c_node;
    const void* z_in; void* z_out;
    const void* Wop; const float* bo; const float* ln_w; const float* ln_b;
    const void* W1p; const float* b1; const void* W2p; const float* b2;
    const void* Wbp; const float* bb; float* bias_out;
    int ldt, b_off, n_pairs;
    float eps, p_drop;
    unsigned seed;
} FabindPairUpdateArgs;
int fabind_pair_update_fused(const FabindPairUpdateArgs* args, int H, hipStream_t stream);

int fabind_post_optimize(const float* x0, const float* ref, const int* atom_off, const int* nbr_ptr, const int* nbr_idx,
                         int n_ligands, int max_atoms, int all_pairs, int steps, float lr, float* x_out, float* loss_out,
                         float* rmsd_out, hipStream_t stream);

int fabind_sym_automorphisms(const int* labels, const int* nbr_ptr, const int* nbr_idx, const int* atom_off, int n_ligands, int cap,
                             int max_steps, const int* flat_off, int* scratch, int* flat, int* count, int* status, hipStream_t stream);
int fabind_sym_score(const float* pred, int n_pose, int n_atoms, const float* ref, const int* atom_off, const int* flat_off,
                     const int* auto_cnt, const int* flat, int n_ligands, int max_atoms, float* min_rmsd, int* arg_rmsd, float* min_sl1,
                     int* arg_sl1, int* best_idx, hipStream_t stream);
int fabind_pose_stats(const float* pred, const float* truth, const int* atom_off, int B, float* rmsd, float* cdis, hipStream_t stream);
int fabind_rank_loss_fwd(const float* scores, const float* rmsd, const int* group_off, int G, int mode, int with_ce, float* terms,
                         float* d_scores, int* counts, hipStream_t stream);

int fabind_cross_attn_fwd(const float* q, int ldq, const float* k, const float* v, int ldkv, const float* gpre,
                          int ldg, const float* bias, int bias_ld, int lin_col, int gate_col, const int* desc, int B,
                          int max_nq, float scale, float* out, int ldo, float* lse, int ksplit, float* part, int n_rows,
                          hipStream_t stream);

int fabind_cross_attn_fused_fwd(const float* q, int ldq, const float* k, const float* v, int ldkv, const float* gpre, int ldg,
                                const void* a0, int lda0, const void* bo, const int* toff, const float* bconst, const int* desc, int B,
                                int max_P, int max_C, int H, int mode, float scale, float* out, int ldo, float* part, int n_lig_rows,
                                float* lse, hipStream_t stream);
int fabind_pair_bo_pack(const float* b0, int ldb, const float* wcomp, int H, const int* c_index, const int* desc, const int* toff,
                        const int* tile_b, int n_tiles, void* out, int n_blocks, long blk_stride, hipStream_t stream);

typedef struct FabindAttnFusedBwdArgs {
    const float* qg; const float* kv; const void* a0; const void* bo; const void* boT; const int* toff; const int* koff;
    const float* bconst; const int* desc; const int* desc_p; const float* out; const float* lse; const float* dout;
    float* dqg; float* dkv; float* dO; float* Dv; float* da0; void* acat; float* colpart; float* part;
    int ldq, ldkv, lda0, ldda0, ldacat, kcol0, ldcolpart, kp;
    float scale;
    int nsplit, B, part_rows;
} FabindAttnFusedBwdArgs;
int fabind_cross_attn_fused_bwd(const FabindAttnFusedBwdArgs* args, int B, int max_P, int max_C, int H, int mode, int n_lig_rows,
                                hipStream_t stream);
long fabind_cross_attn_fused_bwd_scratch(int B, int max_P, int max_C, int n_lig_rows, int mode);
int fabind_cross_attn_fused_bwd_parts(int B, int max_P);
int fabind_pair_bot_pack(const float* b0, int ldb, const float* wcomp, int H, const int* c_index, const int* desc, const int* koff,
                         const int* kstep_b, int n_ksteps, void* out, int n_blocks, long blk_stride, hipStream_t stream);

int fabind_cross_attn_mfma_fwd(const float* q, int ldq, const float* k, const float* v, int ldkv, const float* gpre, int ldg,
                               const float* bias, int bias_ld, int lin_col, int gate_col, const int* desc, int B, int max_nq,
                               float scale, float* out, int ldo, float* lse, int ksplit, float* part, int n_rows,
                               hipStream_t stream);

int fabind_pair_bmat(const float* b0, int ldb, const float* wcomp, int NO, int H, const int* c_node, int n_c,
                     void* bmat, int bmat_dt, hipStream_t stream);
int fabind_pair_hadamard(const float* a0, const float* b0, int ld0, int H, const float* a1, const float* b1, int ld1,
                         int H2, const int* red_p, const int* red_c, int n_red, void* hd, int hd_dt, int ldh,
                         hipStream_t stream);

int fabind_inter_attn_fwd(const float* qkv, int ldqkv, const float* cv, int ldcv, int H, const float* h, int ldh,
                          const float* x, const float* d, const float* rhohat, const int* rowptr, const int* col,
                          const int* red_idx, const float* bias_red, int bias_np, const float* w_rk,
                          const float* w_rv, const float* wcr, const float* w3, float clampv, int n_rows,
                          float* h_out, float* x_out, float* alpha, float* cvs,
                          const float* s_ext ,
                          void* h16 ,
                          hipStream_t stream);
int fabind_inter_attn_fwd_rows(const float* qkv, int ldqkv, const float* cv, int ldcv, int H, const float* h, int ldh,
// ... 209 lines not shown
```

Measured before the change: 521.3.

## Scatter edge-backward dP1 into column-sorted slots and segment-sum contiguously

The edge backward kernels now write each edge's dP1 row to a slot given by the inverse column permutation, so the gradient rows land already grouped by receiving node. A new sorted segment-sum kernel then reduces these contiguous runs with boundary fix-up, replacing the gather through perm in the old segment sum. This trades contiguous writes in the edge kernel for scattered writes, in exchange for streaming reads in the reduction. Adds a cached slot/colsorted index build per graph and a 4 GiB size guard.

New measurement: 517.1. No clear change (-0.8%).

```diff
diff --git a/fabind_amd/_lib.py b/fabind_amd/_lib.py
--- a/fabind_amd/_lib.py
+++ b/fabind_amd/_lib.py
@@ -80,6 +80,7 @@
     "fabind_gcl_edge_fused_x3": [_vp, _i, _i, _i, _vp, _vp, _vp, _vp, _vp, _vp, _vp, _vp, _vp, _vp, _vp, _i, _vp, _vp, _f, ctypes.c_uint, _vp, _vp],
     "fabind_gcl_edge_fused_x3_train": [_vp, _i, _i, _i, _vp, _vp, _vp, _vp, _vp, _vp, _vp, _vp, _vp, _vp, _vp, _i, _vp, _vp, _f, ctypes.c_uint, _vp, _vp, _vp, _vp, _vp],
     "fabind_gcl_edge_fused_bwd": [ctypes.POINTER(EdgeBwdArgs), _i, _i, _vp],
+    "fabind_gcl_edge_fused_bwd_slot": [ctypes.POINTER(EdgeBwdArgs), _i, _i, _vp, _vp],
     "fabind_pair_update_fused": [ctypes.POINTER(PairUpdateArgs), _i, _vp],
     "fabind_gcl_edge_fused_bwd_set_tile": [_i],
     "fabind_gcl_edge_fused_bwd_tile": [],
@@ -114,6 +115,7 @@
     "fabind_zero_empty_rows": [_vp, _i, _vp, _i, _i, _i, _vp, _i, _i, _vp],
     "fabind_split_sum": [_vp, _i, ctypes.c_long, _vp, _i, ctypes.c_long, _vp, _vp],
     "fabind_segment_sum": [_vp, _i, _i, _i, _vp, _vp, _i, _i, _i, _vp, _i, _vp, _i, _vp],
+    "fabind_segment_sum_sorted": [_vp, _i, _i, _vp, _vp, _i, _i, _vp, _i, _vp, _i, _vp, _vp],
     "fabind_coord_update": [_vp, _vp, _vp, _i, _vp, _vp, _i, _i, _f, _vp, _vp, _vp],
     "fabind_cross_attn_fwd": [_vp, _i, _vp, _vp, _i, _vp, _i, _vp, _i, _i, _i, _vp, _i, _i, _f, _vp, _i, _vp, _i, _vp, _i,
                               _vp],
diff --git a/fabind_amd/csrc/fused_common.h b/fabind_amd/csrc/fused_common.h
--- a/fabind_amd/csrc/fused_common.h
+++ b/fabind_amd/csrc/fused_common.h
@@ -231,6 +231,15 @@
     for (unsigned q = tid; q < (unsigned)ne * CH; q += H) {
         const unsigned rw = q / CH, ch = q % CH;
         *(uint4*)&gt[rw * H + ch * 8] = *(const uint4*)&sB[rw * H + ((ch ^ (rw & 7)) * 8)];
+    }
+}
+
+template <int H>
+__device__ __forceinline__ void fe_tile_store_slot(const bf16_t* sB, bf16_t* __restrict__ g, const int* __restrict__ slot, int ne, int tid) {
+    constexpr int CH = H / 8;
+    for (unsigned q = tid; q < (unsigned)ne * CH; q += H) {
+        const unsigned rw = q / CH, ch = q % CH;
+        *(uint4*)&g[(size_t)slot[rw] * H + ch * 8] = *(const uint4*)&sB[rw * H + ((ch ^ (rw & 7)) * 8)];
     }
 }
 
@@ -395,7 +404,7 @@
 }
 
 struct FabindEdgeBwdArgs;
-int fe_bwd3_launch(const FabindEdgeBwdArgs* a, int H, int bm, int n_groups, hipStream_t stream);
+int fe_bwd3_launch(const FabindEdgeBwdArgs* a, int H, int bm, int n_groups, hipStream_t stream, const int* dp1_slot = nullptr);
 int fe_fwd3_launch(const float* AB, int ldab, int H, const int* row, const int* col, const float* rhohat, const float* w_r,
                    const void* W2ph, const void* W2pl, const float* b2, const void* Wcph, const void* Wcpl, const float* bc,
                    const float* w3, int E, float* agg, float* s_out, uint32_t thr16, float dscale, unsigned seed, float* bnd,
@@ -404,4 +413,4 @@
                    const void* W2p, const float* b2, const void* Wcp, const float* bc, const float* w3, int E, float* agg,
                    float* s_out, uint32_t thr16, float dscale, unsigned seed, float* bnd, void* agg16, int xcd_aware, hipStream_t stream,
                    void* Msave = nullptr, void* d2f = nullptr, void* z3f = nullptr);
-int fe_bwd4_launch(const FabindEdgeBwdArgs* a, int H, int n_groups, hipStream_t stream);
+int fe_bwd4_launch(const FabindEdgeBwdArgs* a, int H, int n_groups, hipStream_t stream, const int* dp1_slot = nullptr);
diff --git a/fabind_amd/csrc/fused_edge.hip b/fabind_amd/csrc/fused_edge.hip
--- a/fabind_amd/csrc/fused_edge.hip
+++ b/fabind_amd/csrc/fused_edge.hip
@@ -89,7 +89,7 @@
 }
 
 template <int H, int BM, bool DBG>
-__global__ __launch_bounds__(H, (BM == 32 ? 4 : 2)) void gcl_edge_fused_bwd_kernel(const FabindEdgeBwdArgs p) {
+__global__ __launch_bounds__(H, (BM == 32 ? 4 : 2)) void gcl_edge_fused_bwd_kernel(const FabindEdgeBwdArgs p, const int* __restrict__ dp1_slot) {
     constexpr int TPE = H / BM;
     constexpr int CPT = BM / 8;
     constexpr int MI = BM / 16;
@@ -362,7 +362,8 @@
         fe_prefetch(ur, uc);
         __syncthreads();
         FE_TICK(8)
-        fe_tile_store<H>(sX, (bf16_t*)p.dP1, e0, ne, tid);
+        if (dp1_slot) fe_tile_store_slot<H>(sX, (bf16_t*)p.dP1, dp1_slot + e0, ne, tid);
+        else fe_tile_store<H>(sX, (bf16_t*)p.dP1, e0, ne, tid);
         FE_TICK(1)
 
         {
@@ -424,6 +425,10 @@
 }
 
 extern "C" int fabind_gcl_edge_fused_bwd(const FabindEdgeBwdArgs* a_in, int H, int n_groups, hipStream_t stream) {
+    return fabind_gcl_edge_fused_bwd_slot(a_in, H, n_groups, nullptr, stream);
+}
+
+extern "C" int fabind_gcl_edge_fused_bwd_slot(const FabindEdgeBwdArgs* a_in, int H, int n_groups, const int* dp1_slot, hipStream_t stream) {
     FabindEdgeBwdArgs a_copy = *a_in;
     a_copy.xcd_aware = g_fe_xcd_aware;
     const FabindEdgeBwdArgs* a = &a_copy;
@@ -431,12 +436,13 @@
     FB_REQUIRE(H == 512 || H == 256 || H == 128 || H == 64, "fabind_gcl_edge_fused_bwd: H must be 64, 128, 256 or 512");
     FB_REQUIRE(a->ldab % 8 == 0, "fabind_gcl_edge_fused_bwd: ldab % 8");
     FB_REQUIRE(a->p_drop >= 0.f && a->p_drop < 1.f, "fabind_gcl_edge_fused_bwd: p_drop in [0, 1)");
+    FB_REQUIRE(dp1_slot == nullptr || (unsigned long long)a->E * H * 2 < (1ull << 32), "fabind_gcl_edge_fused_bwd_slot: E * H * 2 must stay below 4 GiB");
     const int g_fe_bwd_variant = fabind_gcl_edge_fused_bwd_variant_for(H);
     if (a->d2f != nullptr || a->z3f != nullptr) {
         FB_REQUIRE(a->d2f != nullptr && a->z3f != nullptr, "fabind_gcl_edge_fused_bwd: d2f and z3f (saved by fabind_gcl_edge_fused_train) come together");
-        return fe_bwd4_launch(a, H, n_groups, stream);
-    }
-    if (g_fe_bwd_variant == 5) return fe_bwd3_launch(a, H, 64, n_groups, stream);
+        return fe_bwd4_launch(a, H, n_groups, stream, dp1_slot);
+    }
+    if (g_fe_bwd_variant == 5) return fe_bwd3_launch(a, H, 64, n_groups, stream, dp1_slot);
     FB_REQUIRE(a->dAB16 == nullptr, "fabind_gcl_edge_fused_bwd: dAB16 (bf16 receiving-side sums) exists in variant 5 only");
     FB_REQUIRE(a->bnd != nullptr, "fabind_gcl_edge_fused_bwd: bnd (ceil(E / tile) x 2 x H floats of scratch) is required");
     const int BMr = g_fe_bwd_bm;
@@ -445,13 +451,13 @@
     do {                                                                                                           \
         static bool set_ = false;                                                                                  \
         if (!set_) { (void)hipFuncSetAttribute((const void*)gcl_edge_fused_bwd_kernel<HH, BB, false>, hipFuncAttributeMaxDynamicSharedMemorySize, (int)lds); set_ = true; } \
-        hipLaunchKernelGGL((gcl_edge_fused_bwd_kernel<HH, BB, false>), dim3(n_groups), dim3(HH), lds, stream, *a);  \
+        hipLaunchKernelGGL((gcl_edge_fused_bwd_kernel<HH, BB, false>), dim3(n_groups), dim3(HH), lds, stream, *a, dp1_slot);  \
     } while (0)
 #define FE_LAUNCH(HH) FE_LAUNCH2(HH, 64)
     if (a->dbg != nullptr && H == 512) {
         static bool setd_ = false;
         if (!setd_) { (void)hipFuncSetAttribute((const void*)gcl_edge_fused_bwd_kernel<512, 64, true>, hipFuncAttributeMaxDynamicSharedMemorySize, (int)lds); }
-        hipLaunchKernelGGL((gcl_edge_fused_bwd_kernel<512, 64, true>), dim3(n_groups), dim3(512), lds, stream, *a);
+        hipLaunchKernelGGL((gcl_edge_fused_bwd_kernel<512, 64, true>), dim3(n_groups), dim3(512), lds, stream, *a, dp1_slot);
     } else
     if (H == 512) FE_LAUNCH(512); else if (H == 256) FE_LAUNCH(256); else if (H == 128) FE_LAUNCH(128); else FE_LAUNCH(64);
     hipLaunchKernelGGL((fe_boundary_fix_kernel<64>), dim3((a->E + 63) / 64), dim3(H < 256 ? H : 256), 0, stream, a->row, a->E, H,
diff --git a/fabind_amd/csrc/fused_edge_bwd3.hip b/fabind_amd/csrc/fused_edge_bwd3.hip
--- a/fabind_amd/csrc/fused_edge_bwd3.hip
+++ b/fabind_amd/csrc/fused_edge_bwd3.hip
@@ -30,8 +30,21 @@
     }
 }
 
+template <int H, int SWZ>
+__device__ __forceinline__ void fe3_wave_store_slot(const bf16_t* sB, bf16_t* __restrict__ g, int e_tot, const int* __restrict__ slot, int ne, int lane) {
+    constexpr int CH = H / 8;
+    const __amdgpu_buffer_rsrc_t rs = fe_rsrc(g, (unsigned)e_tot * H * 2);
+    const unsigned total = (unsigned)ne * CH;
+#pragma unroll 8
+    for (unsigned q = lane; q < total; q += 64) {
+        const unsigned rw = q / CH, ch = q % CH;
+        const uint4 v = *(const uint4*)&sB[rw * H + ((ch ^ (rw & SWZ)) * 8)];
+        __builtin_amdgcn_raw_buffer_store_b128(fe_u32x4_t{v.x, v.y, v.z, v.w}, rs, (int)(((unsigned)slot[rw] * H + ch * 8) * 2), 0,  2);
+    }
+}
+
 template <int H, int BM, bool DROP, bool DBG>
-__global__ __launch_bounds__(H + 64) void gcl_edge_fused_bwd3_kernel(const FabindEdgeBwdArgs p, const int xf) {
+__global__ __launch_bounds__(H + 64) void gcl_edge_fused_bwd3_kernel(const FabindEdgeBwdArgs p, const int xf, const int* __restrict__ dp1_slot) {
     constexpr int MI = BM / 16;
     constexpr int NW = H / 64;
     constexpr int CH = H / 8;
@@ -83,7 +96,9 @@
             __syncthreads();
             __syncthreads();
             __syncthreads();
-            if (st) put((bf16_t*)p.dP1);
+            if (st) {
+                if (dp1_slot) fe3_wave_store_slot<H, SWZ>(sX, (bf16_t*)p.dP1, p.E, dp1_slot + e0, ne, lane); else put((bf16_t*)p.dP1);
+            }
             __syncthreads();
         }
         __syncthreads();
@@ -407,7 +422,7 @@
 static int g_fe_bwd3_exp = 0;
 extern "C" void fabind_gcl_edge_fused_bwd3_set_exp(int m) { g_fe_bwd3_exp = m; }
 
-int fe_bwd3_launch(const FabindEdgeBwdArgs* a, int H, int bm, int n_groups, hipStream_t stream) {
+int fe_bwd3_launch(const FabindEdgeBwdArgs* a, int H, int bm, int n_groups, hipStream_t stream, const int* dp1_slot) {
     FB_REQUIRE(a->d2scratch != nullptr, "fabind_gcl_edge_fused_bwd: the store-wave form needs d2scratch (n_groups x 64 x H x 2 bytes)");
     FB_REQUIRE(a->bnd != nullptr, "fabind_gcl_edge_fused_bwd: bnd (ceil(E / tile) x 2 x H floats of scratch) is required");
     FB_REQUIRE(a->lddagg % 4 == 0 && ((uintptr_t)a->dagg & 15) == 0, "fabind_gcl_edge_fused_bwd: dagg must be 16-byte aligned with lddagg % 4 == 0");
@@ -421,7 +436,7 @@
             if (e_ != hipSuccess) { fabind_set_error(hipGetErrorString(e_)); return (int)e_; }                     \
             set_ = true;                                                                                           \
         }                                                                                                          \
-        hipLaunchKernelGGL((gcl_edge_fused_bwd3_kernel<HH, BB, KK, DD>), dim3(n_groups), dim3(HH + 64), lds, stream, *a, g_fe_bwd3_exp); \
+        hipLaunchKernelGGL((gcl_edge_fused_bwd3_kernel<HH, BB, KK, DD>), dim3(n_groups), dim3(HH + 64), lds, stream, *a, g_fe_bwd3_exp, dp1_slot); \
     } while (0)
 #define FE_LAUNCH3(HH, BB, DD) do { if (a->p_drop > 0.f) FE_LAUNCH3_(HH, BB, true, DD); else FE_LAUNCH3_(HH, BB, false, DD); } while (0)
     FB_REQUIRE(bm == 64, "fabind_gcl_edge_fused_bwd: the store-wave form has 64-edge tiles");
diff --git a/fabind_amd/csrc/fused_edge_bwd4.hip b/fabind_amd/csrc/fused_edge_bwd4.hip
--- a/fabind_amd/csrc/fused_edge_bwd4.hip
+++ b/fabind_amd/csrc/fused_edge_bwd4.hip
@@ -22,8 +22,20 @@
 __device__ __forceinline__ uint2 fe4_ldq(const bf16_t* p_) { return *(const uint2*)p_; }
 #endif
 
+#ifndef FE4_NT_DAGG
+#define FE4_NT_DAGG 0
+#endif
+#ifndef FE4_NT_AROW
+#define FE4_NT_AROW 0
+#endif
+template <bool NT>
+__device__ __forceinline__ uint4 fe4_bload16(const __amdgpu_buffer_rsrc_t rs, const unsigned voff, const unsigned soff) {
+    const fe_u32x4_t v = __builtin_amdgcn_raw_buffer_load_b128(rs, (int)voff, (int)soff, NT ?  2 : 0);
+    return make_uint4(v.x, v.y, v.z, v.w);
+}
+
 template <int H>
-__global__ __launch_bounds__(H, 4) void gcl_edge_fused_bwd4_kernel(const FabindEdgeBwdArgs p, const int xf) {
+__global__ __launch_bounds__(H, 4) void gcl_edge_fused_bwd4_kernel(const FabindEdgeBwdArgs p, const int xf, const int* __restrict__ dp1_slot) {
     constexpr int BM = FE_BM, MI = BM / 16;
     constexpr int NW = H / 64;
     constexpr int CH = H / 8;
@@ -181,7 +193,7 @@
             auto fetch_block = [&](int j, int slot) {
 #pragma unroll
                 for (int i = 0; i < MI; ++i) {
-                    const uint4 v = fe3_bload16(rs_dagg, dgo[i], (unsigned)(j * 64));
+                    const uint4 v = fe4_bload16<FE4_NT_DAGG != 0>(rs_dagg, dgo[i], (unsigned)(j * 64));
                     dg[slot][i] = make_float4(__uint_as_float(v.x), __uint_as_float(v.y), __uint_as_float(v.z), __uint_as_float(v.w));
                     dq[slot][i] = fe4_ldq(&d2f[FE_FOFF(i, j)]);
                 }
@@ -235,17 +247,20 @@
                 wv2[0] = fe_f2{w0.x, w0.y}; wv2[1] = fe_f2{w0.z, w0.w}; wv2[2] = fe_f2{w1.x, w1.y}; wv2[3] = fe_f2{w1.z, w1.w};
             }
             const __amdgpu_buffer_rsrc_t rs_s1 = fe_rsrc((bf16_t*)p.S1 + (size_t)e0 * H, (unsigned)ne * H * 2);
-            const __amdgpu_buffer_rsrc_t rs_p1 = fe_rsrc((bf16_t*)p.dP1 + (size_t)e0 * H, (unsigned)ne * H * 2);
+            const __amdgpu_buffer_rsrc_t rs_p1 = dp1_slot ? fe_rsrc(p.dP1, (unsigned)p.E * H * 2)
+                                                          : fe_rsrc((bf16_t*)p.dP1 + (size_t)e0 * H, (unsigned)ne * H * 2);
             constexpr int PB = (NIT % FE4_P5_BATCH == 0) ? FE4_P5_BATCH : NIT;
 #pragma unroll
             for (int u0 = 0; u0 < NIT; u0 += PB) {
             uint4 ga[PB], gb[PB];
+            int sl[PB];
 #pragma unroll
             for (int v = 0; v < PB; ++v) {
                 const int e = (u0 + v) * EPI + es_;
                 const unsigned r = (unsigned)max(sRow[e], 0), c = (unsigned)sCol[e];
-                ga[v] = fe3_bload16(rs_ab, (r * uld + ch * 8) * 2, 0);
+                ga[v] = fe4_bload16<FE4_NT_AROW != 0>(rs_ab, (r * uld + ch * 8) * 2, 0);
                 gb[v] = fe3_bload16(rs_ab, (c * uld + H + ch * 8) * 2, 0);
+                sl[v] = dp1_slot ? (dp1_slot + e0)[min(e, ne - 1)] : e;
             }
 #pragma unroll
             for (int v = 0; v < PB; ++v) {
@@ -272,7 +287,8 @@
                 const unsigned goff = (unsigned)(e * H + ch * 8) * 2;
                 if (!(xf & 2)) {
                     __builtin_amdgcn_raw_buffer_store_b128(fe_u32x4_t{po[0], po[1], po[2], po[3]}, rs_s1, (int)goff, 0,  2);
-                    __builtin_amdgcn_raw_buffer_store_b128(fe_u32x4_t{pg[0], pg[1], pg[2], pg[3]}, rs_p1, (int)goff, 0,  2);
+                    if (!dp1_slot || e < ne)
+                        __builtin_amdgcn_raw_buffer_store_b128(fe_u32x4_t{pg[0], pg[1], pg[2], pg[3]}, rs_p1, (int)((unsigned)(sl[u] * H + ch * 8) * 2), 0,  2);
                 }
                 float dot = dot2.x + dot2.y;
                 if constexpr (CH >= 16) {
@@ -316,7 +332,7 @@
 static int g_fe_bwd4_exp = 0;
 extern "C" void fabind_gcl_edge_fused_bwd4_set_exp(int m) { g_fe_bwd4_exp = m; }
 
-int fe_bwd4_launch(const FabindEdgeBwdArgs* a, int H, int n_groups, hipStream_t stream) {
+int fe_bwd4_launch(const FabindEdgeBwdArgs* a, int H, int n_groups, hipStream_t stream, const int* dp1_slot) {
     FB_REQUIRE(a->bnd != nullptr, "fabind_gcl_edge_fused_bwd: bnd (ceil(E / 64) x 2 x H floats of scratch) is required");
     FB_REQUIRE(a->lddagg % 4 == 0 && ((uintptr_t)a->dagg & 15) == 0, "fabind_gcl_edge_fused_bwd: dagg must be 16-byte aligned with lddagg % 4 == 0");
     const size_t lds = (size_t)FE_BM * H * 2 + (size_t)8 * FE_BM * sizeof(int) + (size_t)4 * H * sizeof(float);
@@ -329,7 +345,7 @@
             if (e_ != hipSuccess) { fabind_set_error(hipGetErrorString(e_)); return (int)e_; }                     \
             set_ = true;                                                                                           \
         }                                                                                                          \
-        hipLaunchKernelGGL((gcl_edge_fused_bwd4_kernel<HH>), dim3(n_groups), dim3(HH), lds, stream, *a, g_fe_bwd4_exp); \
+        hipLaunchKernelGGL((gcl_edge_fused_bwd4_kernel<HH>), dim3(n_groups), dim3(HH), lds, stream, *a, g_fe_bwd4_exp, dp1_slot); \
     } while (0)
     if (H == 512) FE_LAUNCH4(512); else if (H == 256) FE_LAUNCH4(256); else if (H == 128) FE_LAUNCH4(128); else FE_LAUNCH4(64);
 #undef FE_LAUNCH4
diff --git a/fabind_amd/csrc/gcl.hip b/fabind_amd/csrc/gcl.hip
--- a/fabind_amd/csrc/gcl.hip
+++ b/fabind_amd/csrc/gcl.hip
@@ -289,6 +289,122 @@
     return 0;
 }
 
+typedef unsigned ss_u32x4_nt_t __attribute__((ext_vector_type(4)));
+template <int LPR>
+__global__ __launch_bounds__(256) void segment_sum_sorted_kernel(const bf16_t* __restrict__ Z, int ldz, const int* __restrict__ seg,
+                                                                 int E, float* out, int ldo, bf16_t* out16, int ldo16,
+                                                                 float* __restrict__ bnd) {
+    constexpr int H = LPR * 8, G = 64 / LPR, R = 64;
+    constexpr int NB = 4 * G * R;
+    __shared__ int sId[NB + 2];
+    const long long base = (long long)blockIdx.x * NB;
+    for (int i = threadIdx.x; i < NB + 2; i += 256) {
+        const long long r = base - 1 + i;
+        sId[i] = (r >= 0 && r < E) ? seg[r] : -1;
+    }
+    __syncthreads();
+    const int lane = threadIdx.x & 63, wave = threadIdx.x >> 6;
+    const int lc = wave * G + lane / LPR, c = (lane % LPR) * 8;
+    const long long r0 = base + (long long)lc * R;
+    if (r0 >= E) return;
+    const int nr = (int)(E - r0 < R ? E - r0 : R);
+    const int* id = sId + 1 + lc * R;
+    const bool head_cont = id[-1] == id[0], tail_cont = id[nr] == id[nr - 1];
+    const bf16_t* zp = Z + (size_t)r0 * ldz + c;
+    float* bt = bnd + (size_t)(r0 / R) * 2 * H + c;
+    F8 acc;
+#pragma unroll
+    for (int k = 0; k < 8; ++k) acc.v[k] = 0.f;
+    auto put = [&](int node) {
+        if (out) st8_any(out, FB_DT_F32, (size_t)node * ldo + c, acc);
+        if (out16) st8_any(out16, FB_DT_BF16, (size_t)node * ldo16 + c, acc);
+    };
+    int cur = id[0];
+    bool first = true;
+    for (int rw0 = 0; rw0 < nr; rw0 += 8) {
+        ss_u32x4_nt_t v[8];
+        int rr[8];
+#pragma unroll
+        for (int u = 0; u < 8; ++u) {
+            const int rw = min(rw0 + u, nr - 1);
+            v[u] = __builtin_nontemporal_load((const ss_u32x4_nt_t*)(zp + (size_t)rw * ldz));
+            rr[u] = id[rw];
+        }
+#pragma unroll
+        for (int u = 0; u < 8; ++u) {
+            if (rw0 + u < nr) {
+                if (rr[u] != cur) {
+                    if (first && head_cont) st8_any(bt, FB_DT_F32, 0, acc); else put(cur);
+#pragma unroll
+                    for (int k = 0; k < 8; ++k) acc.v[k] = 0.f;
+                    cur = rr[u]; first = false;
+                }
+                const unsigned w[4] = {v[u].x, v[u].y, v[u].z, v[u].w};
+#pragma unroll
+                for (int k = 0; k < 4; ++k) {
+                    acc.v[2 * k] += __uint_as_float(w[k] << 16);
+                    acc.v[2 * k + 1] += __uint_as_float(w[k] & 0xffff0000u);
+                }
+            }
+        }
+    }
+    if (first && head_cont) st8_any(bt, FB_DT_F32, 0, acc);
+    else if (tail_cont) st8_any(bt, FB_DT_F32, H, acc);
+    else put(cur);
+}
+
+__global__ void segment_sum_sorted_fix_kernel(const int* __restrict__ seg, int E, int H, const float* __restrict__ bnd, float* out,
+                                              int ldo, bf16_t* out16, int ldo16) {
+    constexpr int R = 64;
+    const long long e0 = (long long)blockIdx.x * R;
+    if (e0 + R >= E) return;
+    const int r = seg[e0 + R - 1];
+    if (seg[e0 + R] != r) return;
+    if (seg[e0] == r && e0 > 0 && seg[e0 - 1] == r) return;
+    for (int c = threadIdx.x; c < H; c += blockDim.x) {
+        float sum = bnd[((size_t)blockIdx.x * 2 + 1) * H + c];
+        for (long long u = (long long)blockIdx.x + 1;; ++u) {
+            const long long f0 = u * R, fn = E - f0 < R ? E - f0 : R;
+            sum += bnd[((size_t)u * 2) * H + c];
+            const bool through = seg[f0 + fn - 1] == r && f0 + fn < E && seg[f0 + fn] == r;
+            if (!through) break;
+        }
+        if (out) out[(size_t)r * ldo + c] = sum;
+        if (out16) out16[(size_t)r * ldo16 + c] = f32_to_bf16(sum);
+    }
+}
+
+extern "C" int fabind_segment_sum_sorted(const void* Z, int ldz, int H, const int* seg, const int* segptr, int n_seg, int n_rows,
+                                         float* out, int ldo, void* out16v, int ldo16, float* bnd, hipStream_t stream) {
+    bf16_t* out16 = (bf16_t*)out16v;
+    FB_REQUIRE(H == 64 || H == 128 || H == 256 || H == 512, "fabind_segment_sum_sorted: H must be 64, 128, 256 or 512");
+    FB_REQUIRE(ldz % 8 == 0 && ldz >= H && ((uintptr_t)Z % 16 == 0), "fabind_segment_sum_sorted: Z needs 16-byte rows (ldz % 8 == 0, ldz >= H)");
+    FB_REQUIRE(out != nullptr || out16 != nullptr, "fabind_segment_sum_sorted: no output");
+    FB_REQUIRE(out == nullptr || (ldo % 4 == 0 && ldo >= H && (uintptr_t)out % 16 == 0), "fabind_segment_sum_sorted: out needs 16-byte alignment and ldo % 4 == 0");
+    FB_REQUIRE(out16 == nullptr || (ldo16 % 8 == 0 && ldo16 >= H && (uintptr_t)out16 % 16 == 0), "fabind_segment_sum_sorted: out16 needs 16-byte alignment and ldo16 % 8 == 0");
+    FB_REQUIRE(n_rows <= 0 || (seg != nullptr && bnd != nullptr && ((uintptr_t)bnd % 16 == 0)), "fabind_segment_sum_sorted: seg / bnd (ceil(n_rows / 64) x 2 x H floats of scratch)");
+    if (n_seg <= 0) return 0;
+    if (segptr != nullptr) {
+        const int rc = fabind_zero_empty_rows(segptr, n_seg, out ? (void*)out : (void*)out16, out ? FB_DT_F32 : FB_DT_BF16, out ? ldo : ldo16, H,
+                                              (out && out16) ? (void*)out16 : nullptr, FB_DT_BF16, ldo16, stream);
+        if (rc != 0) return rc;
+    }
+    if (n_rows > 0) {
+        const int n_chunks = (n_rows + 63) / 64;
+        const int rows_wg = 256 * 512 / H;
+        const dim3 g((unsigned)(((long long)n_rows + rows_wg - 1) / rows_wg));
+        if (H == 512) hipLaunchKernelGGL((segment_sum_sorted_kernel<64>), g, dim3(256), 0, stream, (const bf16_t*)Z, ldz, seg, n_rows, out, ldo, out16, ldo16, bnd);
+        else if (H == 256) hipLaunchKernelGGL((segment_sum_sorted_kernel<32>), g, dim3(256), 0, stream, (const bf16_t*)Z, ldz, seg, n_rows, out, ldo, out16, ldo16, bnd);
+        else if (H == 128) hipLaunchKernelGGL((segment_sum_sorted_kernel<16>), g, dim3(256), 0, stream, (const bf16_t*)Z, ldz, seg, n_rows, out, ldo, out16, ldo16, bnd);
+        else hipLaunchKernelGGL((segment_sum_sorted_kernel<8>), g, dim3(256), 0, stream, (const bf16_t*)Z, ldz, seg, n_rows, out, ldo, out16, ldo16, bnd);
+        if (n_chunks > 1)
+            hipLaunchKernelGGL(segment_sum_sorted_fix_kernel, dim3(n_chunks - 1), dim3(H < 256 ? H : 256), 0, stream, seg, n_rows, H, bnd, out, ldo,
+                               out16, ldo16);
+    }
+    FB_CHECK_LAUNCH();
+    return 0;
+}
+
 __global__ __launch_bounds__(256) void coord_update_kernel(const float* __restrict__ x, const float* __restrict__ d,
                                                            const float* __restrict__ s_part, int n_part,
                                                            const float* weight, const int* rowptr, int n_rows, int mean,
diff --git a/fabind_amd/engine.py b/fabind_amd/engine.py
--- a/fabind_amd/engine.py
+++ b/fabind_amd/engine.py
@@ -114,6 +114,13 @@
         return out
 
 
+def _sending_order(colsorted, perm):
+    E = perm.shape[0]
+    slot = torch.empty(E, dtype=torch.int32, device=perm.device)
+    slot[perm] = torch.arange(E, dtype=torch.int32, device=perm.device)
+    return slot, colsorted.to(torch.int32).contiguous()
+
+
 class Graph:
     _warned_fallback = False
 
@@ -163,6 +170,7 @@
             lay.node_off, lay.c_cnt, lay.B, rp_int, self.col_int, self.row_int)
         self.int_deal = (torch.argsort(deg_int, descending=True, stable=True).to(torch.int32), int(n_heavy), int(n_act))
         self._ctx_bycol = None
+        self._ctx_sending = None
         self.N = lay.N
 
     def int_by_col(self):
@@ -175,7 +183,12 @@
             colptr = torch.zeros(self.N + 1, dtype=torch.int32, device=perm.device)
             colptr[1:] = torch.cumsum(cnt, 0).to(torch.int32)
             self._ctx_bycol = (colptr, perm.to(torch.int32).contiguous())
+            self._ctx_sending = _sending_order(colsorted, perm)
         return self._ctx_bycol
+
+    def ctx_sending(self):
+        self.ctx_by_col()
+        return self._ctx_sending
 
 
 def _cat(ts, d=0):
@@ -751,7 +764,12 @@
             cp = torch.zeros(self.N + 1, dtype=torch.int32, device=perm.device)
             cp[1:] = torch.cumsum(torch.bincount(cs, minlength=self.N), 0).to(torch.int32)
             self._bycol = (cp, perm.to(torch.int32).contiguous())
+            self._sending = _sending_order(cs, perm)
         return self._bycol
+
+    def ctx_sending(self):
+        self.ctx_by_col()
+        return self._sending
 
 
 class BatchOnlyLayout:
diff --git a/fabind_amd/kernels.py b/fabind_amd/kernels.py
--- a/fabind_amd/kernels.py
+++ b/fabind_amd/kernels.py
@@ -216,6 +216,27 @@
     return out if out is not None else out16
 
 
+def segment_sum_sorted(Z, seg, n_seg, segptr=None, out=None, out16=None, bnd=None):
+    n, H = Z.shape
+    assert Z.dtype == torch.bfloat16 and seg.dtype == torch.int32 and seg.shape[0] == n and seg.is_contiguous()
+    if out is None and out16 is None:
+        out = torch.empty((n_seg, H), dtype=torch.float32, device=Z.device)
+    if bnd is None:
+        bnd = torch.empty(((n + 63) // 64 * 2 + 2, H), dtype=torch.float32, device=Z.device)
+    assert bnd.dtype == torch.float32 and bnd.is_contiguous() and bnd.numel() >= (n + 63) // 64 * 2 * H
+    check(_lib.load().fabind_segment_sum_sorted(ptr(Z) if n > 0 else None, _ld(Z), H, ptr(seg) if n > 0 else None, ptr(segptr), n_seg, n,
+                                                ptr(out), _ld(out) if out is not None else 0, ptr(out16),
+                                                _ld(out16) if out16 is not None else 0, ptr(bnd), stream()), "fabind_segment_sum_sorted")
+    return out if out is not None else out16
+
+
+def edge_sending_order(col, perm):
+    E = perm.shape[0]
+    slot = torch.empty(E, dtype=torch.int32, device=perm.device)
+    slot[perm.long()] = torch.arange(E, dtype=torch.int32, device=perm.device)
+    return slot, col[perm.long()].to(torch.int32).contiguous()
+
+
 def coord_update(x, d, s_part, rowptr, mean, clampv, weight=None, want_s=False):
     n_rows = x.shape[0]
     x_out = torch.empty_like(x)
@@ -703,7 +724,7 @@
 
 
 def gcl_edge_fused_bwd(AB16, H, row, col, rhohat, w_r, W2, b2, Wc, bc, w3, ds, dagg, colptr, perm, p_drop=0.0, seed=0,
-                       dab_bf16=False, w_dtype=torch.float32, rowptr=None, frags=None, saved=None):
+                       dab_bf16=False, w_dtype=torch.float32, rowptr=None, frags=None, saved=None, sending=None):
     E, N, dev = row.shape[0], AB16.shape[0], AB16.device
     ng = _N_CU.get(dev)
     if ng is None:
@@ -755,19 +776,26 @@
     a.dbg = ptr(EDGE_BWD_TIMES) if (EDGE_BWD_TIMES is not None and variant != 6) else None
     if variant == 6:
         a.d2f, a.z3f = ptr(saved[1]), ptr(saved[2])
+    if sending is None and E > 0:
+        sending = edge_sending_order(col, perm)
+    if not sending or E == 0 or E * H * 2 >= 2 ** 32:
+        sending = None
+    slot = sending[0] if sending is not None else None
+    assert slot is None or (slot.dtype == torch.int32 and slot.shape[0] == E and slot.is_contiguous())
     _profiled(("gcl_edge_fused_bwd4_kernel<%d> E=%d (2 chained H x H contractions per edge over the forward's saved tiles)" % (H, E)) if variant == 6 else
               "gcl_edge_fused_bwd%s_kernel<%d> E=%d (recompute + 4 chained H x H contractions per edge)" % ("3" if variant == 5 else "", H, E),
               (4.0 if variant == 6 else 8.0) * E * H * H,
-              lambda: check(_lib.load().fabind_gcl_edge_fused_bwd(ctypes.byref(a), H, ng, stream()),
+              lambda: check(_lib.load().fabind_gcl_edge_fused_bwd_slot(ctypes.byref(a), H, ng, ptr(slot), stream()),
                             "fabind_gcl_edge_fused_bwd"),
               E * ((12.0 if variant == 6 else 10.0) * H + 20) + N * (4.0 * H + 4.0 * H + (2.0 if dab_bf16 else 4.0) * H),
               algo=N * (2.0 * H * 2 + 4.0 * H + 2.0 * H * (2.0 if dab_bf16 else 4.0)) + E * 20.0)
     del keep
     if E > 0:
-        if dab_bf16:
-            segment_sum(dP1[:E], colptr, N, eidx=perm, out16=dAB[:, H:])
+        half = {"out16": dAB[:, H:]} if dab_bf16 else {"out": dAB[:, H:]}
+        if sending is not None:
+            segment_sum_sorted(dP1[:E], sending[1], N, segptr=colptr, bnd=bnd, **half)
         else:
-            segment_sum(dP1[:E], colptr, N, eidx=perm, out=dAB[:, H:])
+            segment_sum(dP1[:E], colptr, N, eidx=perm, **half)
         if tn_can_queue(dP2[:E], S1[:E], W2.data_ptr()) and tn_can_queue(dT[:E], Mm[:E], Wc.data_ptr()):
             dW2, dWc = torch.empty((H, H), dtype=w_dtype, device=dev), torch.empty((H, H), dtype=w_dtype, device=dev)
             gemm_tn_queued(dP2[:E], S1[:E], dW2, key=W2.data_ptr())
diff --git a/fabind_amd/ops.py b/fabind_amd/ops.py
--- a/fabind_amd/ops.py
+++ b/fabind_amd/ops.py
@@ -633,7 +633,7 @@
         dAB, drh, dwr, dW2, db2, dWc, dbc, dw3 = K.gcl_edge_fused_bwd(
             AB16, ctx.H, g.row_ctx, g.col_ctx, rhohat, w_r, W2, b2, Wc, bc, w3, ds.reshape(-1).float(), dagg.float(),
             colptr, perm, ctx.p_drop, ctx.seed, dab_bf16=AB16.dtype == torch.bfloat16, w_dtype=W2.dtype, rowptr=g.rp_ctx, frags=ctx.frags,
-            saved=saved)
+            saved=saved, sending=g.ctx_sending() if hasattr(g, "ctx_sending") else None)
         return (dAB.to(AB16.dtype), drh, dwr, dW2.to(W2.dtype), db2, dWc.to(Wc.dtype), dbc, dw3, None, None, None, None, None, None)
 
 
@@ -662,7 +662,8 @@
             ds = torch.zeros(g.row_ctx.shape[0], dtype=torch.float32, device=AB.device)
         dAB, drh, dwr, dW2, db2, dWc, dbc, dw3 = K.gcl_edge_fused_bwd(
             AB.to(torch.bfloat16), ctx.H, g.row_ctx, g.col_ctx, rhohat, w_r, W2, b2, Wc, bc, w3, ds.reshape(-1).float(), dagg.float(),
-            colptr, perm, ctx.p_drop, ctx.seed, dab_bf16=False, w_dtype=torch.float32, rowptr=g.rp_ctx, saved=saved)
+            colptr, perm, ctx.p_drop, ctx.seed, dab_bf16=False, w_dtype=torch.float32, rowptr=g.rp_ctx, saved=saved,
+            sending=g.ctx_sending() if hasattr(g, "ctx_sending") else None)
         return (dAB, drh, dwr, dW2, db2, dWc, dbc, dw3, None, None, None, None)
 
 
diff --git a/include/fabind_hip.h b/include/fabind_hip.h
--- a/include/fabind_hip.h
+++ b/include/fabind_hip.h
@@ -131,6 +131,8 @@
                        int act, float* out, int ldo,
                        void* out16 , int ldo16,
                        hipStream_t stream);
+int fabind_segment_sum_sorted(const void* Z, int ldz, int H, const int* seg, const int* segptr, int n_seg, int n_rows, float* out,
+                              int ldo, void* out16, int ldo16, float* bnd, hipStream_t stream);
 int fabind_zero_empty_rows(const int* rowptr, int n_rows, void* out, int out_dt, int ld, int C, void* out2, int out2_dt, int ld2,
                            hipStream_t stream);
 int fabind_coord_update(const float* x, const float* d, const float* s_part, int n_part, const float* weight,
@@ -177,6 +179,7 @@
     const void* z3f;
 } FabindEdgeBwdArgs;
 int fabind_gcl_edge_fused_bwd(const FabindEdgeBwdArgs* args, int H, int n_groups, hipStream_t stream);
+int fabind_gcl_edge_fused_bwd_slot(const FabindEdgeBwdArgs* args, int H, int n_groups, const int* dp1_slot, hipStream_t stream);
 int fabind_gcl_edge_fused_bwd_set_tile(int bm);
 int fabind_gcl_edge_fused_bwd_tile(void);
 int fabind_gcl_edge_fused_bwd_set_variant(int v);
```
